# adrelino/mv-lm-icp

Hardware: AMD Instinct MI355X
Metric: ICP iterations/sec (NN+Jacobian+LM) (higher is better)
Workload: dtype f64; 1 GPU; cfg4: multiview 32 views x 200k pts, point-to-plane, SophusSE3 (E=62); views=32, pts_per_view=200000, edges=62, parallelism=single GPU, nn=auto

## Files before the change

mv-lm-icp_amd/csrc/api.cpp:

```cpp
#include <algorithm>
#include <cmath>
#include <cstring>
#include <ctime>
#include <chrono>
#include <condition_variable>
#include <exception>
#include <limits>
#include <mutex>
#include <new>
#include <thread>

#include "common.h"
#include "comm.h"
#include "nn_tie.h"
#include "../host/se3.h"

namespace mvicp {

static thread_local char g_err[1024] = "";

void set_error(const char* fmt, ...) {
  va_list ap;
  va_start(ap, fmt);
  vsnprintf(g_err, sizeof(g_err), fmt, ap);
// ... 35 lines not shown

int scratch_upload(mvicp_ctx* c, const void* src, size_t bytes, void** dptr) {
  const size_t aligned = (bytes + 255) & ~(size_t)255;
  if (c->scratch_used + aligned > c->scratch_bytes) {
    if (c->scratch_used != 0) { set_error("scratch overflow (%zu + %zu > %zu)", c->scratch_used, aligned, c->scratch_bytes); return MVICP_ERR_STATE; }
    MV_HIP(hipStreamSynchronize(c->stream));
    if (c->d_scratch) MV_HIP(hipFree(c->d_scratch));
    c->scratch_bytes = std::max<size_t>(aligned * 4, 1 << 20);
    MV_HIP(hipMalloc((void**)&c->d_scratch, c->scratch_bytes));
  }
  void* d = c->d_scratch + c->scratch_used;
  MV_HIP(hipMemcpyAsync(d, src, bytes, hipMemcpyHostToDevice, c->stream));
  MV_HIP(hipStreamSynchronize(c->stream));
  c->scratch_used += aligned;
  *dptr = d;
  return MVICP_OK;
}

ProfScope::ProfScope(mvicp_ctx* ctx, const char* nm, double bytes) : c(ctx), name(nm), on(ctx->profile) {
  if (on && ctx->profile_level >= 2 && ((std::strncmp(nm, "nn_", 3) != 0 && std::strncmp(nm, "linearize", 9) != 0 && std::strcmp(nm, "comm") != 0) ||
                                        std::strcmp(nm, "nn_tie") == 0)) on = false;
  if (!on) return;
  ProfEntry& pe = c->prof[name];
  auto get = [&]() {
    hipEvent_t ev = nullptr;
    if (!pe.pool.empty()) { ev = pe.pool.back(); pe.pool.pop_back(); }
    else if (hipEventCreate(&ev) != hipSuccess) ev = nullptr;
    return ev;
  };
  a = get(); b = get();
  pe.bytes += bytes;
  if (std::strncmp(nm, "nn_", 3) == 0) { pe.survey_bytes += bytes; pe.queries += bytes / 36.0; }
  pe.launches += 1;
  if (a) (void)hipEventRecord(a, c->stream);
}
ProfScope::~ProfScope() {
  if (!on) return;
  if (b) (void)hipEventRecord(b, c->stream);
  if (a && b) c->prof[name].pending.push_back(std::make_pair(a, b));
}
static double now_ms() {
  timespec ts;
  clock_gettime(CLOCK_MONOTONIC, &ts);
  return ts.tv_sec * 1e3 + ts.tv_nsec * 1e-6;
}
HostScope::HostScope(mvicp_ctx* ctx, const char* nm) : c(ctx), name(nm), t0(0.0), on(ctx->profile) { if (on) t0 = now_ms(); }
HostScope::~HostScope() {
  if (!on) return;
  ProfEntry& pe = c->prof[name];
  pe.ms += now_ms() - t0;
  pe.launches += 1;
}
void prof_collect_lazy(mvicp_ctx* c) {
  for (auto& kv : c->prof) if (kv.second.pending.size() > 256) { prof_collect(c); return; }
}
void prof_collect(mvicp_ctx* c) {
  for (auto& kv : c->prof) {
    ProfEntry& pe = kv.second;
    for (auto& pr : pe.pending) {
      float ms = 0.f;
      if (hipEventSynchronize(pr.second) == hipSuccess && hipEventElapsedTime(&ms, pr.first, pr.second) == hipSuccess) pe.ms += ms;
      pe.pool.push_back(pr.first);
      pe.pool.push_back(pr.second);
    }
    pe.pending.clear();
  }
}

namespace {

template <typename T> int dev_alloc(T** p, size_t n) {
  *p = nullptr;
  if (n == 0) n = 1;
  MV_HIP(hipMalloc((void**)p, sizeof(T) * n));
  return MVICP_OK;
}
template <typename T> void dev_free(T*& p) {
  if (p) (void)hipFree(p);
  p = nullptr;
}

void free_graph(mvicp_ctx* c) {
  dev_free(c->d_esrc); dev_free(c->d_edst); dev_free(c->d_cap_off); dev_free(c->d_count);
  dev_free(c->d_ctl); c->d_nsrc = nullptr; c->d_a = nullptr; c->d_xf = nullptr; c->d_rel = nullptr; c->d_rel2 = nullptr; c->d_dirty = nullptr;
  dev_free(c->d_nn_idx); dev_free(c->d_nn_d2); dev_free(c->d_nn_lb); dev_free(c->d_first); dev_free(c->d_second);
  dev_free(c->d_sblock_off); dev_free(c->d_sel_keys1); c->n_sblocks = 0;
  dev_free(c->d_cd2); dev_free(c->d_qpos); dev_free(c->d_dirty_slots); dev_free(c->d_dslot_off); dev_free(c->d_stream); dev_free(c->d_cblock_off); dev_free(c->d_cblock_cnt);
  dev_free(c->d_sel_hist); dev_free(c->d_median); dev_free(c->d_chunk_edge); dev_free(c->d_chunk_start);
  dev_free(c->d_chunk_first); dev_free(c->d_partials); dev_free(c->d_out);
  c->sym_lo_pin.release(); c->sym_lo_dev.release();
  if (c->h_pin) (void)hipHostFree(c->h_pin);
  c->h_pin = nullptr; c->h_pin_doubles = 0; c->d_res_host = nullptr; c->d_blocks_host = nullptr; c->lin_out = nullptr;
  c->census_pending = false; c->spec_ready = false; c->spec2_ready = false; c->spec_arm = false; c->d_spec_host = nullptr; c->d_adev_host = nullptr; c->d_res_target = nullptr; c->d_a_check = nullptr;
  dev_free(c->d_xblock_cnt); c->export_valid = false; c->export_in_flight = false; c->export_chunks = 0;
  for (hipEvent_t ev : c->export_events) (void)hipEventDestroy(ev);
  c->export_events.clear();
  if (c->d_export) (void)hipFree(c->d_export);
  if (c->h_export) (void)hipHostFree(c->h_export);
  c->d_export = nullptr; c->h_export = nullptr; c->export_cap = 0;
  c->E = 0; c->total_cap = 0; c->n_cblocks = 0; c->n_chunks = 0; c->have_corr = false;
}

int bind(mvicp_ctx* c) {
  if (!c) { set_error("null context"); return MVICP_ERR_ARG; }
  MV_HIP(hipSetDevice(c->device));
  return MVICP_OK;
}

double sqrt_bound(double t) {
  double x = t * t;
  while (std::sqrt(x) >= t && x > 0.0) x = std::nextafter(x, 0.0);
  while (std::sqrt(x) < t) x = std::nextafter(x, INFINITY);
  return x;
}

void inverse3(const double* m, double* r) {
#define M(i, j) m[(i) + 3 * (j)]
#define COF(i, j) (M(((i) + 1) % 3, ((j) + 1) % 3) * M(((i) + 2) % 3, ((j) + 2) % 3) - M(((i) + 1) % 3, ((j) + 2) % 3) * M(((i) + 2) % 3, ((j) + 1) % 3))
  const double c00 = COF(0, 0), c10 = COF(1, 0), c20 = COF(2, 0);
  const double det = (c00 * M(0, 0) + c10 * M(1, 0)) + c20 * M(2, 0);
  const double invdet = 1.0 / det;
  r[0] = c00 * invdet; r[3] = c10 * invdet; r[6] = c20 * invdet;
  r[1] = COF(0, 1) * invdet; r[4] = COF(1, 1) * invdet; r[7] = COF(2, 1) * invdet;
  r[2] = COF(0, 2) * invdet; r[5] = COF(1, 2) * invdet; r[8] = COF(2, 2) * invdet;
#undef COF
#undef M
}

void fill_query_xf(const double* Ps, const double* Pd, double* x) {
  double Rd[9];
  for (int j = 0; j < 3; ++j)
    for (int i = 0; i < 3; ++i) { x[i + 3 * j] = Ps[i + 4 * j]; Rd[i + 3 * j] = Pd[i + 4 * j]; }
  for (int i = 0; i < 3; ++i) { x[9 + i] = Ps[12 + i]; x[21 + i] = Pd[12 + i]; }
  inverse3(Rd, x + 12);
}

void query_affine(const double* x, double* Mq) {
  for (int j = 0; j < 3; ++j)
    for (int i = 0; i < 3; ++i) Mq[i + 3 * j] = x[12 + i] * x[0 + 3 * j] + x[12 + i + 3] * x[1 + 3 * j] + x[12 + i + 6] * x[2 + 3 * j];
  const double dt[3] = {x[9] - x[21], x[10] - x[22], x[11] - x[23]};
  for (int i = 0; i < 3; ++i) Mq[9 + i] = x[12 + i] * dt[0] + x[12 + i + 3] * dt[1] + x[12 + i + 6] * dt[2];
}

double cache_allowance_xf(const double* x_old, const double* x_new, double r) {
  if (std::memcmp(x_old, x_new, sizeof(double) * kXfRigid) == 0) return 0.0;
  double b = 0.0;
  for (const double* x : {x_old, x_new}) {
    double fr = 0.0, fi = 0.0;
    for (int k = 0; k < 9; ++k) { fr += x[k] * x[k]; fi += x[12 + k] * x[12 + k]; }
    const double dt[3] = {x[9] - x[21], x[10] - x[22], x[11] - x[23]};
    const double ts = std::sqrt(x[9] * x[9] + x[10] * x[10] + x[11] * x[11]), dtn = std::sqrt(dt[0] * dt[0] + dt[1] * dt[1] + dt[2] * dt[2]);
    b += std::sqrt(fi) * (ts + 16.0 * std::sqrt(fr) * r + 13.0 * dtn);
  }
  return std::max(0x1p-52 * b, std::numeric_limits<double>::min());
}

int ensure_pin(mvicp_ctx* c, size_t doubles) {
  if (doubles <= c->h_pin_doubles) return MVICP_OK;
  if (c->h_pin) MV_HIP(hipHostFree(c->h_pin));
  c->h_pin = nullptr;
  MV_HIP(hipHostMalloc((void**)&c->h_pin, sizeof(double) * doubles, hipHostMallocMapped));
  std::memset(c->h_pin, 0, sizeof(double) * doubles);
  c->h_pin_doubles = doubles;
  return MVICP_OK;
}

}
// ... 128 lines not shown
static int build_frame_structures(mvicp_ctx* c, FrameDev& f, const double* xyz, const double* nrm) {
  if (injected_build_failure(c)) return MVICP_ERR_INTERNAL;
  const auto t0 = std::chrono::steady_clock::now();
  MV_CHECK(build_grid(c, f, xyz));
  if (nrm) MV_CHECK(upload_sorted_normals(f, nrm));
  f.build_ms[0] = std::chrono::duration<double, std::milli>(std::chrono::steady_clock::now() - t0).count();
  f.build_ms[1] = -1.0;
  return MVICP_OK;
}

static int build_frame_structures_device(mvicp_ctx* c, FrameDev& f, const DevBounds& b, int grid_curve, double grid_target) {
  if (injected_build_failure(c)) return MVICP_ERR_INTERNAL;
  return build_grid_device(c, f, b, grid_curve, grid_target);
}

int finish_builds(mvicp_ctx* c) {
  for (FrameDev& f : c->frames) {
    if (!f.job) continue;
    int s1 = MVICP_ERR_INTERNAL;
    try { s1 = f.job->fut.get(); } catch (...) { f.job->err = "structure build threw"; }
    if (s1 != MVICP_OK) {
      f.build_error = f.job->err.empty() ? std::string("structure build failed") : f.job->err;
      (void)hipSetDevice(c->device);
      free_grid(f.grid); f.has_grid = false;
    }
    f.job.reset();
  }
  for (size_t i = 0; i < c->frames.size(); ++i)
    if (!c->frames[i].build_error.empty()) {
      set_error("frame %d: %s (upload the cloud again with mvicp_set_frame)", (int)i, c->frames[i].build_error.c_str());
      return MVICP_ERR_STATE;
    }
  return MVICP_OK;
}

static void throttle_builds(mvicp_ctx* c) {
  const int limit = std::max(2, (int)std::min(32u, std::thread::hardware_concurrency()));
  for (;;) {
    int pending = 0;
    BuildJob* oldest = nullptr;
    for (FrameDev& f : c->frames)
      if (f.job && f.job->fut.valid() && f.job->fut.wait_for(std::chrono::seconds(0)) != std::future_status::ready) { if (!oldest) oldest = f.job.get(); ++pending; }
    if (pending < limit || !oldest) return;
    oldest->fut.wait();
  }
}

static int check_evaluable(mvicp_ctx* c, int metric) {
  if (!c->have_corr) { set_error("no correspondences: call mvicp_correspond or mvicp_set_correspondences first"); return MVICP_ERR_STATE; }
  if (metric == MVICP_METRIC_SYMMETRIC) {
    for (int e = 0; e < c->E; ++e)
      if (c->owned[e] && c->h_count[e] > 0) {
        const int missing = c->frames[c->edst[e]].grid.snor == nullptr ? c->edst[e] : c->frames[c->esrc[e]].grid.snor == nullptr ? c->esrc[e] : -1;
        if (missing >= 0) { set_error("symmetric needs normals on frame %d", missing); return MVICP_ERR_STATE; }
      }
  } else if (metric) {
    for (int e = 0; e < c->E; ++e)
      if (c->owned[e] && c->h_count[e] > 0 && c->frames[c->edst[e]].grid.snor == nullptr) {
        set_error("point-to-plane needs normals on frame %d", c->edst[e]);
        return MVICP_ERR_STATE;
      }
  }
  return MVICP_OK;
}

int evaluate_pair(mvicp_ctx* c, const double* poses_a, const double* poses_b, int plane, int robust, double* out_a, double* out_b) {
  MV_CHECK(check_evaluable(c, plane));
  HostScope hs(c, "host.evaluate");
  const size_t n = (size_t)c->E * MVICP_EDGE_BLOCK;
  fill_rel_into(c, poses_b, c->h_pin + c->ctl_rel2_off);
  fill_rel(c, poses_a);
  MV_HIP(hipMemcpyAsync(c->d_rel2, c->h_pin + c->ctl_rel2_off, sizeof(double) * ((size_t)c->E * kEdgeRel + c->ctl_r2), hipMemcpyHostToDevice, c->stream));
  MV_CHECK(launch_linearize_pair(c, plane, robust, c->d_blocks_host, c->d_blocks2_host));
  MV_CHECK(stream_wait(c));
  std::memcpy(out_a, c->h_pin + c->pin_blocks_off, sizeof(double) * n);
  std::memcpy(out_b, c->h_pin + c->pin_blocks2_off, sizeof(double) * n);
  return MVICP_OK;
}

static int launch_metric(mvicp_ctx* c, int metric, int robust) {
  return metric == MVICP_METRIC_SYMMETRIC ? launch_linearize_sym(c, robust) : launch_linearize(c, metric, robust);
}

int evaluate_blocks(mvicp_ctx* c, const double* poses, int plane, int robust, double* out) {
  MV_CHECK(check_evaluable(c, plane));
  HostScope hs(c, "host.evaluate");
  const size_t n = (size_t)c->E * MVICP_EDGE_BLOCK;
  if (c->spec_ready) {
    c->spec_ready = false;
    if (plane == c->spec_q_plane && robust == c->spec_q_robust && c->spec_poses.size() == 16 * (size_t)c->n_frames &&
        std::memcmp(poses, c->spec_poses.data(), sizeof(double) * c->spec_poses.size()) == 0) {
      std::memcpy(out, c->h_pin + c->pin_spec_off, sizeof(double) * n);
      if (c->profile) c->prof["spec.hit"].launches += 1;
      return MVICP_OK;
    }
    c->spec2_ready = false;
  }
  if (c->spec2_ready) {
    c->spec2_ready = false;
    if (plane == c->spec2_plane && robust == c->spec2_robust && c->spec2_poses.size() == 16 * (size_t)c->n_frames &&
        std::memcmp(poses, c->spec2_poses.data(), sizeof(double) * c->spec2_poses.size()) == 0) {
      std::memcpy(out, c->h_pin + c->pin_spec2_off, sizeof(double) * n);
      if (c->profile) c->prof["spec2.hit"].launches += 1;
      c->last_cand_poses.assign(poses, poses + 16 * (size_t)c->n_frames); c->last_cand_plane = plane; c->last_cand_robust = robust;
      return MVICP_OK;
    }
  }
  c->last_cand_poses.assign(poses, poses + 16 * (size_t)c->n_frames); c->last_cand_plane = plane; c->last_cand_robust = robust;
  double* h = c->h_pin + c->pin_blocks_off;
  if (c->comm || c->ar_fn) {
    c->lin_out = c->d_out;
    int st_l = plane == MVICP_METRIC_SYMMETRIC ? upload_rel_sym(c, poses) : upload_rel(c, poses);
    if (st_l == MVICP_OK && c->fault_inject_eval > 0 && --c->fault_inject_eval == 0) { set_error("injected launch failure (option fault_inject_eval)"); st_l = MVICP_ERR_HIP; }
    if (st_l == MVICP_OK) st_l = launch_metric(c, plane, robust);
    char local_msg[sizeof(g_err)] = "";
    if (st_l != MVICP_OK) std::memcpy(local_msg, g_err, sizeof(local_msg));
    if (hipMemsetAsync(c->d_out + n, st_l == MVICP_OK ? 0 : 0xFF, sizeof(double), c->stream) != hipSuccess) {
      if (st_l != MVICP_OK) return st_l;
      set_error("hipMemsetAsync of the poison slot failed"); return MVICP_ERR_HIP;
    }
    { ProfScope pc(c, "comm", 8.0 * (double)(n + 1)); MV_CHECK(comm_allreduce_sum(c, c->d_out, n + 1)); }
    double* hx = c->h_pin + c->pin_spec_off;
    MV_HIP(hipMemcpyAsync(hx, c->d_out, sizeof(double) * (n + 1), hipMemcpyDeviceToHost, c->stream));
    MV_CHECK(stream_wait(c));
    if (std::isnan(hx[n])) {
      if (st_l != MVICP_OK) { set_error("%s", local_msg); return st_l; }
      set_error("a peer rank failed before the exchange of this evaluation (poisoned exchange buffer)");
      return MVICP_ERR_COMM;
    }
    std::memcpy(out, hx, sizeof(double) * n);
    return MVICP_OK;
  } else {
    MV_CHECK(plane == MVICP_METRIC_SYMMETRIC ? upload_rel_sym(c, poses) : upload_rel(c, poses));
    c->lin_out = c->d_blocks_host;
    MV_CHECK(launch_metric(c, plane, robust));
  }
  MV_CHECK(stream_wait(c));
  std::memcpy(out, h, sizeof(double) * n);
  return MVICP_OK;
}

}

using namespace mvicp;

extern "C" {

const char* mvicp_last_error(void) { return g_err; }
const char* mvicp_version(void) { return "mvicp_hip 0.5 (gfx950)"; }

int mvicp_create(int device, mvicp_ctx** out) try {
  if (!out) { set_error("out is null"); return MVICP_ERR_ARG; }
  *out = nullptr;
  int ndev = 0;
  hipError_t e = hipGetDeviceCount(&ndev);
  if (e != hipSuccess || ndev <= 0) {
    set_error("no HIP device available (%s): libmvicp_hip has no CPU fallback", e == hipSuccess ? "device count 0" : hipGetErrorString(e));
    return MVICP_ERR_HIP;
  }
  if (device < 0 || device >= ndev) { set_error("device %d out of range [0,%d)", device, ndev); return MVICP_ERR_ARG; }
  mvicp_ctx* c = new mvicp_ctx();
  c->device = device;
  MV_HIP(hipSetDevice(device));
  MV_HIP(hipStreamCreateWithFlags(&c->stream, hipStreamNonBlocking));
  *out = c;
  return MVICP_OK;
} MVICP_GUARD_ABI

static void release_stages(mvicp_ctx* c) {
  c->vox.release(); c->out.release(); c->knn.release(); c->fpfh.release();
  c->match.release(); c->cons.release(); c->coarse.release(); c->iss.release();
}

int mvicp_destroy(mvicp_ctx* c) try {
  if (!c) return MVICP_OK;
  (void)hipSetDevice(c->device);
  (void)finish_builds(c);
  (void)hipStreamSynchronize(c->stream);
  comm_destroy(c);
  free_graph(c);
  for (FrameDev& f : c->frames) { dev_free(f.pts); dev_free(f.nor); free_grid(f.grid); free_tie(f); }
  dev_free(c->d_split_idx); dev_free(c->d_split_d2); dev_free(c->d_scratch);
  free_overlap(c);
  release_stages(c);
  for (auto& kv : c->tables) if (kv.second.d) (void)hipFree(kv.second.d);
  if (c->d_census) (void)hipFree(c->d_census);
  if (c->h_census) (void)hipHostFree(c->h_census);
  if (c->d_tie_list) (void)hipFree(c->d_tie_list);
  if (c->d_tie_count) (void)hipFree(c->d_tie_count);
  if (c->d_tie_deep) (void)hipFree(c->d_tie_deep);
  if (c->h_tie_seen) (void)hipHostFree(c->h_tie_seen);
  if (c->h_far_seen) (void)hipHostFree(c->h_far_seen);
  if (c->d_far_list) (void)hipFree(c->d_far_list);
  if (c->d_far_count) (void)hipFree(c->d_far_count);
  for (auto& kv : c->prof) {
    for (auto& pr : kv.second.pending) { (void)hipEventDestroy(pr.first); (void)hipEventDestroy(pr.second); }
    for (hipEvent_t ev : kv.second.pool) (void)hipEventDestroy(ev);
  }
  (void)hipStreamDestroy(c->stream);
  delete c;
  return MVICP_OK;
} MVICP_GUARD_ABI

int mvicp_set_num_frames(mvicp_ctx* c, int n_frames) try {
  MV_CHECK(bind(c));
  if (n_frames < 0) { set_error("n_frames < 0"); return MVICP_ERR_ARG; }
  (void)finish_builds(c);
  if (c->E) free_graph(c);
  release_stages(c);
  for (FrameDev& f : c->frames) { dev_free(f.pts); dev_free(f.nor); free_grid(f.grid); free_tie(f); }
  c->frames.assign(n_frames, FrameDev());
  c->n_frames = n_frames;
  return MVICP_OK;
} MVICP_GUARD_ABI

int mvicp_set_frame(mvicp_ctx* c, int frame, const double* xyz, const double* nrm, int n) try {
  MV_CHECK(bind(c));
  if (frame < 0 || frame >= c->n_frames) { set_error("frame %d out of range [0,%d)", frame, c->n_frames); return MVICP_ERR_ARG; }
  if (n < 0 || (n > 0 && !xyz)) { set_error("bad cloud (n=%d)", n); return MVICP_ERR_ARG; }
  if (c->E) { set_error("set frames before mvicp_set_graph"); return MVICP_ERR_STATE; }
// ... 662 lines not shown
    });
    const int take = std::min<int>(knn, (int)cand.size());
    for (int k = 0; k < take; ++k) {
      parent[root(i)] = root(cand[k]);
      if (i == 0 && skip_frame0) continue;
      if (n_edges >= cap) { set_error("more than cap = %d edges (frame %d of %d, knn = %d)", cap, i, K, knn); return MVICP_ERR_ARG; }
      if (!src || !dst) { set_error("src / dst is null"); return MVICP_ERR_ARG; }
      src[n_edges] = i; dst[n_edges] = cand[k]; ++n_edges;
    }
  }
  if (n_components) {
    int comps = 0;
    for (int i = 0; i < K; ++i) comps += root(i) == i ? 1 : 0;
    *n_components = comps;
  }
  return n_edges;
} MVICP_GUARD_ABI

int mvicp_set_graph(mvicp_ctx* c, int n_edges, const int* src, const int* dst) try {
  MV_CHECK(bind(c));
  if (n_edges < 0 || (n_edges > 0 && (!src || !dst))) { set_error("bad edge list"); return MVICP_ERR_ARG; }
  for (int e = 0; e < n_edges; ++e)
    if (src[e] < 0 || src[e] >= c->n_frames || dst[e] < 0 || dst[e] >= c->n_frames || src[e] == dst[e]) {
      set_error("edge %d (%d->%d) invalid", e, src[e], dst[e]);
      return MVICP_ERR_ARG;
    }
  MV_CHECK(finish_builds(c));
  free_graph(c);
  const int E = n_edges;
  c->E = E;
  c->esrc.assign(src, src + E);
  c->edst.assign(dst, dst + E);
  c->owned.assign(E, 0);
  c->active.assign(E, 0);
  c->h_count.assign(E, 0);
  c->h_weight.assign(E, 0.f);
  {
    std::vector<int> ns(E), owner(E);
    for (int e = 0; e < E; ++e) ns[e] = c->frames[src[e]].n;
    MV_CHECK(mvicp_edge_owner(E, ns.data(), c->world, owner.data()));
    for (int e = 0; e < E; ++e) c->owned[e] = owner[e] == c->rank;
  }
  {
    double total = 0;
    for (int e = 0; e < E; ++e) total += c->frames[src[e]].n;
    c->lin_chunk = total >= 6e6 ? 8192 : total >= 2e6 ? 4096 : total >= 5e5 ? 1024 : 512;
    if (c->lin_chunk_override > 0) c->lin_chunk = c->lin_chunk_override;
  }
  const int kLinChunk = c->lin_chunk;
  c->cap_off.assign(E + 1, 0);
  c->cblock_off.assign(E + 1, 0);
  c->chunk_first.assign(E + 1, 0);
  std::vector<int> chunk_edge, chunk_start;
  for (int e = 0; e < E; ++e) {
    const long long n = c->owned[e] ? c->frames[src[e]].n : 0;
    c->cap_off[e + 1] = c->cap_off[e] + ((n + 63) / 64) * 64;
    c->cblock_off[e + 1] = c->cblock_off[e] + (int)((n + kCompactBlock - 1) / kCompactBlock);
    const int nch = (int)((n + kLinChunk - 1) / kLinChunk);
    c->chunk_first[e + 1] = c->chunk_first[e] + nch;
    for (int k = 0; k < nch; ++k) { chunk_edge.push_back(e); chunk_start.push_back(k * kLinChunk); }
  }
  c->total_cap = c->cap_off[E];
  c->n_cblocks = c->cblock_off[E];
  c->n_chunks = c->chunk_first[E];
  if (c->lin_interleave) {
    std::vector<int> ce, cs;
    for (int e0 = 0; e0 < E;) {
      int e1 = e0 + 1;
      while (e1 < E && src[e1] == src[e0]) ++e1;
      int maxc = 0;
      for (int e = e0; e < e1; ++e) maxc = std::max(maxc, c->chunk_first[e + 1] - c->chunk_first[e]);
      for (int g = 0; g < maxc; g += 8)
        for (int e = e0; e < e1; ++e) {
          const int nch = c->chunk_first[e + 1] - c->chunk_first[e];
          for (int k = g; k < std::min(g + 8, nch); ++k) { ce.push_back(e); cs.push_back(k * kLinChunk); }
        }
      e0 = e1;
    }
    chunk_edge.swap(ce); chunk_start.swap(cs);
  }
  const size_t cap = (size_t)c->total_cap;
  MV_CHECK(dev_alloc(&c->d_esrc, E)); MV_CHECK(dev_alloc(&c->d_edst, E)); MV_CHECK(dev_alloc(&c->d_cap_off, E + 1));
  MV_CHECK(dev_alloc(&c->d_count, E));
  c->ctl_r1 = (size_t)E * kEdgeXf + (size_t)E + 2 * (size_t)E;
  c->ctl_rel2_off = (c->ctl_r1 + 1) & ~(size_t)1;
  c->ctl_r2_off = c->ctl_rel2_off + (size_t)E * kEdgeRel;
  c->ctl_r2 = (size_t)E * (kEdgeRel + 1);
  MV_CHECK(dev_alloc(&c->d_ctl, c->ctl_r2_off + c->ctl_r2));
  MV_HIP(hipMemset(c->d_ctl, 0, sizeof(double) * std::max<size_t>(c->ctl_r2_off + c->ctl_r2, 1)));
  c->d_xf = c->d_ctl; c->d_nsrc = reinterpret_cast<int*>(c->d_ctl + (size_t)E * kEdgeXf); c->d_dirty = c->d_nsrc + E;
  c->d_sel_lohi = c->d_ctl + (size_t)E * (kEdgeXf + 1);
  c->sel_med1.assign(E, -1.0); c->sel_med2.assign(E, -1.0);
  c->d_rel = c->d_ctl + c->ctl_r2_off; c->d_a = c->d_rel + (size_t)E * kEdgeRel; c->d_rel2 = c->d_ctl + c->ctl_rel2_off;
  MV_CHECK(dev_alloc(&c->d_nn_idx, cap)); MV_CHECK(dev_alloc(&c->d_nn_d2, cap)); MV_CHECK(dev_alloc(&c->d_nn_lb, cap));
  c->nn_cache_valid = false; c->prev_q.assign((size_t)E * 12, 0.0); c->nn_cache_edge.assign(E, 0);
  c->auto_prev_dist = 0.0; c->auto_last_method = -1; c->corr_tie_seen = c->corr_far_seen = 1u;
  MV_CHECK(dev_alloc(&c->d_first, cap)); MV_CHECK(dev_alloc(&c->d_second, cap)); MV_CHECK(dev_alloc(&c->d_cd2, cap));
  MV_CHECK(dev_alloc(&c->d_stream, 10 * cap));
  MV_CHECK(dev_alloc(&c->d_qpos, cap));
  MV_HIP(hipMemset(c->d_qpos, 0xff, sizeof(int) * std::max<size_t>(cap, 1)));
  c->list_valid.assign(E, 0); c->explicit_list.assign(E, 0); c->export_valid = false; c->export_off.assign((size_t)E + 1, 0);
  c->qpos_valid.assign(E, 0); c->corr_epoch.assign(E, 0);
  for (int e = 0; e < E; ++e) c->corr_epoch[e] = ++c->epoch_counter;
  c->dslot_off.assign(E + 1, 0);
  for (int e = 0; e < E; ++e) c->dslot_off[e + 1] = c->dslot_off[e] + (int)(((c->owned[e] ? c->frames[src[e]].n : 0) + 255) / 256);
  c->n_dslots = c->dslot_off[E];
  MV_CHECK(dev_alloc(&c->d_dirty_slots, (size_t)c->n_dslots)); MV_CHECK(dev_alloc(&c->d_dslot_off, (size_t)E + 1));
  MV_HIP(hipMemset(c->d_dirty_slots, 0, sizeof(int) * std::max<size_t>((size_t)c->n_dslots, 1)));
  MV_HIP(hipMemcpy(c->d_dslot_off, c->dslot_off.data(), sizeof(int) * (E + 1), hipMemcpyHostToDevice));
  MV_CHECK(dev_alloc(&c->d_cblock_off, E + 1)); MV_CHECK(dev_alloc(&c->d_cblock_cnt, (size_t)c->n_cblocks));
  MV_CHECK(dev_alloc(&c->d_sel_hist, (size_t)E * (2048 + 2)));
  MV_HIP(hipMemset(c->d_sel_hist, 0, sizeof(unsigned int) * std::max<size_t>((size_t)E * (2048 + 2), 1)));
  c->sel_scratch_clean = true; c->sel_result_valid = false; c->sel_result_armed = false;
  c->sblock_off.assign(E + 1, 0);
  for (int e = 0; e < E; ++e) c->sblock_off[e + 1] = c->sblock_off[e] + (int)(((c->owned[e] ? c->frames[src[e]].n : 0) + kSelBlock - 1) / kSelBlock);
  c->n_sblocks = c->sblock_off[E];
  MV_CHECK(dev_alloc(&c->d_sblock_off, (size_t)E + 1));
  MV_HIP(hipMemcpy(c->d_sblock_off, c->sblock_off.data(), sizeof(int) * (E + 1), hipMemcpyHostToDevice));
  MV_CHECK(dev_alloc(&c->d_sel_keys1, cap));
  if (cap > c->far_cap) {
    if (c->d_far_list) MV_HIP(hipFree(c->d_far_list));
    c->d_far_list = nullptr; c->far_cap = 0;
    MV_HIP(hipMalloc(&c->d_far_list, sizeof(int) * 2 * cap));
    c->far_cap = cap;
  }
  MV_CHECK(warm_nn_grid(c)); MV_CHECK(warm_nn_tile(c)); MV_CHECK(warm_nn_mfma(c));
  if (c->tie_rule && !(c->tie_lazy && c->world == 1)) {
    std::vector<int> need;
    for (int e = 0; e < E; ++e) if (c->owned[e]) need.push_back(dst[e]);
    MV_CHECK(ensure_tie_trees(c, need));
  }
  MV_CHECK(dev_alloc(&c->d_median, E));
  MV_CHECK(dev_alloc(&c->d_chunk_edge, (size_t)c->n_chunks)); MV_CHECK(dev_alloc(&c->d_chunk_start, (size_t)c->n_chunks));
  MV_CHECK(dev_alloc(&c->d_chunk_first, E + 1));
  MV_CHECK(dev_alloc(&c->d_partials, 2 * (size_t)c->n_chunks * kLinPartial));
  MV_CHECK(dev_alloc(&c->d_out, (size_t)E * (MVICP_EDGE_BLOCK + 3) + 2));
  MV_HIP(hipMemset(c->d_out, 0, sizeof(double) * ((size_t)E * (MVICP_EDGE_BLOCK + 3) + 2)));
  if (E) {
    MV_HIP(hipMemcpy(c->d_esrc, src, sizeof(int) * E, hipMemcpyHostToDevice));
    MV_HIP(hipMemcpy(c->d_edst, dst, sizeof(int) * E, hipMemcpyHostToDevice));
    MV_HIP(hipMemset(c->d_count, 0, sizeof(int) * E));
  }
  MV_HIP(hipMemcpy(c->d_cap_off, c->cap_off.data(), sizeof(long long) * (E + 1), hipMemcpyHostToDevice));
  MV_HIP(hipMemcpy(c->d_cblock_off, c->cblock_off.data(), sizeof(int) * (E + 1), hipMemcpyHostToDevice));
  MV_HIP(hipMemcpy(c->d_chunk_first, c->chunk_first.data(), sizeof(int) * (E + 1), hipMemcpyHostToDevice));
  if (c->n_chunks) {
    MV_HIP(hipMemcpy(c->d_chunk_edge, chunk_edge.data(), sizeof(int) * c->n_chunks, hipMemcpyHostToDevice));
    MV_HIP(hipMemcpy(c->d_chunk_start, chunk_start.data(), sizeof(int) * c->n_chunks, hipMemcpyHostToDevice));
  }
  c->pin_blocks_off = c->ctl_r2_off + c->ctl_r2;
  c->pin_res_off = c->pin_blocks_off + (size_t)E * MVICP_EDGE_BLOCK;
  c->pin_misc_off = c->pin_res_off + 2 * (size_t)E + 2;
  c->pin_spec_off = c->pin_misc_off + 4 * (size_t)E + 64;
  c->pin_adev_off = c->pin_spec_off + (size_t)E * (MVICP_EDGE_BLOCK + 3) + 2;
  if (c->h_pin) { MV_HIP(hipHostFree(c->h_pin)); c->h_pin = nullptr; c->h_pin_doubles = 0; }
  c->pin_spec2_off = (c->pin_adev_off + (size_t)E + 8 + 1) & ~(size_t)1;
  c->pin_rel2_off = c->pin_spec2_off + (size_t)E * MVICP_EDGE_BLOCK + ((size_t)E * MVICP_EDGE_BLOCK & 1);
  c->pin_blocks2_off = (c->pin_rel2_off + (size_t)E * kEdgeRel + 1) & ~(size_t)1;
  MV_CHECK(ensure_pin(c, c->pin_blocks2_off + (size_t)E * MVICP_EDGE_BLOCK + 8));
  {
    void* dp = nullptr;
    MV_HIP(hipHostGetDevicePointer(&dp, c->h_pin, 0));
    c->d_blocks_host = (double*)dp + c->pin_blocks_off;
    c->d_res_host = (double*)dp + c->pin_res_off;
    c->d_spec_host = (double*)dp + c->pin_spec_off;
    c->d_adev_host = (double*)dp + c->pin_adev_off;
    c->d_spec2_host = (double*)dp + c->pin_spec2_off;
    c->d_blocks2_host = (double*)dp + c->pin_blocks2_off;
  }
  c->spec_ready = false; c->spec_arm = false;
  c->spec2_ready = false; c->spec2_armed = false; c->last_cand_poses.clear();
  c->prev_xf.assign((size_t)E * kXfRigid, 0.0);
  if (!c->h_census) MV_HIP(hipHostMalloc((void**)&c->h_census, 8 * sizeof(unsigned long long), hipHostMallocDefault));
  return MVICP_OK;
} MVICP_GUARD_ABI

static void forget_history(mvicp_ctx* c) {
  const int E = c->E;
  c->nn_cache_valid = false; c->nn_cache_thresh = -1.f;
  c->prev_q.assign((size_t)E * 12, 0.0); c->prev_xf.assign((size_t)E * kXfRigid, 0.0);
  c->nn_cache_edge.assign(E, 0);
  c->auto_prev_dist = 0.0; c->auto_last_method = -1; c->last_rms = -1.0; c->prev_grid_kernel = false;
  c->corr_tie_seen = c->corr_far_seen = 1u;
  c->list_valid.assign(E, 0);
  c->export_valid = false;
  c->qpos_valid.assign(E, 0);
  for (int e = 0; e < E; ++e) c->corr_epoch[e] = ++c->epoch_counter;
  c->sel_med1.assign(E, -1.0); c->sel_med2.assign(E, -1.0);
  c->sel_result_valid = false;
  c->spec_ready = false; c->spec_arm = false; c->spec_flags_valid = false;
  c->spec2_ready = false; c->spec2_armed = false; c->last_cand_poses.clear();
  c->have_corr = false;
  std::fill(c->h_count.begin(), c->h_count.end(), 0); std::fill(c->h_weight.begin(), c->h_weight.end(), 0.f);
}

int mvicp_reset_history(mvicp_ctx* c) try {
  MV_CHECK(bind(c));
  MV_HIP(hipStreamSynchronize(c->stream));
  forget_history(c);
  return MVICP_OK;
} MVICP_GUARD_ABI

static int correspond_once(mvicp_ctx* c, const double* poses, const unsigned char* fixed, float thresh, int nn_method, int* counts, float* weights, bool* tie_unresolved);

int mvicp_correspond(mvicp_ctx* c, const double* poses, const unsigned char* fixed, float thresh, int nn_method, int* counts, float* weights) try {
  MV_CHECK(bind(c));
  struct Forget { mvicp_ctx* c; bool ok = false; ~Forget() { if (!ok) { (void)hipStreamSynchronize(c->stream); forget_history(c); } } } forget{c};
  bool unresolved = false;
  MV_CHECK(correspond_once(c, poses, fixed, thresh, nn_method, counts, weights, &unresolved));
  if (!unresolved) { forget.ok = true; return MVICP_OK; }
  std::vector<int> need;
  for (int e = 0; e < c->E; ++e) if (c->active[e] && !c->frames[c->edst[e]].has_tie) need.push_back(c->edst[e]);
  MV_HIP(hipStreamSynchronize(c->stream));
  MV_CHECK(ensure_tie_trees(c, need));
  forget_history(c);
  unresolved = false;
  MV_CHECK(correspond_once(c, poses, fixed, thresh, nn_method, counts, weights, &unresolved));
  if (unresolved) { set_error("tie fix-up still without a tree after building them"); return MVICP_ERR_INTERNAL; }
  forget.ok = true;
  return MVICP_OK;
} MVICP_GUARD_ABI

static int correspond_body(mvicp_ctx* c, const double* poses, const unsigned char* fixed, float thresh, int nn_method, int* counts, float* weights, bool* tie_unresolved);

static int correspond_once(mvicp_ctx* c, const double* poses, const unsigned char* fixed, float thresh, int nn_method, int* counts, float* weights, bool* tie_unresolved) {
  struct Guard { mvicp_ctx* c; bool ok = false; ~Guard() { if (!ok) { c->sel_result_valid = false; c->sel_scratch_clean = false; } } } guard{c};
  const int st = correspond_body(c, poses, fixed, thresh, nn_method, counts, weights, tie_unresolved);
  guard.ok = st == MVICP_OK;
  return st;
}

static int correspond_body(mvicp_ctx* c, const double* poses, const unsigned char* fixed, float thresh, int nn_method, int* counts, float* weights, bool* tie_unresolved) {
  if (!poses) { set_error("poses is null"); return MVICP_ERR_ARG; }
  if (c->E == 0) { set_error("no graph: call mvicp_set_graph first"); return MVICP_ERR_STATE; }
  const int E = c->E;
  HostScope hs_all(c, "host.correspond");
  std::vector<int> nsrc(E, 0);
  std::vector<char> same_edge(E, 0);
  std::vector<char> unchanged(E, 0);
  const bool hist_ok = c->have_corr && (int)c->nn_cache_edge.size() == E && c->nn_cache_thresh == thresh && (int)c->qpos_valid.size() == E;
  std::vector<double> eps_ratio;
  bool same_active_set = (int)c->nn_cache_edge.size() == E;
  double* hx = c->h_pin;
  for (int e = 0; e < E; ++e) {
    c->active[e] = c->owned[e] && !(fixed && fixed[c->esrc[e]]);
    if (same_active_set && (c->active[e] != 0) != (c->nn_cache_edge[e] != 0)) same_active_set = false;
    nsrc[e] = c->active[e] ? c->frames[c->esrc[e]].n : 0;
    const double* Ps = poses + 16 * (size_t)c->esrc[e];
    const double* Pd = poses + 16 * (size_t)c->edst[e];
    double* x = hx + (size_t)e * kEdgeXf;
    fill_query_xf(Ps, Pd, x);
    double Mq[12];
    query_affine(x, Mq);
    double* pq = &c->prev_q[(size_t)e * 12];
    for (int k = 0; k < 12; ++k) x[kXfDM + k] = Mq[k] - pq[k];
    const double rmax = c->frames[c->esrc[e]].max_norm;
    if (c->active[e]) {
      double fro = 0.0;
      for (int k = 0; k < 9; ++k) fro += x[kXfDM + k] * x[kXfDM + k];
      const double eps_e = std::sqrt(fro) * rmax + std::sqrt(x[kXfDv] * x[kXfDv] + x[kXfDv + 1] * x[kXfDv + 1] + x[kXfDv + 2] * x[kXfDv + 2]);
      const double mu_e = c->tile_mu * c->frames[c->edst[e]].grid.cell;
      eps_ratio.push_back(mu_e > 0.0 ? eps_e / mu_e : 1e300);
    }
    const bool cache_on = c->nn_cache_valid && c->nn_cache_enable && c->active[e] && (int)c->nn_cache_edge.size() == E && c->nn_cache_edge[e] &&
                          c->nn_cache_thresh == thresh;
    double* pxf = &c->prev_xf[(size_t)e * kXfRigid];
    if (!c->owned[e]) unchanged[e] = 1;
    else if (c->active[e]) unchanged[e] = hist_ok && c->nn_cache_edge[e] && c->qpos_valid[e] && !c->explicit_list[e] && std::memcmp(pxf, x, sizeof(double) * kXfRigid) == 0;
    else unchanged[e] = hist_ok && !c->nn_cache_edge[e] && !c->explicit_list[e] && c->h_count[e] == 0;
    const bool same_xf = cache_on && std::memcmp(pxf, x, sizeof(double) * kXfRigid) == 0;
    x[kXfCache] = cache_on ? cache_allowance_xf(pxf, x, rmax) : -1.0;
    same_edge[e] = same_xf;
    std::memcpy(pxf, x, sizeof(double) * kXfRigid);
    for (int k = kXfPad; k < kEdgeXf; ++k) x[k] = 0.0;
    std::memcpy(pq, Mq, sizeof(Mq));
  }
  int* hn = reinterpret_cast<int*>(hx + (size_t)E * kEdgeXf);
  int* hd = hn + E;
  std::memcpy(hn, nsrc.data(), sizeof(int) * E);

  int st_local = MVICP_OK;
  if (c->tie_rule && !(c->tie_lazy && c->world == 1)) {
    std::vector<int> need;
    for (int e = 0; e < E; ++e) if (c->active[e] && !c->frames[c->edst[e]].has_tie) need.push_back(c->edst[e]);
    if (!need.empty()) st_local = ensure_tie_trees(c, need);
  }
  const double bound = sqrt_bound((double)thresh);
  double t_mark = now_ms();
  auto mark = [&](const char* nm) { if (c->profile) { const double t = now_ms(); ProfEntry& pe = c->prof[nm]; pe.ms += t - t_mark; pe.launches += 1; t_mark = t; } };
  mark("host.corr.setup");
  int method = nn_method;
  if (method == MVICP_NN_AUTO) {
    method = MVICP_NN_TILE;
    if (c->have_corr) {
      double dist = 0.0, cell = 0.0;
      int m = 0;
      for (int e = 0; e < E; ++e)
        if (c->h_count[e] > 0) { dist += c->h_weight[e] / 1.5; cell += c->frames[c->edst[e]].grid.cell; ++m; }
      if (m > 0) {
        dist /= m; cell /= m;
        const bool settled = c->auto_prev_dist > 0.0 ? dist > c->auto_settle * c->auto_prev_dist : dist < 0.5 * cell;
        if (c->nn_cell) {
          double pred = dist;
          if (c->last_rms >= 0.0) pred = std::min(pred, std::sqrt(c->last_rms * c->last_rms + 0.09 * cell * cell));
          if (pred < c->auto_switch * cell || c->auto_last_method == MVICP_NN_GRID) method = MVICP_NN_GRID;
        } else if (dist < 1.5 * cell && (settled || c->auto_last_method == MVICP_NN_GRID)) method = MVICP_NN_GRID;
        c->auto_prev_dist = dist;
      }
    }
  }
  if (method == MVICP_NN_GRID || method == MVICP_NN_TILE) {
    for (int e = 0; e < E; ++e)
      if (c->active[e] && (!c->frames[c->edst[e]].has_grid || !c->frames[c->esrc[e]].has_grid)) method = MVICP_NN_BRUTE;
  }
  bool tile_lb = false, handed_over = false;
  if (nn_method == MVICP_NN_AUTO && method == MVICP_NN_GRID && c->auto_last_method == MVICP_NN_TILE && c->tile_bounds >= 1 &&
      c->nn_cache_enable && !c->nn_cell) { method = MVICP_NN_TILE; tile_lb = true; handed_over = true; }
  if (method == MVICP_NN_TILE && c->tile_bounds >= 2 && c->nn_cache_enable) tile_lb = true;
  bool tile_cached = false;
  bool all_same = true;
  {
    for (int e = 0; e < E; ++e) if (c->active[e] && !same_edge[e]) all_same = false;
    if (nn_method == MVICP_NN_AUTO && method == MVICP_NN_GRID && !handed_over && c->tile_cache && c->tile_bounds >= 1 && c->nn_cache_valid &&
        c->nn_cache_enable && !c->nn_cell && !all_same) { method = MVICP_NN_TILE; tile_lb = true; tile_cached = true; handed_over = true; }
    if (method == MVICP_NN_TILE && !tile_cached && c->tile_cache >= 2 && tile_lb && c->nn_cache_valid && c->nn_cache_enable && !all_same) tile_cached = true;
  }
  {
    std::vector<int> dirty(E, 1);
    if ((method == MVICP_NN_TILE || (method == MVICP_NN_GRID && !c->nn_tree_only && !c->nn_skip_far)) && c->list_reuse)
      for (int e = 0; e < E; ++e) if (c->active[e] && c->list_valid[e]) dirty[e] = 0;
    std::memcpy(hd, dirty.data(), sizeof(int) * E);
  }
  bool use_bracket = c->sel_bracket && c->have_corr;
  {
    double* lohi = hx + (size_t)E * (kEdgeXf + 1);
    for (int e = 0; e < E; ++e) {
      lohi[2 * e] = lohi[2 * e + 1] = 0.0;
      if (!c->active[e]) continue;
      const double m1 = c->sel_med1[e], m2 = c->sel_med2[e];
      if (!(m1 > 0.0 && m2 > 0.0 && std::fabs(m1 - m2) <= 0.001 * m1)) { use_bracket = false; continue; }
      lohi[2 * e] = m1 * 0.994; lohi[2 * e + 1] = m1 * 1.006;
    }
  }
  bool nothing_can_change = method == MVICP_NN_GRID && c->list_reuse && !c->nn_tree_only && !c->nn_skip_far && same_active_set && !c->nn_cell;
  for (int e = 0; e < E && nothing_can_change; ++e)
    if (c->active[e] && !(same_edge[e] && hd[e] == 0)) nothing_can_change = false;
  c->skip_dirty_reduce = nothing_can_change;
  c->tie_skip = nothing_can_change && c->corr_tie_seen == 0u;
  c->far_skip = nothing_can_change && c->corr_far_seen == 0u && c->prev_grid_kernel && method == MVICP_NN_GRID;
  const bool tie_launched = c->tie_rule && !c->tie_skip, far_launched = method == MVICP_NN_GRID && !c->far_skip;
  const bool exchange = c->comm != nullptr || c->ar_fn != nullptr;
  c->spec_ready = false; c->spec2_ready = false;
  c->spec_arm = c->spec_enable && c->spec_flags_valid;
  if (c->spec_arm && c->spec_plane)
    for (int e = 0; e < E; ++e) if (!(fixed && fixed[c->esrc[e]]) && c->frames[c->edst[e]].n > 0 && c->frames[c->edst[e]].grid.snor == nullptr) c->spec_arm = false;
  const size_t nb = (size_t)E * MVICP_EDGE_BLOCK, ntail = 3 * (size_t)E + 1;
  c->d_res_target = exchange ? c->d_out + nb : nullptr;
  c->d_a_check = exchange ? c->d_out + nb + 2 * (size_t)E + 1 : c->d_adev_host;
  size_t upload_doubles = c->ctl_r1;
  bool spec2_plan = false;
  if (c->spec_arm) {
    c->spec_poses.resize(16 * (size_t)c->n_frames);
    double xp[7];
    for (int k = 0; k < c->n_frames; ++k) { se3::pose_to_x(c->spec_param, poses + 16 * (size_t)k, xp); se3::x_to_pose(c->spec_param, xp, &c->spec_poses[16 * (size_t)k]); }
    fill_rel(c, c->spec_poses.data());
    c->spec_q_plane = c->spec_plane; c->spec_q_robust = c->spec_robust;
    upload_doubles = c->ctl_r2_off + (size_t)E * kEdgeRel;
    spec2_plan = !exchange && c->spec2_enable && all_same && same_active_set && c->have_corr && c->last_cand_poses.size() == 16 * (size_t)c->n_frames &&
                 c->last_cand_plane == c->spec_q_plane && c->last_cand_robust == c->spec_q_robust;
    if (spec2_plan && c->lin_pair) fill_rel_into(c, c->last_cand_poses.data(), hx + c->ctl_rel2_off);
  }
  const bool sel_skip = !exchange && c->sel_reuse && nothing_can_change && c->sel_result_valid && (!c->spec_arm || c->sel_result_armed);
  if (method != MVICP_NN_BRUTE && method != MVICP_NN_GRID && method != MVICP_NN_TILE) { set_error("unknown nn_method %d", nn_method); return MVICP_ERR_ARG; }
  bool all_unchanged = true;
  for (int e = 0; e < E; ++e) { if (!unchanged[e]) all_unchanged = false; if (c->active[e]) c->qpos_valid[e] = 0; }
  auto local_search = [&]() -> int {
  MV_HIP(hipMemcpyAsync(c->d_ctl, hx, sizeof(double) * upload_doubles, hipMemcpyHostToDevice, c->stream));
  c->far_narrow = nn_method == MVICP_NN_AUTO && method == MVICP_NN_GRID && c->nn_cache_valid && c->nn_cache_enable && all_same;
  if (c->fault_inject > 0 && --c->fault_inject == 0) { set_error("injected launch failure (option fault_inject)"); return MVICP_ERR_HIP; }
  if (method == MVICP_NN_BRUTE) MV_CHECK(launch_nn_brute_edges(c));
  else if (method == MVICP_NN_GRID) MV_CHECK(launch_nn_grid_edges(c, bound));
  else {
    c->cached_on_mfma = false;
    if (tile_cached && c->tile_mfma == 1 && c->cache_mfma_ratio > 0.0 && !eps_ratio.empty()) {
      std::nth_element(eps_ratio.begin(), eps_ratio.begin() + eps_ratio.size() / 2, eps_ratio.end());
      const double med = eps_ratio[eps_ratio.size() / 2];
      if (c->profile) { ProfEntry& pe = c->prof["auto.eps_over_mu"]; pe.ms = med; pe.launches += 1; }
      c->cached_on_mfma = med > c->cache_mfma_ratio;
    }
    MV_CHECK(launch_nn_tile_edges(c, bound, tile_lb, tile_cached, c->list_reuse));
  }
  c->tie_skip = false; c->far_skip = false;
  c->prev_grid_kernel = method == MVICP_NN_GRID;
  c->last_rms = -1.0;
  c->nn_cache_valid = ((method == MVICP_NN_GRID) && !c->nn_tree_only && !c->nn_skip_far) || tile_lb;
  c->nn_cache_thresh = thresh;
  c->auto_last_method = handed_over ? MVICP_NN_GRID : method;
  c->nn_cache_edge.assign(c->active.begin(), c->active.end());
  for (int e = 0; e < E; ++e) { c->list_valid[e] = c->active[e]; if (c->owned[e]) c->qpos_valid[e] = c->active[e]; if (c->active[e]) c->explicit_list[e] = 0; }
  if (!all_unchanged) c->export_valid = false;

  mark("host.corr.nn_launch");
  if (!nothing_can_change) {
    MV_CHECK(launch_compact(c, bound));
    MV_CHECK(launch_gather_stream(c));
  }
  if (sel_skip) { c->h_pin[c->pin_res_off + 2 * (size_t)E] = c->spec_arm ? 1.0 : 0.0; return MVICP_OK; }
  return use_bracket ? launch_select_bracket(c) : launch_select_median(c, bound);
  };
  if (st_local == MVICP_OK) st_local = local_search();
  if (st_local != MVICP_OK && !exchange) { c->spec_flags_valid = false; return st_local; }
  int st_q = MVICP_OK;
  char local_msg[sizeof(g_err)] = "";
  if (exchange) {
    c->lin_out = c->d_out;
    if (st_local == MVICP_OK) {
      if (c->spec_arm) st_local = launch_linearize(c, c->spec_q_plane, c->spec_q_robust);
      else {
        if (hipMemsetAsync(c->d_out, 0, sizeof(double) * nb, c->stream) != hipSuccess ||
            hipMemsetAsync(c->d_out + nb + 2 * (size_t)E + 1, 0, sizeof(double) * (size_t)E, c->stream) != hipSuccess) { set_error("hipMemsetAsync of the exchange buffer failed"); st_local = MVICP_ERR_HIP; }
      }
    }
    if (st_local != MVICP_OK) {
      std::memcpy(local_msg, g_err, sizeof(local_msg));
      if (hipMemsetAsync(c->d_out + nb + 2 * (size_t)E, 0xFF, sizeof(double), c->stream) != hipSuccess) {
        set_error("%s — and the exchange buffer could not be poisoned: the peers of this rank will block in the collective", local_msg);
        c->spec_flags_valid = false; c->spec_arm = false;
        return st_local;
      }
    }
    { ProfScope pc(c, "comm", 8.0 * (double)(nb + ntail)); st_q = comm_allreduce_sum(c, c->d_out, nb + ntail); }
    if (st_q == MVICP_OK && hipMemcpyAsync(c->h_pin + c->pin_spec_off, c->d_out, sizeof(double) * (nb + ntail), hipMemcpyDeviceToHost, c->stream) != hipSuccess) {
      set_error("hipMemcpyAsync of the exchanged buffer failed"); st_q = MVICP_ERR_HIP;
    }
  } else if (c->spec_arm && spec2_plan && c->lin_pair) {
    c->spec2_armed = false;
    st_q = launch_linearize_pair(c, c->spec_q_plane, c->spec_q_robust, c->d_spec_host, c->d_spec2_host);
    if (st_q == MVICP_OK) { c->spec2_armed = true; c->spec2_poses = c->last_cand_poses; c->spec2_plane = c->spec_q_plane; c->spec2_robust = c->spec_q_robust; }
  } else if (c->spec_arm) {
    c->lin_out = c->d_spec_host;
    st_q = launch_linearize(c, c->spec_q_plane, c->spec_q_robust);
    c->spec2_armed = false;
    if (st_q == MVICP_OK && spec2_plan) {
      fill_rel_into(c, c->last_cand_poses.data(), c->h_pin + c->pin_rel2_off);
      if (hipMemcpyAsync(c->d_rel, c->h_pin + c->pin_rel2_off, sizeof(double) * (size_t)E * kEdgeRel, hipMemcpyHostToDevice, c->stream) == hipSuccess) {
        c->lin_out = c->d_spec2_host;
        st_q = launch_linearize(c, c->spec_q_plane, c->spec_q_robust);
        if (st_q == MVICP_OK) { c->spec2_armed = true; c->spec2_poses = c->last_cand_poses; c->spec2_plane = c->spec_q_plane; c->spec2_robust = c->spec_q_robust; }
      }
    }
  }
  mark("host.corr.post_launch");
  if (st_q == MVICP_OK) st_q = stream_wait(c);
  if (st_q != MVICP_OK) { c->spec_flags_valid = false; c->spec_arm = false; return st_q; }
  if (exchange && std::isnan(c->h_pin[c->pin_spec_off + nb + 2 * (size_t)E])) {
    forget_history(c);
    c->census_pending = false;
    if (st_local != MVICP_OK) { set_error("%s", local_msg); return st_local; }
    set_error("a peer rank failed before the exchange of this search (poisoned exchange buffer); nothing was updated, cross-round state dropped on every rank");
    return MVICP_ERR_COMM;
  }
  census_resolve(c);
  if (tie_launched) c->corr_tie_seen = c->h_tie_seen ? *c->h_tie_seen : 1u;
  if (tie_launched && c->h_tie_seen && c->h_tie_seen[1] != 0u) *tie_unresolved = true;
  if (tie_launched && c->h_tie_seen && c->h_tie_seen[2] != 0u) { set_error("tie fix-up: a walk ran out of stack (a tree deeper than its recorded levels)"); return MVICP_ERR_INTERNAL; }
  if (far_launched) c->corr_far_seen = c->h_far_seen ? *c->h_far_seen : 1u;
  else if (method != MVICP_NN_GRID) c->corr_far_seen = 1u;
  mark("host.corr.wait");
  const double* hr = exchange ? c->h_pin + c->pin_spec_off + nb : c->h_pin + c->pin_res_off;
  bool spec_bad = false;
  {
    bool redo = false;
    for (int e = 0; e < E; ++e) if (hr[2 * e + 1] < 0.0) redo = true;
    if (redo) {
      spec_bad = true;
      int st_r = launch_select_median(c, bound);
      if (exchange) {
        int st_x = MVICP_OK;
        if (st_r != MVICP_OK) {
          std::memcpy(local_msg, g_err, sizeof(local_msg));
          if (hipMemsetAsync(c->d_out + nb + 2 * (size_t)E, 0xFF, sizeof(double), c->stream) != hipSuccess) { c->spec_flags_valid = false; c->spec_arm = false; return st_r; }
        }
        { ProfScope pc(c, "comm", 8.0 * (double)ntail); st_x = comm_allreduce_sum(c, c->d_out + nb, ntail); }
        if (st_x == MVICP_OK && hipMemcpyAsync(c->h_pin + c->pin_spec_off + nb, c->d_out + nb, sizeof(double) * ntail, hipMemcpyDeviceToHost, c->stream) != hipSuccess) {
          set_error("hipMemcpyAsync of the exchanged tail failed"); st_x = MVICP_ERR_HIP;
        }
        if (st_x == MVICP_OK) st_x = stream_wait(c);
        if (st_x != MVICP_OK) { c->spec_flags_valid = false; c->spec_arm = false; return st_x; }
// ... 182 lines not shown
  c->have_corr = true;
  const int one = 1;
  MV_HIP(hipMemcpy(c->d_dirty + edge, &one, sizeof(int), hipMemcpyHostToDevice));
  MV_CHECK(launch_gather_stream(c));
  MV_HIP(hipStreamSynchronize(c->stream));
  return MVICP_OK;
} MVICP_GUARD_ABI

int mvicp_nn_query(mvicp_ctx* c, int frame, const double* queries, int n, int nn_method, int* idx, double* d2) try {
  MV_CHECK(bind(c));
  if (frame < 0 || frame >= c->n_frames) { set_error("frame %d out of range", frame); return MVICP_ERR_ARG; }
  if (n < 0 || (n && (!queries || !idx || !d2))) { set_error("bad query buffers"); return MVICP_ERR_ARG; }
  if (nn_method < MVICP_NN_AUTO || nn_method > MVICP_NN_TILE) { set_error("unknown nn_method %d", nn_method); return MVICP_ERR_ARG; }
  MV_CHECK(finish_builds(c));
  const FrameDev& f = c->frames[frame];
  if (f.n == 0) { set_error("frame %d is empty (nanoflann throws here: nanoflann.hpp:904)", frame); return MVICP_ERR_STATE; }
  if (n == 0) return MVICP_OK;
  double* dq = nullptr; int* di = nullptr; double* dd = nullptr;
  MV_CHECK(dev_alloc(&dq, 3 * (size_t)n)); MV_CHECK(dev_alloc(&di, (size_t)n)); MV_CHECK(dev_alloc(&dd, (size_t)n));
  MV_HIP(hipMemcpy(dq, queries, sizeof(double) * 3 * (size_t)n, hipMemcpyHostToDevice));
  int method = (nn_method == MVICP_NN_AUTO || nn_method == MVICP_NN_TILE) ? MVICP_NN_GRID : nn_method;
  if (c->tie_rule) MV_CHECK(ensure_tie_trees(c, std::vector<int>(1, frame)));
  c->tie_skip = false;
  if (method == MVICP_NN_GRID && !f.has_grid) method = MVICP_NN_BRUTE;
  int st;
  if (method == MVICP_NN_BRUTE) st = launch_nn_brute_queries(c, f, dq, n, di, dd);
  else if (method == MVICP_NN_GRID) st = launch_nn_grid_queries(c, f, dq, n, di, dd);
  else { set_error("unknown nn_method %d", nn_method); st = MVICP_ERR_ARG; }
  if (st == MVICP_OK) {
    hipError_t e1 = hipStreamSynchronize(c->stream);
    if (e1 == hipSuccess) census_resolve(c);
    if (e1 == hipSuccess && c->tie_rule && c->h_tie_seen && c->h_tie_seen[2] != 0u) { set_error("tie fix-up: a walk ran out of stack (a tree deeper than its recorded levels)"); st = MVICP_ERR_INTERNAL; }
    hipError_t e2 = hipMemcpy(idx, di, sizeof(int) * n, hipMemcpyDeviceToHost);
    hipError_t e3 = hipMemcpy(d2, dd, sizeof(double) * n, hipMemcpyDeviceToHost);
    if (e1 != hipSuccess || e2 != hipSuccess || e3 != hipSuccess) { set_error("nn_query copy-back failed"); st = MVICP_ERR_HIP; }
  }
  dev_free(dq); dev_free(di); dev_free(dd);
  if (c->profile) prof_collect_lazy(c);
  return st;
} MVICP_GUARD_ABI

int mvicp_linearize(mvicp_ctx* c, const double* poses, int point_to_plane, int robust, double* out) try {
  MV_CHECK(bind(c));
  if (!poses || !out) { set_error("null argument"); return MVICP_ERR_ARG; }
  if (c->E == 0) { set_error("no graph"); return MVICP_ERR_STATE; }
  MV_CHECK(evaluate_blocks(c, poses, point_to_plane ? MVICP_METRIC_PLANE : MVICP_METRIC_POINT, robust, out));
  if (c->profile) prof_collect_lazy(c);
  return MVICP_OK;
} MVICP_GUARD_ABI

int mvicp_linearize_metric(mvicp_ctx* c, const double* poses, int metric, int robust, double* out) try {
  if (metric != MVICP_METRIC_POINT && metric != MVICP_METRIC_PLANE && metric != MVICP_METRIC_SYMMETRIC) { set_error("metric %d is not an mvicp_metric", metric); return MVICP_ERR_ARG; }
  MV_CHECK(bind(c));
  if (!poses || !out) { set_error("null argument"); return MVICP_ERR_ARG; }
  if (c->E == 0) { set_error("no graph"); return MVICP_ERR_STATE; }
  MV_CHECK(evaluate_blocks(c, poses, metric, robust, out));
  if (c->profile) prof_collect_lazy(c);
  return MVICP_OK;
} MVICP_GUARD_ABI

int mvicp_linearize_pair(mvicp_ctx* c, const double* poses_a, const double* poses_b, int point_to_plane, int robust, double* out_a, double* out_b) try {
  MV_CHECK(bind(c));
  if (!poses_a || !poses_b || !out_a || !out_b) { set_error("null argument"); return MVICP_ERR_ARG; }
  if (c->E == 0) { set_error("no graph"); return MVICP_ERR_STATE; }
  if (c->comm || c->ar_fn) {
    MV_CHECK(evaluate_blocks(c, poses_a, point_to_plane ? MVICP_METRIC_PLANE : MVICP_METRIC_POINT, robust, out_a));
    MV_CHECK(evaluate_blocks(c, poses_b, point_to_plane ? MVICP_METRIC_PLANE : MVICP_METRIC_POINT, robust, out_b));
  } else {
    MV_CHECK(evaluate_pair(c, poses_a, poses_b, point_to_plane ? MVICP_METRIC_PLANE : MVICP_METRIC_POINT, robust, out_a, out_b));
  }
  if (c->profile) prof_collect_lazy(c);
  return MVICP_OK;
} MVICP_GUARD_ABI

int mvicp_set_option(mvicp_ctx* c, const char* name, double value) try {
  MV_CHECK(bind(c));
  if (!name) { set_error("null option name"); return MVICP_ERR_ARG; }
  if (std::strcmp(name, "async_build") == 0) { c->async_build = value != 0.0; return MVICP_OK; }
  if (std::strcmp(name, "grid_target") == 0 || std::strcmp(name, "grid_curve") == 0) MV_CHECK(finish_builds(c));
  if (std::strcmp(name, "nn_tree_only") == 0) { c->nn_tree_only = value != 0.0; return MVICP_OK; }
  if (std::strcmp(name, "nn_cache") == 0) { c->nn_cache_enable = value != 0.0; c->nn_cache_valid = false; return MVICP_OK; }
  if (std::strcmp(name, "lin_chunk") == 0) { c->lin_chunk_override = (int)value; return MVICP_OK; }
  if (std::strcmp(name, "list_reuse") == 0) { c->list_reuse = value != 0.0; return MVICP_OK; }
  if (std::strcmp(name, "lin_interleave") == 0) { c->lin_interleave = value != 0.0; return MVICP_OK; }
  if (std::strcmp(name, "lin_share_p") == 0) { c->lin_share_p = value != 0.0; return MVICP_OK; }
  if (std::strcmp(name, "lin_pair") == 0) { c->lin_pair = value != 0.0; return MVICP_OK; }
  if (std::strcmp(name, "nn_census") == 0) { c->nn_census = value != 0.0; return MVICP_OK; }
  if (std::strcmp(name, "nn_skip_far") == 0) { c->nn_skip_far = value != 0.0; return MVICP_OK; }
  if (std::strcmp(name, "sel_bracket") == 0) { c->sel_bracket = value != 0.0; return MVICP_OK; }
  if (std::strcmp(name, "sel_reuse") == 0) { c->sel_reuse = value != 0.0; return MVICP_OK; }
  if (std::strcmp(name, "prune_rho") == 0) { c->prune_rho = value; return MVICP_OK; }
  if (std::strcmp(name, "grid_curve") == 0) { c->grid_curve = (int)value; return MVICP_OK; }
  if (std::strcmp(name, "auto_settle") == 0) { c->auto_settle = value; return MVICP_OK; }
  if (std::strcmp(name, "auto_switch") == 0) { c->auto_switch = value; return MVICP_OK; }
  if (std::strcmp(name, "nn_cell") == 0) { c->nn_cell = value != 0.0; return MVICP_OK; }
  if (std::strcmp(name, "nn_search_factor") == 0) { if (!(value >= 0.0)) { set_error("nn_search_factor < 0"); return MVICP_ERR_ARG; } c->nn_search_factor = value; c->nn_cache_valid = false; return MVICP_OK; }
  if (std::strcmp(name, "tie_rule") == 0) {
    const bool on = value != 0.0;
    if (on != c->tie_rule) { MV_HIP(hipStreamSynchronize(c->stream)); c->tie_rule = on; forget_history(c); }
    return MVICP_OK;
  }
  if (std::strcmp(name, "tie_lazy") == 0) { c->tie_lazy = value != 0.0; return MVICP_OK; }
  if (std::strcmp(name, "tile_seed") == 0) { c->tile_seed = value != 0.0; return MVICP_OK; }
  if (std::strcmp(name, "tile_bounds") == 0) { c->tile_bounds = (int)value; return MVICP_OK; }
  if (std::strcmp(name, "tile_mu") == 0) { if (!(value > 0.0 && value <= 1.0)) { set_error("tile_mu outside (0, 1]"); return MVICP_ERR_ARG; } c->tile_mu = value; return MVICP_OK; }
  if (std::strcmp(name, "mfma_kacc") == 0) { if (!(value >= 1.0 && value <= 1024.0)) { set_error("mfma_kacc outside [1, 1024]"); return MVICP_ERR_ARG; } c->mfma_kacc = value; return MVICP_OK; }
  if (std::strcmp(name, "mfma_lbt") == 0) { c->mfma_lbt = (int)value; return MVICP_OK; }
  if (std::strcmp(name, "mfma_entry") == 0) { c->mfma_entry = (int)value; return MVICP_OK; }
  if (std::strcmp(name, "mfma_trig") == 0) { c->mfma_trig = (int)value; return MVICP_OK; }
  if (std::strcmp(name, "tile_mfma") == 0) { c->tile_mfma = (int)value; return MVICP_OK; }
  if (std::strcmp(name, "tile_waves") == 0) { c->tile_waves = (int)value; return MVICP_OK; }
  if (std::strcmp(name, "cache_mfma_ratio") == 0) { c->cache_mfma_ratio = value; return MVICP_OK; }
  if (std::strcmp(name, "reject_cache") == 0) { c->reject_cache = value != 0.0; return MVICP_OK; }
  if (std::strcmp(name, "tile_miss") == 0) { if (!(value >= 0.0 && value <= 64.0)) { set_error("tile_miss outside [0, 64]"); return MVICP_ERR_ARG; } c->tile_miss = (int)value; return MVICP_OK; }
  if (std::strcmp(name, "tile_cache") == 0) { c->tile_cache = (int)value; return MVICP_OK; }
  if (std::strcmp(name, "voxel_permute") == 0) { c->voxel_permute = value != 0.0; return MVICP_OK; }
  if (std::strcmp(name, "knn_order") == 0) { c->knn_order = value != 0.0; return MVICP_OK; }
  if (std::strcmp(name, "match_chunk") == 0) {
    if (!(value >= 1.0 && value < 2147483648.0)) { set_error("match_chunk must be in [1, 2^31)"); return MVICP_ERR_ARG; }
    c->match_chunk = (int)value; return MVICP_OK;
  }
  if (std::strcmp(name, "spin_wait") == 0) { c->spin_wait = value != 0.0; return MVICP_OK; }
  if (std::strcmp(name, "fault_inject") == 0) { c->fault_inject = (int)value; return MVICP_OK; }
  if (std::strcmp(name, "fault_inject_build") == 0) { c->fault_inject_build.store((int)value); return MVICP_OK; }
  if (std::strcmp(name, "fault_inject_eval") == 0) { c->fault_inject_eval = (int)value; return MVICP_OK; }
  if (std::strcmp(name, "spec_eval") == 0) { c->spec_enable = value != 0.0; c->spec_ready = false; c->spec2_ready = false; return MVICP_OK; }
  if (std::strcmp(name, "spec2_eval") == 0) { c->spec2_enable = value != 0.0; c->spec2_ready = false; return MVICP_OK; }
  if (std::strcmp(name, "grid_target") == 0) {
    if (!(value >= 0.5 && value <= 64.0)) { set_error("grid_target out of range"); return MVICP_ERR_ARG; }
    c->grid_target = value;
    return MVICP_OK;
  }
  set_error("unknown option '%s'", name);
  return MVICP_ERR_ARG;
} MVICP_GUARD_ABI
int mvicp_nn_census_ex(mvicp_ctx* c, double* out, int cap) try {
  MV_CHECK(bind(c));
  if (!out || cap < 0) { set_error("bad output buffer"); return MVICP_ERR_ARG; }
  const double v[10] = {c->nn_queries, c->nn_candidates, c->nn_nodes, c->nn_far, c->nn_hits, c->nn_fetched, c->nn_dbg[0], c->nn_dbg[1], c->nn_dbg[2], c->nn_dbg[3]};
  const int n = std::min(cap, 10);
  for (int i = 0; i < n; ++i) out[i] = v[i];
  return n;
} MVICP_GUARD_ABI
int mvicp_nn_census(mvicp_ctx* c, double* out5) try {
  const int n = mvicp_nn_census_ex(c, out5, 5);
  return n < 0 ? n : MVICP_OK;
} MVICP_GUARD_ABI

int mvicp_profile_enable(mvicp_ctx* c, int on) try {
  MV_CHECK(bind(c));
  c->profile = on != 0;
  c->profile_level = on;
  return MVICP_OK;
} MVICP_GUARD_ABI
int mvicp_profile_reset(mvicp_ctx* c) try {
  MV_CHECK(bind(c));
  MV_HIP(hipStreamSynchronize(c->stream));
  prof_collect(c);
  for (auto& kv : c->prof) { kv.second.ms = 0; kv.second.launches = 0; kv.second.bytes = 0; kv.second.survey_bytes = 0; kv.second.queries = 0; }
  c->nn_candidates = c->nn_nodes = c->nn_far = c->nn_queries = c->nn_hits = c->nn_fetched = 0;
  for (int k = 0; k < 4; ++k) c->nn_dbg[k] = 0;
  return MVICP_OK;
} MVICP_GUARD_ABI
static void prof_sum(mvicp_ctx* c, const char* kernel, double out[5]) {
  for (int k = 0; k < 5; ++k) out[k] = 0.0;
  const std::string key = kernel ? kernel : "";
// ... 38 lines not shown
```

mv-lm-icp_amd/csrc/common.h:

```cpp
#pragma once
#include <hip/hip_runtime.h>

#include <atomic>
#include <cstdarg>
#include <cstdio>
#include <future>
#include <map>
#include <memory>
#include <string>
#include <vector>

#include "../../include/mvicp.h"
#include "abi_guard.h"

namespace mvicp {

void set_error(const char* fmt, ...);

#define MV_HIP(expr)                                                                          \
  do {                                                                                        \
    hipError_t _e = (expr);                                                                   \
    if (_e != hipSuccess) {                                                                   \
      mvicp::set_error("%s:%d: %s -> %s", __FILE__, __LINE__, #expr, hipGetErrorString(_e));  \
      return MVICP_ERR_HIP;                                                                   \
// ... 117 lines not shown
};
struct OutlierStage {
  DevBuf dev, tmp; PinBuf pin;
  double* xyz = nullptr; double* nrm = nullptr; double* mdist = nullptr; double* kd2 = nullptr; int* idx = nullptr;
  long long n = -1, kept = -1; int has_normals = 0;
  void release() { dev.release(); tmp.release(); pin.release(); *this = OutlierStage(); }
};
struct KnnStage {
  DevBuf dev, ent, tmp; PinBuf pin;
  int* cnt = nullptr; long long* off = nullptr; int* idx = nullptr; double* d2 = nullptr;
  long long m = -1, total = 0; int k = 0;
  void release() { dev.release(); ent.release(); tmp.release(); pin.release(); *this = KnnStage(); }
};
struct FpfhStage {
  DevBuf dev;
  double* desc = nullptr; int* used = nullptr;
  long long rows = -1;
  void release() { dev.release(); *this = FpfhStage(); }
};
struct MatchStage {
  DevBuf dev, tmp;
  int* fwd_idx = nullptr; int* bwd_idx = nullptr; double* fwd_d2 = nullptr; double* bwd_d2 = nullptr;
  long long m = -1, n = -1;
  void release() { dev.release(); tmp.release(); *this = MatchStage(); }
};
struct ConsensusStage {
  DevBuf dev;
  int* count = nullptr; unsigned char* flags = nullptr;
  long long H = -1, c = -1;
  void release() { dev.release(); *this = ConsensusStage(); }
};
struct CoarseStage {
  DevBuf dev, tmp, work;
  int* pairs = nullptr; unsigned char* flags = nullptr;
  std::vector<long long> seg; std::vector<int> cnt;
  int edges = -1;
  void release() { dev.release(); tmp.release(); work.release(); *this = CoarseStage(); }
};
struct IssStage {
  DevBuf dev, tmp; PinBuf pin;
  double* sal = nullptr; int* cnt_s = nullptr; int* cnt_n = nullptr; int* idx = nullptr; double* xyz = nullptr; double* nrm = nullptr;
  long long n = -1, k = 0; int has_normals = 0;
  void release() { dev.release(); tmp.release(); pin.release(); *this = IssStage(); }
};

struct RcclApi;

}

struct mvicp_ctx {
  int device = 0;
  hipStream_t stream = nullptr;
  int n_frames = 0;
  std::vector<mvicp::FrameDev> frames;

  int rank = 0, world = 1;
  int E = 0;
  std::vector<int> esrc, edst;
  std::vector<char> owned;
  std::vector<long long> cap_off;
  long long total_cap = 0;
  std::vector<int> h_count;
  std::vector<float> h_weight;
  bool have_corr = false;

  double* d_ctl = nullptr; size_t ctl_r1 = 0, ctl_rel2_off = 0, ctl_r2_off = 0, ctl_r2 = 0;
  int* d_esrc = nullptr; int* d_edst = nullptr;
  long long* d_cap_off = nullptr;
  int* d_nsrc = nullptr;
  int* d_count = nullptr;
  double* d_a = nullptr;
  double* d_xf = nullptr;
  double* d_rel = nullptr;
  double* d_rel2 = nullptr;
  int* d_nn_idx = nullptr; double* d_nn_d2 = nullptr;
  float* d_nn_lb = nullptr;
  bool nn_cache_valid = false; bool nn_cache_enable = true; float nn_cache_thresh = -1.f;
  std::vector<char> nn_cache_edge;
  std::vector<double> prev_q;
  std::vector<double> prev_xf;
  int* d_first = nullptr; int* d_second = nullptr; double* d_cd2 = nullptr;
  int* d_qpos = nullptr;
  int* d_dirty = nullptr;
  int* d_dirty_slots = nullptr; int* d_dslot_off = nullptr; std::vector<int> dslot_off; int n_dslots = 0;
  std::vector<char> list_valid;
  std::vector<char> explicit_list;
  void* d_export = nullptr; void* h_export = nullptr; size_t export_cap = 0;
  int* d_xblock_cnt = nullptr;
  std::vector<long long> export_off;
  bool export_valid = false;
  std::vector<hipEvent_t> export_events; std::vector<int> export_edge_chunk; int export_chunks = 0; bool export_in_flight = false;
  std::vector<char> qpos_valid;
  std::vector<unsigned long long> corr_epoch;
  unsigned long long epoch_counter = 0;
  double* d_stream = nullptr;
  int n_cblocks = 0;
  std::vector<int> cblock_off;
  int* d_cblock_off = nullptr; int* d_cblock_cnt = nullptr;
  unsigned int* d_sel_hist = nullptr;
  double* d_median = nullptr;
  int n_sblocks = 0; std::vector<int> sblock_off; int* d_sblock_off = nullptr;
  double* d_sel_lohi = nullptr;
  std::vector<double> sel_med1, sel_med2;
  bool sel_bracket = true;
  bool sel_scratch_clean = false;
  bool sel_reuse = true;
  bool sel_result_valid = false;
  bool sel_result_armed = false;
  double* d_sel_keys1 = nullptr;
  bool lin_interleave = true;
  bool lin_share_p = true;
  int lin_chunk_override = 0;
  int lin_chunk = 4096;
  int n_chunks = 0;
  std::vector<int> chunk_first;
  int* d_chunk_edge = nullptr; int* d_chunk_start = nullptr; int* d_chunk_first = nullptr;
  double* d_partials = nullptr;
  bool lin_pair = true;
  mvicp::PinBuf sym_lo_pin; mvicp::DevBuf sym_lo_dev;
  double* d_out = nullptr;
  double* d_res_target = nullptr;
  double* h_pin = nullptr; size_t h_pin_doubles = 0;
  size_t pin_blocks_off = 0, pin_res_off = 0, pin_misc_off = 0;
  double* d_res_host = nullptr;
  double* d_blocks_host = nullptr;
  double* lin_out = nullptr;
  bool spec_enable = true; bool spec_flags_valid = false; int spec_param = 0, spec_plane = 0, spec_robust = 0;
  int spec_q_plane = 0, spec_q_robust = 0;
  bool spec_arm = false;
  bool spec_ready = false;
  std::vector<double> spec_poses;
  size_t pin_spec_off = 0, pin_adev_off = 0; double* d_spec_host = nullptr; double* d_adev_host = nullptr;
  bool spec2_enable = true, spec2_armed = false, spec2_ready = false; int spec2_plane = 0, spec2_robust = 0;
  std::vector<double> spec2_poses;
  std::vector<double> last_cand_poses;
  int last_cand_plane = -1, last_cand_robust = -1;
  size_t pin_spec2_off = 0, pin_rel2_off = 0; double* d_spec2_host = nullptr;
  size_t pin_blocks2_off = 0; double* d_blocks2_host = nullptr;
  double* d_a_check = nullptr;
  bool spin_wait = false;
  unsigned long long* h_census = nullptr;
  bool census_pending = false; double census_nq = 0; int census_kind = 0; const char* census_scope = "nn_grid";
  int* d_split_idx = nullptr; double* d_split_d2 = nullptr; size_t split_cap = 0;

  char* ov_dev = nullptr; char* ov_pin = nullptr; size_t ov_bytes = 0;

  mvicp::VoxelStage vox;
  int voxel_permute = 1;
  mvicp::OutlierStage out;
  mvicp::KnnStage knn;
  int knn_order = 1;
  mvicp::FpfhStage fpfh;
  mvicp::MatchStage match;
  int match_chunk = 2048;
  mvicp::ConsensusStage cons;
  mvicp::CoarseStage coarse;
  mvicp::IssStage iss;

  struct CachedTable { std::vector<char> bytes; void* d = nullptr; size_t cap = 0; };
  std::map<std::string, CachedTable> tables;
  char* d_scratch = nullptr; size_t scratch_bytes = 0, scratch_used = 0;
  std::vector<char> active;

  mvicp::RcclApi* rccl = nullptr;
  void* comm = nullptr;
  mvicp_allreduce_fn ar_fn = nullptr; void* ar_user = nullptr;
  std::vector<double> ar_host;

  bool async_build = true;
  std::atomic<int> fault_inject_build{0};
  int fault_inject = 0, fault_inject_eval = 0;
  bool list_reuse = true;
  bool nn_tree_only = false;
  bool nn_census = false;
  void* d_census = nullptr; size_t census_bytes = 0;
  void* d_far_list = nullptr; size_t far_cap = 0; unsigned int* d_far_count = nullptr;
  int far_parity = 0;
  unsigned int* h_far_seen = nullptr; unsigned int* d_far_seen = nullptr;
  bool prev_grid_kernel = false;
  bool far_skip = false;
  bool far_narrow = false;
  bool skip_dirty_reduce = false;
  bool nn_skip_far = false;
  double nn_search_factor = 4.0;
  bool tie_lazy = true;
  bool tie_rule = true;
  unsigned long long* d_tie_list = nullptr; size_t tie_cap = 0; unsigned int* d_tie_count = nullptr; int tie_parity = 0;
  void* d_tie_deep = nullptr; size_t tie_deep_bytes = 0;
  unsigned int* h_tie_seen = nullptr; unsigned int* d_tie_seen = nullptr;
  unsigned int corr_tie_seen = 1u, corr_far_seen = 1u;
  bool tie_skip = false;
  bool tile_seed = true;
  int tile_bounds = 1;
  int tile_cache = 1;
  double cache_mfma_ratio = 3.0;
  bool cached_on_mfma = false;
  bool reject_cache = true;
  int tile_miss = 8;
  double tile_mu = 0.02;
  int tile_mfma = 1;
  double mfma_kacc = 34.0;
  int mfma_lbt = 1;
  int mfma_entry = 0;
  int mfma_trig = 2;
  int tile_waves = 0;
  double auto_prev_dist = 0.0; int auto_last_method = -1; double auto_settle = 0.5;
  double last_rms = -1.0;
  bool nn_cell = false;
  double auto_switch = 1.0;
  double prune_rho = 0.05;
  int grid_curve = 2;
  double grid_target = 5.0;
  double nn_candidates = 0, nn_nodes = 0, nn_far = 0, nn_queries = 0, nn_hits = 0, nn_fetched = 0;
  double nn_dbg[4] = {0, 0, 0, 0};

  bool profile = false; int profile_level = 0;
  std::map<std::string, mvicp::ProfEntry> prof;
};

namespace mvicp {

int launch_nn_brute_edges(mvicp_ctx* c);
int launch_nn_brute_queries(mvicp_ctx* c, const FrameDev& f, const double* d_q, int n, int* d_idx, double* d_d2);
int launch_nn_grid_edges(mvicp_ctx* c, double d2_bound);
double search_bound(const mvicp_ctx* c, double d2_bound);
int launch_nn_tile_edges(mvicp_ctx* c, double d2_bound, bool with_bounds, bool with_cache, bool with_list);
int launch_nn_mfma_edges(mvicp_ctx* c, double d2_bound, bool with_bounds, bool with_cache, bool with_list);
int build_mfma(FrameDev& f, const double* sorted_pts);
int warm_nn_mfma(mvicp_ctx* c);
int warm_nn_tile(mvicp_ctx* c); int warm_nn_grid(mvicp_ctx* c);
int build_wide(FrameDev& f, const double* sorted_pts);
int launch_nn_grid_queries(mvicp_ctx* c, const FrameDev& f, const double* d_q, int n, int* d_idx, double* d_d2);
int build_grid(mvicp_ctx* c, FrameDev& f, const double* h_xyz);
int device_bounds(hipStream_t stream, const double* d_xyz, int n, DevBounds* out);
int build_grid_device(mvicp_ctx* c, FrameDev& f, const DevBounds& b, int grid_curve, double grid_target);
int finish_builds(mvicp_ctx* c);
void free_grid(GridDev& g);
void free_tie(FrameDev& f);
int overlap_census(mvicp_ctx* c, const double* xf, double B2, double scale, int max_samples, int* samples, int* hits, long long* sumq);
void free_overlap(mvicp_ctx* c);
long long voxel_reduce(mvicp_ctx* c, int n_sel, const int* sel, const double* poses, double voxel, int* has_normals);
long long outlier_filter(mvicp_ctx* c, const FrameDev& f, int k, double std_ratio, double radius, mvicp_outlier_stats* stats);
long long knn_search(mvicp_ctx* c, const FrameDev& f, const double* queries, int queries_on_device, long long m, int k, double radius, double B2);
long long fpfh_compute(mvicp_ctx* c, const FrameDev& f, int max_nn, double radius, double B2);
long long feature_match(mvicp_ctx* c, const double* A, int a_on_device, long long m, const double* B, int b_on_device, long long n, int dim);
int consensus(mvicp_ctx* c, const double* P, int p_on_device, const double* Q, int q_on_device, long long n_pairs, long long H, unsigned long long seed,
              double tau, double edge_sim, mvicp_consensus_result* out);
long long coarse_pairs(mvicp_ctx* c, const double* desc, int desc_on_device, const double* xyz, int xyz_on_device, const long long* offsets, int n_sets, int dim,
                       int n_edges, const int* src, const int* dst, const unsigned long long* seeds, int mutual, double ratio, long long H, double tau,
                       double edge_sim, mvicp_coarse_edge* results);
long long iss_keypoints(mvicp_ctx* c, const FrameDev& f, double B2_salient, double B2_nms, int q, double gamma21, double gamma32, int min_neighbors);
int launch_compact(mvicp_ctx* c, double d2_bound);
int launch_gather_stream(mvicp_ctx* c);
int launch_select_median(mvicp_ctx* c, double d2_bound);
int launch_export(mvicp_ctx* c);
int launch_select_bracket(mvicp_ctx* c);
int launch_linearize(mvicp_ctx* c, int plane, int robust);
int launch_linearize_pair(mvicp_ctx* c, int plane, int robust, double* out_a, double* out_b);
int launch_linearize_sym(mvicp_ctx* c, int robust);
int launch_normals(mvicp_ctx* c, FrameDev& f, int k, int* d_knn);
int stream_wait(mvicp_ctx* c);
void census_resolve(mvicp_ctx* c);

int cached_upload(mvicp_ctx* c, const char* key, const void* src, size_t bytes, void** dptr);
void scratch_reset(mvicp_ctx* c);
int scratch_upload(mvicp_ctx* c, const void* src, size_t bytes, void** dptr);

struct ProfScope {
  mvicp_ctx* c; const char* name; hipEvent_t a = nullptr, b = nullptr; bool on;
  ProfScope(mvicp_ctx* c, const char* name, double bytes);
  ~ProfScope();
};
void prof_collect(mvicp_ctx* c);
void prof_collect_lazy(mvicp_ctx* c);
struct HostScope {
  mvicp_ctx* c; const char* name; double t0; bool on;
  HostScope(mvicp_ctx* c, const char* name);
  ~HostScope();
};

}
```

mv-lm-icp_amd/csrc/corr.hip:

```cpp
#include "common.h"

#include <cstring>

namespace mvicp {

namespace {

constexpr int NT = 256;
constexpr int IPT = kCompactBlock / NT;

__device__ __forceinline__ int find_edge(const int* __restrict__ off, int E, int b) {
  int lo = 0, hi = E;
  while (hi - lo > 1) {
    const int mid = (lo + hi) >> 1;
    if (off[mid] <= b) lo = mid; else hi = mid;
  }
  return lo;
}

__device__ __forceinline__ int block_exclusive_scan(int v, int* __restrict__ wave_tot, int* total) {
  const int lane = threadIdx.x & 63, wave = threadIdx.x >> 6;
  int inc = v;
#pragma unroll
  for (int d = 1; d < 64; d <<= 1) {
// ... 59 lines not shown
}

__global__ __launch_bounds__(NT) void scatter_kernel(const int* __restrict__ cblock_off, int E, const int* __restrict__ nsrc,
                                                     const long long* __restrict__ cap_off, const int* __restrict__ nn_idx,
                                                     const double* __restrict__ nn_d2, double bound, const int* __restrict__ cblock_cnt,
                                                     int* __restrict__ first, int* __restrict__ second, double* __restrict__ cd2,
                                                     int* __restrict__ qpos, const int* __restrict__ dirty) {
  __shared__ int wave_tot[NT / 64];
  const int b = blockIdx.x;
  const int e = find_edge(cblock_off, E, b);
  if (dirty[e] == 0) return;
  const int lb = b - cblock_off[e];
  const int n = nsrc[e];
  const long long base = cap_off[e];
  int idx[IPT];
  double d2[IPT];
  bool ok[IPT];
  int cnt = 0;
#pragma unroll
  for (int i = 0; i < IPT; ++i) {
    const int k = lb * kCompactBlock + threadIdx.x * IPT + i;
    ok[i] = false;
    if (k < n) {
      idx[i] = nn_idx[base + k];
      d2[i] = nn_d2[base + k];
      ok[i] = idx[i] >= 0 && d2[i] < bound;
    }
    cnt += ok[i] ? 1 : 0;
  }
  int total;
  int pos = cblock_cnt[b] + block_exclusive_scan(cnt, wave_tot, &total);
#pragma unroll
  for (int i = 0; i < IPT; ++i) {
    const int k = lb * kCompactBlock + threadIdx.x * IPT + i;
    if (k < n) qpos[base + k] = ok[i] ? pos : -1;
    if (!ok[i]) continue;
    first[base + pos] = k;
    second[base + pos] = idx[i];
    cd2[base + pos] = d2[i];
    ++pos;
  }
}

__global__ __launch_bounds__(NT) void gather_kernel(const int* __restrict__ cblock_off, int E, const int* __restrict__ count,
                                                    const long long* __restrict__ cap_off, long long total_cap, const int* __restrict__ first,
                                                    const int* __restrict__ second, const PointRec* const* __restrict__ src_rec,
                                                    const PointRec* const* __restrict__ dst_rec, const double* const* __restrict__ dst_nor,
                                                    double* __restrict__ stream, const int* __restrict__ dirty) {
  const int b = blockIdx.x;
  const int e = find_edge(cblock_off, E, b);
  if (dirty[e] == 0) return;
  const int lb = b - cblock_off[e];
  const int cnt = count[e];
  if (lb * kCompactBlock >= cnt) return;
  const long long base = cap_off[e];
  const PointRec* __restrict__ sp = src_rec[e];
  const PointRec* __restrict__ dp = dst_rec[e];
  const double* __restrict__ dn = dst_nor[e];
  for (int i = 0; i < IPT; ++i) {
    const int pos = lb * kCompactBlock + i * NT + threadIdx.x;
    if (pos >= cnt) break;
    const size_t f = (size_t)first[base + pos], s = (size_t)second[base + pos];
    const size_t o = (size_t)(base + pos);
    const double2* pa = reinterpret_cast<const double2*>(sp + f);
    const double2 a0 = pa[0], a1 = pa[1];
    const double2* pb = reinterpret_cast<const double2*>(dp + s);
    const double2 b0 = pb[0], b1 = pb[1];
    __builtin_nontemporal_store(a0.x, &stream[0 * total_cap + o]);
    __builtin_nontemporal_store(a0.y, &stream[1 * total_cap + o]);
    __builtin_nontemporal_store(a1.x, &stream[2 * total_cap + o]);
    __builtin_nontemporal_store(b0.x, &stream[7 * total_cap + o]);
    __builtin_nontemporal_store(b0.y, &stream[8 * total_cap + o]);
    __builtin_nontemporal_store(b1.x, &stream[9 * total_cap + o]);
    if (dn != nullptr) {
      const double n0 = dn[3 * s], n1 = dn[3 * s + 1], n2 = dn[3 * s + 2];
      __builtin_nontemporal_store(n0, &stream[3 * total_cap + o]);
      __builtin_nontemporal_store(n1, &stream[4 * total_cap + o]);
      __builtin_nontemporal_store(n2, &stream[5 * total_cap + o]);
      __builtin_nontemporal_store(n0 * b0.x + n1 * b0.y + n2 * b1.x, &stream[6 * total_cap + o]);
    }
  }
}

constexpr int kSelBins = 2048;
constexpr int kSelShift = 46;

__device__ __forceinline__ unsigned int sel_bin(unsigned long long key, long long kbq) {
  const long long d = kbq - (long long)(key >> kSelShift);
  return d <= 0 ? (unsigned int)(kSelBins - 1) : d >= kSelBins - 1 ? 0u : (unsigned int)(kSelBins - 1 - d);
}

template <int PER, typename F>
__device__ __forceinline__ void pick_bin(F get, unsigned int k, int* __restrict__ wave_tot, int* __restrict__ sh_pick, int& bin, unsigned int& below) {
  unsigned int h[PER];
  int mine = 0;
#pragma unroll
  for (int i = 0; i < PER; ++i) { h[i] = get(threadIdx.x * PER + i); mine += (int)h[i]; }
  int total;
  const int ex = block_exclusive_scan(mine, wave_tot, &total);
  if (threadIdx.x == 0) { sh_pick[0] = NT * PER - 1; sh_pick[1] = total; }
  __syncthreads();
  if ((unsigned int)ex <= k && k < (unsigned int)(ex + mine)) {
    unsigned int cum = (unsigned int)ex;
#pragma unroll
    for (int i = 0; i < PER; ++i) {
      if (cum + h[i] > k) { sh_pick[0] = threadIdx.x * PER + i; sh_pick[1] = (int)cum; break; }
      cum += h[i];
    }
  }
  __syncthreads();
  bin = sh_pick[0]; below = (unsigned int)sh_pick[1];
  __syncthreads();
}

__global__ __launch_bounds__(NT) void select_hist_kernel(const int* __restrict__ sblock_off, int E, const int* __restrict__ count,
                                                         const long long* __restrict__ cap_off, const double* __restrict__ keys,
                                                         long long kbq, unsigned int* __restrict__ hist) {
  constexpr int SPT = kSelBlock / NT;
  __shared__ unsigned int lh[kSelBins];
  const int b = blockIdx.x;
  const int e = find_edge(sblock_off, E, b);
  const int lb = b - sblock_off[e];
  const int cnt = count[e];
  if ((long long)lb * kSelBlock >= cnt) return;
  for (int i = threadIdx.x; i < kSelBins; i += NT) lh[i] = 0u;
  __syncthreads();
  const long long base = cap_off[e];
#pragma unroll
  for (int i = 0; i < SPT / 2; ++i) {
    const int pos = lb * kSelBlock + 2 * (i * NT + threadIdx.x);
    if (pos + 1 < cnt) {
      typedef double d2v __attribute__((ext_vector_type(2)));
      const d2v v = __builtin_nontemporal_load(reinterpret_cast<const d2v*>(keys + base + pos));
      atomicAdd(&lh[sel_bin((unsigned long long)__double_as_longlong(v.x), kbq)], 1u);
      atomicAdd(&lh[sel_bin((unsigned long long)__double_as_longlong(v.y), kbq)], 1u);
    } else if (pos < cnt) {
      atomicAdd(&lh[sel_bin((unsigned long long)__double_as_longlong(keys[base + pos]), kbq)], 1u);
    }
  }
  __syncthreads();
  for (int i = threadIdx.x; i < kSelBins; i += NT) {
    const unsigned int v = lh[i];
    if (v) atomicAdd(&hist[(size_t)e * kSelBins + i], v);
  }
}

__global__ __launch_bounds__(NT) void select_pick_kernel(int E, const int* __restrict__ count, unsigned int* __restrict__ hist, long long kbq,
                                                         double* __restrict__ lohi) {
  __shared__ int wave_tot[NT / 64];
  __shared__ int sh_pick[2];
  const int e = blockIdx.x;
  const int cnt = count[e];
  if (cnt <= 0) {
    if (threadIdx.x == 0) { lohi[2 * e] = 0.0; lohi[2 * e + 1] = 0.0; }
    return;
  }
  unsigned int* hp = hist + (size_t)e * kSelBins;
  int bin; unsigned int below;
  pick_bin<kSelBins / NT>([&](int i) { return hp[i]; }, (unsigned int)(cnt / 2), wave_tot, sh_pick, bin, below);
#pragma unroll
  for (int i = 0; i < kSelBins / NT; ++i) hp[threadIdx.x * (kSelBins / NT) + i] = 0u;
  if (threadIdx.x == 0) {
    const long long q = kbq - (long long)(kSelBins - 1 - bin);
    const unsigned long long low_mask = (1ull << kSelShift) - 1ull;
    unsigned long long lo = 0ull, hi = 0ull;
    if (bin == kSelBins - 1) { lo = (unsigned long long)(kbq > 0 ? kbq : 0) << kSelShift; hi = 0x7FFFFFFFFFFFFFFFull; }
// ... 67 lines not shown

__global__ __launch_bounds__(NT) void bracket_final_kernel(int E, const int* __restrict__ count, const long long* __restrict__ cap_off,
                                                           const double* __restrict__ keys1, unsigned int* __restrict__ cnt_lt,
                                                           unsigned int* __restrict__ cnt_mid, double* __restrict__ median,
                                                           double* __restrict__ host_res, double* __restrict__ a_dev, double* __restrict__ a_host, double armed) {
  __shared__ unsigned int lh[kSelBins];
  __shared__ int wave_tot[NT / 64];
  __shared__ int sh_pick[2];
  const int e = blockIdx.x;
  const int cnt = count[e];
  double med = 0.0;
  bool ok = true;
  if (cnt > 0) {
    const unsigned int k = (unsigned int)(cnt / 2), nlt = cnt_lt[e], nmid = cnt_mid[e];
    ok = nlt <= k && k < nlt + nmid;
    if (ok) {
      unsigned long long prefix = 0ull;
      unsigned int rank = k - nlt;
      const long long base = cap_off[e];
      constexpr int KR = 8;
      const bool in_regs = nmid <= (unsigned int)(KR * NT);
      unsigned long long kreg[KR];
#pragma unroll
      for (int i = 0; i < KR; ++i) {
        const unsigned int pos = threadIdx.x + i * NT;
        kreg[i] = (in_regs && pos < nmid) ? (unsigned long long)__double_as_longlong(keys1[base + pos]) : ~0ull;
      }
      int hi_bit = 63;
#pragma unroll 1
      for (int pass = 0; pass < 6; ++pass) {
        const int bits = pass < 3 ? 11 : 10;
        const int shift = hi_bit - bits;
        for (int i = threadIdx.x; i < kSelBins; i += NT) lh[i] = 0u;
        __syncthreads();
        if (in_regs) {
#pragma unroll
          for (int i = 0; i < KR; ++i) {
            const unsigned long long key = kreg[i];
            if ((key >> hi_bit) == (prefix >> hi_bit)) atomicAdd(&lh[(key >> shift) & ((1ull << bits) - 1ull)], 1u);
          }
        } else {
          for (unsigned int pos = threadIdx.x; pos < nmid; pos += NT) {
            const unsigned long long key = (unsigned long long)__double_as_longlong(keys1[base + pos]);
            if ((key >> hi_bit) == (prefix >> hi_bit)) atomicAdd(&lh[(key >> shift) & ((1ull << bits) - 1ull)], 1u);
          }
        }
        __syncthreads();
        int bin; unsigned int below;
        pick_bin<kSelBins / NT>([&](int i) { return lh[i]; }, rank, wave_tot, sh_pick, bin, below);
        prefix |= (unsigned long long)bin << shift;
        rank -= below;
        hi_bit = shift;
      }
      med = __longlong_as_double((long long)prefix);
    }
  }
  if (threadIdx.x == 0) {
    if (ok) median[e] = med;
    host_res[2 * e] = (double)(cnt > 0 ? cnt : 0);
    host_res[2 * e + 1] = ok ? med : -1.0;
    if (e == 0) host_res[2 * E] = armed;
    write_a_scale(ok ? cnt : 0, med, e, a_dev, a_host);
  }
  __syncthreads();
  if (threadIdx.x == 0) { cnt_lt[e] = 0u; cnt_mid[e] = 0u; }
}

}

int launch_compact(mvicp_ctx* c, double d2_bound) {
  if (c->n_cblocks == 0) return MVICP_OK;
  double bytes = 0;
  for (int e = 0; e < c->E; ++e) if (c->owned[e]) bytes += 2.0 * 12.0 * c->frames[c->esrc[e]].n;
  ProfScope ps(c, "compact", bytes);
  hipLaunchKernelGGL(count_kernel, dim3(c->n_cblocks), dim3(NT), 0, c->stream, c->d_cblock_off, c->E, c->d_nsrc, c->d_cap_off, c->d_nn_idx,
                     c->d_nn_d2, d2_bound, c->d_cblock_cnt, c->d_dirty);
  hipLaunchKernelGGL(scan_kernel, dim3(c->E), dim3(NT), 0, c->stream, c->d_cblock_off, c->d_cblock_cnt, c->d_count, c->d_dirty);
  hipLaunchKernelGGL(scatter_kernel, dim3(c->n_cblocks), dim3(NT), 0, c->stream, c->d_cblock_off, c->E, c->d_nsrc, c->d_cap_off, c->d_nn_idx,
                     c->d_nn_d2, d2_bound, c->d_cblock_cnt, c->d_first, c->d_second, c->d_cd2, c->d_qpos, c->d_dirty);
  MV_HIP(hipGetLastError());
  return MVICP_OK;
}

int launch_gather_stream(mvicp_ctx* c) {
  if (c->n_cblocks == 0) return MVICP_OK;
  std::vector<const void*> tab(3 * (size_t)c->E, nullptr);
  for (int e = 0; e < c->E; ++e) {
    tab[e] = c->frames[c->esrc[e]].grid.srec;
    tab[c->E + e] = c->frames[c->edst[e]].grid.srec;
    tab[2 * c->E + e] = c->frames[c->edst[e]].grid.snor;
  }
  const void** d_tab = nullptr;
  MV_CHECK(cached_upload(c, "gather_tab", tab.data(), sizeof(void*) * tab.size(), (void**)&d_tab));
  {
    ProfScope ps(c, "gather", 0.0);
    hipLaunchKernelGGL(gather_kernel, dim3(c->n_cblocks), dim3(NT), 0, c->stream, c->d_cblock_off, c->E, c->d_count, c->d_cap_off, c->total_cap,
                       c->d_first, c->d_second, (const PointRec* const*)d_tab, (const PointRec* const*)(d_tab + c->E), (const double* const*)(d_tab + 2 * c->E), c->d_stream, c->d_dirty);
  }
  MV_HIP(hipGetLastError());
  return MVICP_OK;
}

static int select_scratch(mvicp_ctx* c, unsigned int** cnt_lt, unsigned int** cnt_mid, unsigned int** hist) {
  const size_t E = (size_t)c->E;
  *cnt_lt = c->d_sel_hist; *cnt_mid = *cnt_lt + E; *hist = *cnt_mid + E;
  if (!c->sel_scratch_clean) {
    MV_HIP(hipMemsetAsync(c->d_sel_hist, 0, sizeof(unsigned int) * E * (kSelBins + 2), c->stream));
    c->sel_scratch_clean = true;
  }
  return MVICP_OK;
}

static void launch_bracket_final(mvicp_ctx* c, unsigned int* cnt_lt, unsigned int* cnt_mid) {
  hipLaunchKernelGGL(bracket_final_kernel, dim3(c->E), dim3(NT), 0, c->stream, c->E, c->d_count, c->d_cap_off, c->d_sel_keys1, cnt_lt,
                     cnt_mid, c->d_median, c->d_res_target ? c->d_res_target : c->d_res_host, c->spec_arm ? c->d_a : (double*)nullptr,
                     c->spec_arm ? c->d_a_check : (double*)nullptr, c->spec_arm ? 1.0 : 0.0);
}

int launch_select_bracket(mvicp_ctx* c) {
  if (c->E == 0) return MVICP_OK;
  double bytes = 0;
  for (int e = 0; e < c->E; ++e) if (c->owned[e]) bytes += 8.0 * c->h_count[e];
  ProfScope ps(c, "select", bytes);
  unsigned int *cnt_lt, *cnt_mid, *hist;
  MV_CHECK(select_scratch(c, &cnt_lt, &cnt_mid, &hist));
  if (c->n_sblocks)
    hipLaunchKernelGGL(bracket_pass_kernel, dim3(c->n_sblocks), dim3(NT), 0, c->stream, c->d_sblock_off, c->E, c->d_count, c->d_cap_off, c->d_cd2,
                       (const double*)c->d_sel_lohi, cnt_lt, c->d_sel_keys1, cnt_mid);
  launch_bracket_final(c, cnt_lt, cnt_mid);
  MV_HIP(hipGetLastError());
  return MVICP_OK;
}

int launch_select_median(mvicp_ctx* c, double d2_bound) {
  if (c->E == 0) return MVICP_OK;
  double bytes = 0;
  for (int e = 0; e < c->E; ++e) if (c->owned[e]) bytes += 16.0 * c->h_count[e];
  ProfScope ps(c, "select", bytes);
  unsigned int *cnt_lt, *cnt_mid, *hist;
  MV_CHECK(select_scratch(c, &cnt_lt, &cnt_mid, &hist));
  if (c->n_sblocks) {
    long long kb;
    std::memcpy(&kb, &d2_bound, sizeof(kb));
    const long long kbq = kb > 0 ? kb >> kSelShift : 0;
    const dim3 grid(c->n_sblocks), blk(NT);
    hipLaunchKernelGGL(select_hist_kernel, grid, blk, 0, c->stream, c->d_sblock_off, c->E, c->d_count, c->d_cap_off, c->d_cd2, kbq, hist);
    hipLaunchKernelGGL(select_pick_kernel, dim3(c->E), blk, 0, c->stream, c->E, c->d_count, hist, kbq, c->d_sel_lohi);
    hipLaunchKernelGGL(bracket_pass_kernel, grid, blk, 0, c->stream, c->d_sblock_off, c->E, c->d_count, c->d_cap_off, c->d_cd2,
                       (const double*)c->d_sel_lohi, cnt_lt, c->d_sel_keys1, cnt_mid);
  }
  launch_bracket_final(c, cnt_lt, cnt_mid);
  MV_HIP(hipGetLastError());
  return MVICP_OK;
}

}
```

mv-lm-icp_amd/csrc/lin_common.h:

```cpp
#pragma once
#include "common.h"

namespace mvicp {

namespace {

constexpr int NT = kLinThreads;
constexpr int NB = MVICP_EDGE_BLOCK;
constexpr int NACC = kLinPartial;

__device__ __forceinline__ double half_rho(double s, double w) {
  const double d = 1.0 + w;
  double r = __builtin_amdgcn_rcp(d);
  r = __builtin_fma(__builtin_fma(-d, r, 1.0), r, r);
  r = __builtin_fma(__builtin_fma(-d, r, 1.0), r, r);
  return (s * w) * r;
}

__device__ __forceinline__ double fast_rsqrt(double y) {
  double r = __builtin_amdgcn_rsq(y);
  r = r * (1.5 - 0.5 * y * r * r);
  r = r * (1.5 - 0.5 * y * r * r);
  return r;
}

template <int NP> struct PairArgs {};
template <> struct PairArgs<2> { const double* rel2; size_t partials2_off; double* out2; };

__device__ __forceinline__ void cross_mat(const double* a, double* M) {
  M[0] = 0; M[1] = -a[2]; M[2] = a[1];
  M[3] = a[2]; M[4] = 0; M[5] = -a[0];
  M[6] = -a[1]; M[7] = a[0]; M[8] = 0;
}

template <bool PLANE, int NP>
__global__ __launch_bounds__(256) void reduce_expand_kernel(const int* __restrict__ chunk_first, int chunk, const int* __restrict__ count,
                                                           const double* __restrict__ rel, const double* __restrict__ partials,
                                                           double* __restrict__ out, PairArgs<NP> x) {
  if constexpr (NP > 1) {
    if (blockIdx.y) { rel = x.rel2; partials += x.partials2_off; out = x.out2; }
  }
  const int e = blockIdx.x;
  const int tid = threadIdx.x;
  __shared__ double m[8][NACC];
  __shared__ double S[36], X[36], Y[36], R6[36], Lm[36], T1[36], T2[36], T3[36], H[144], v[6];
  const int c0 = chunk_first[e];
  const int nchunks = min(chunk_first[e + 1] - c0, (count[e] + chunk - 1) / chunk);
  {
    const int val = tid & (NACC - 1), part = tid >> 5;
    double s = 0.0;
    for (int c = part; c < nchunks; c += 8) s += partials[(size_t)(c0 + c) * NACC + val];
    m[part][val] = s;
  }
  if (tid < 36) { S[tid] = 0.0; X[tid] = 0.0; Y[tid] = 0.0; R6[tid] = 0.0; Lm[tid] = (tid / 6 == tid % 6) ? 1.0 : 0.0; }
  __syncthreads();
  if (tid < NACC) {
    double s = m[0][tid];
#pragma unroll
    for (int k = 1; k < 8; ++k) s += m[k][tid];
    m[0][tid] = s;
  }
  __syncthreads();
  const double* mm = m[0];
  const double* A = rel + (size_t)e * kEdgeRel;
  const double* t = A + 9;
  if (tid < 9) {
    const int i = tid / 3, j = tid % 3;
    double tx[9];
    cross_mat(t, tx);
    const double a = A[i + 3 * j];
    R6[i * 6 + j] = a;
    R6[(3 + i) * 6 + 3 + j] = a;
    Lm[(3 + i) * 6 + j] = tx[i * 3 + j];
    if (PLANE) {
      if (tid < 6) v[tid] = mm[21 + tid];
    } else {
      const double w = mm[0];
      const double px[3] = {mm[1], mm[2], mm[3]};
      const double P[9] = {mm[4], mm[5], mm[6], mm[5], mm[7], mm[8], mm[6], mm[8], mm[9]};
      const double rr[3] = {mm[10], mm[11], mm[12]};
      const double PR[9] = {mm[13], mm[14], mm[15], mm[16], mm[17], mm[18], mm[19], mm[20], mm[21]};
      const double RR[9] = {mm[22], mm[23], mm[24], mm[23], mm[25], mm[26], mm[24], mm[26], mm[27]};
      double pxm[9], rxm[9];
      cross_mat(px, pxm);
      cross_mat(rr, rxm);
      const double trP = P[0] + P[4] + P[8], trRR = RR[0] + RR[4] + RR[8], trPR = PR[0] + PR[4] + PR[8];
      const double I = i == j ? 1.0 : 0.0;
      S[i * 6 + j] = w * I;
      S[i * 6 + 3 + j] = -pxm[i * 3 + j];
      S[(3 + i) * 6 + j] = pxm[i * 3 + j];
      S[(3 + i) * 6 + 3 + j] = trP * I - P[i * 3 + j];
      X[i * 6 + 3 + j] = -rxm[i * 3 + j];
      X[(3 + i) * 6 + 3 + j] = -(PR[j * 3 + i] - trPR * I);
      Y[(3 + i) * 6 + 3 + j] = trRR * I - RR[i * 3 + j];
      if (tid == 0) {
        v[0] = rr[0]; v[1] = rr[1]; v[2] = rr[2];
        v[3] = PR[1 * 3 + 2] - PR[2 * 3 + 1];
        v[4] = PR[2 * 3 + 0] - PR[0 * 3 + 2];
        v[5] = PR[0 * 3 + 1] - PR[1 * 3 + 0];
      }
    }
  }
  if (PLANE && tid >= 16 && tid < 16 + 21) {
    const int k = tid - 16;
    int i = 0, o = k;
    while (o >= 6 - i) { o -= 6 - i; ++i; }
    const int j = i + o;
    S[i * 6 + j] = mm[k];
    S[j * 6 + i] = mm[k];
  }
  __syncthreads();
  if (tid < 36) {
    const int i = tid / 6, j = tid % 6;
    double s = 0.0;
#pragma unroll
    for (int k = 0; k < 6; ++k) s += S[i * 6 + k] * R6[k * 6 + j];
    T1[tid] = s;
    T2[tid] = S[tid] - X[tid];
    T3[tid] = S[tid] - X[tid] - X[j * 6 + i] + Y[tid];
  }
  __syncthreads();
  double zl = 0.0, dl = 0.0;
  if (tid < 36) {
    const int i = tid / 6, j = tid % 6;
#pragma unroll
    for (int k = 0; k < 6; ++k) { zl += T2[i * 6 + k] * Lm[j * 6 + k]; dl += T3[i * 6 + k] * Lm[j * 6 + k]; }
  }
  __syncthreads();
  if (tid < 36) { T2[tid] = zl; T3[tid] = dl; }
  __syncthreads();
  double* o = out + (size_t)e * NB;
  if (tid < 36) {
    const int i = tid / 6, j = tid % 6;
    double hss = 0.0, hsd = 0.0, hdd = 0.0;
#pragma unroll
    for (int k = 0; k < 6; ++k) { hss += R6[k * 6 + i] * T1[k * 6 + j]; hsd += R6[k * 6 + i] * T2[k * 6 + j]; hdd += Lm[i * 6 + k] * T3[k * 6 + j]; }
    H[i * 12 + j] = hss;
    H[i * 12 + 6 + j] = -hsd;
    H[(6 + i) * 12 + 6 + j] = hdd;
  } else if (tid < 42) {
    const int i = tid - 36;
    double s = 0.0, l = 0.0;
#pragma unroll
    for (int k = 0; k < 6; ++k) { s += R6[k * 6 + i] * v[k]; l += Lm[i * 6 + k] * v[k]; }
    o[78 + i] = s;
    o[84 + i] = -l;
  } else if (tid == 42) {
    o[90] = count[e] > 0 ? mm[PLANE ? 27 : 28] : 0.0;
  }
  __syncthreads();
  for (int k = tid; k < 78; k += 256) {
    int i = 0, r = k;
    while (r >= 12 - i) { r -= 12 - i; ++i; }
// ... 19 lines not shown
```

mv-lm-icp_amd/csrc/linearize.hip:

```cpp
#include "lin_common.h"

namespace mvicp {

namespace {

template <bool PLANE, bool ROBUST>
__device__ __forceinline__ void accumulate(double (&acc)[NACC], const double* __restrict__ A, const double* __restrict__ t, double inv_a2,
                                           double p0, double p1, double p2, double q0, double q1, double q2, double n0, double n1, double n2) {
  const double x0 = __builtin_fma(A[6], p2, __builtin_fma(A[3], p1, A[0] * p0));
  const double x1 = __builtin_fma(A[7], p2, __builtin_fma(A[4], p1, A[1] * p0));
  const double x2 = __builtin_fma(A[8], p2, __builtin_fma(A[5], p1, A[2] * p0));
  if (PLANE) {
    const double nt_c = __builtin_fma(n2, t[2], __builtin_fma(n1, t[1], __builtin_fma(n0, t[0], -q0)));
    const double r = __builtin_fma(n2, x2, __builtin_fma(n1, x1, n0 * x0)) + nt_c;
    double u[6];
    u[0] = n0; u[1] = n1; u[2] = n2;
    u[3] = x1 * n2 - x2 * n1; u[4] = x2 * n0 - x0 * n2; u[5] = x0 * n1 - x1 * n0;
    const double s = r * r;
    double w = 1.0;
    if (ROBUST) {
      const double y = 1.0 + s * inv_a2;
      w = fast_rsqrt(y);
      acc[27] += half_rho(s, w);
    } else {
      acc[27] += 0.5 * s;
    }
    int o = 0;
#pragma unroll
    for (int i = 0; i < 6; ++i) {
      const double wu = w * u[i];
#pragma unroll
      for (int j = i; j < 6; ++j) { acc[o] = __builtin_fma(wu, u[j], acc[o]); ++o; }
      acc[21 + i] = __builtin_fma(wu, r, acc[21 + i]);
    }
  } else {
    const double f0 = (x0 + t[0]) - q0, f1 = (x1 + t[1]) - q1, f2 = (x2 + t[2]) - q2;
    const double s = f0 * f0 + f1 * f1 + f2 * f2;
    double w = 1.0;
    if (ROBUST) {
      const double y = 1.0 + s * inv_a2;
      w = fast_rsqrt(y);
      acc[28] += half_rho(s, w);
    } else {
      acc[28] += 0.5 * s;
    }
    const double wx0 = w * x0, wx1 = w * x1, wx2 = w * x2;
    const double wf0 = w * f0, wf1 = w * f1, wf2 = w * f2;
    acc[0] += w;
    acc[1] += wx0; acc[2] += wx1; acc[3] += wx2;
    acc[4] += wx0 * x0; acc[5] += wx0 * x1; acc[6] += wx0 * x2; acc[7] += wx1 * x1; acc[8] += wx1 * x2; acc[9] += wx2 * x2;
    acc[10] += wf0; acc[11] += wf1; acc[12] += wf2;
    acc[13] += wx0 * f0; acc[14] += wx0 * f1; acc[15] += wx0 * f2;
    acc[16] += wx1 * f0; acc[17] += wx1 * f1; acc[18] += wx1 * f2;
    acc[19] += wx2 * f0; acc[20] += wx2 * f1; acc[21] += wx2 * f2;
    acc[22] += wf0 * f0; acc[23] += wf0 * f1; acc[24] += wf0 * f2; acc[25] += wf1 * f1; acc[26] += wf1 * f2; acc[27] += wf2 * f2;
  }
}

template <bool PLANE, bool ROBUST, int NP>
__global__ __launch_bounds__(NT) void linearize_kernel(const int* __restrict__ chunk_edge, const int* __restrict__ chunk_start, int chunk,
                                                       const int* __restrict__ count, const long long* __restrict__ cap_off, long long total_cap,
                                                       const double* __restrict__ rel, const double* __restrict__ a_scale,
                                                       const double* __restrict__ stream, double* __restrict__ partials,
                                                       const double* const* __restrict__ src_pts, const int* __restrict__ nsrc,
                                                       const int* __restrict__ chunk_first, PairArgs<NP> x) {
  const int e = chunk_edge[blockIdx.x];
  const int start = chunk_start[blockIdx.x];
  const int c = chunk_first[e] + start / chunk;
  const int cnt = count[e];
  if (start >= cnt) return;
  const int end = min(cnt, start + chunk);
  __shared__ double srel[NP][kEdgeRel];
  __shared__ double red[NACC / 2][NT + 1];
  if (threadIdx.x < kEdgeRel) srel[0][threadIdx.x] = rel[(size_t)e * kEdgeRel + threadIdx.x];
  if constexpr (NP > 1) { if (threadIdx.x >= 32 && threadIdx.x < 32 + kEdgeRel) srel[1][threadIdx.x - 32] = x.rel2[(size_t)e * kEdgeRel + threadIdx.x - 32]; }
  __syncthreads();
  double A[NP][9], t[NP][3];
#pragma unroll
  for (int k = 0; k < NP; ++k) {
#pragma unroll
    for (int i = 0; i < 9; ++i) A[k][i] = srel[k][i];
#pragma unroll
    for (int i = 0; i < 3; ++i) t[k][i] = srel[k][9 + i];
  }
  double inv_a2 = 1.0;
  if (ROBUST) { const double a = a_scale[e]; inv_a2 = 1.0 / (a * a); }

  double acc[NP][NACC];
#pragma unroll
  for (int k = 0; k < NP; ++k)
#pragma unroll
    for (int i = 0; i < NACC; ++i) acc[k][i] = 0.0;

  const size_t base = (size_t)cap_off[e];
  const double* __restrict__ s0 = stream + base;
  constexpr int NS = PLANE ? 7 : 6;
  auto arr = [](int j) { return PLANE ? j : (j < 3 ? j : j + 4); };
  int pos = start + 2 * threadIdx.x;
  double2 cur[9], nxt[9];
#pragma unroll
  for (int j = 0; j < 9; ++j) { cur[j] = make_double2(0.0, 0.0); nxt[j] = make_double2(0.0, 0.0); }
  const double* __restrict__ sp = (src_pts != nullptr && cnt == nsrc[e]) ? src_pts[e] : nullptr;
  auto load = [&](double2 (&v)[9], int at) {
    if (at + 1 < end) {
      if (sp != nullptr) {
        const double2 a = *reinterpret_cast<const double2*>(sp + 3 * (size_t)at);
        const double2 b = *reinterpret_cast<const double2*>(sp + 3 * (size_t)at + 2);
        const double2 c2 = *reinterpret_cast<const double2*>(sp + 3 * (size_t)at + 4);
        v[0] = make_double2(a.x, b.y); v[1] = make_double2(a.y, c2.x); v[2] = make_double2(b.x, c2.y);
      }
#pragma unroll
      for (int j = 0; j < NS; ++j) {
        if (j < 3 && sp != nullptr) continue;
        typedef double d2v __attribute__((ext_vector_type(2)));
        const d2v t = __builtin_nontemporal_load(reinterpret_cast<const d2v*>(s0 + (size_t)arr(j) * total_cap + at));
        v[j] = make_double2(t.x, t.y);
      }
    } else if (at < end) {
#pragma unroll
      for (int j = 0; j < NS; ++j) { v[j].x = (j < 3 && sp != nullptr) ? sp[3 * (size_t)at + j] : s0[(size_t)arr(j) * total_cap + at]; v[j].y = 0.0; }
    }
  };
  load(cur, pos);
  while (pos < end) {
    const int npos = pos + 2 * NT;
    load(nxt, npos);
#define MVICP_LIN_STEP(k)                                                                                                                                   \
    if (PLANE) {                                                                                                                                            \
      accumulate<PLANE, ROBUST>(acc[k], A[k], t[k], inv_a2, cur[0].x, cur[1].x, cur[2].x, cur[6].x, 0.0, 0.0, cur[3].x, cur[4].x, cur[5].x);             \
      if (pos + 1 < end)                                                                                                                                    \
        accumulate<PLANE, ROBUST>(acc[k], A[k], t[k], inv_a2, cur[0].y, cur[1].y, cur[2].y, cur[6].y, 0.0, 0.0, cur[3].y, cur[4].y, cur[5].y);           \
    } else {                                                                                                                                                \
      accumulate<PLANE, ROBUST>(acc[k], A[k], t[k], inv_a2, cur[0].x, cur[1].x, cur[2].x, cur[3].x, cur[4].x, cur[5].x, 0.0, 0.0, 0.0);                  \
      if (pos + 1 < end)                                                                                                                                    \
        accumulate<PLANE, ROBUST>(acc[k], A[k], t[k], inv_a2, cur[0].y, cur[1].y, cur[2].y, cur[3].y, cur[4].y, cur[5].y, 0.0, 0.0, 0.0);                \
    }
    MVICP_LIN_STEP(0)
    if constexpr (NP > 1) { MVICP_LIN_STEP(NP - 1) }
#undef MVICP_LIN_STEP
#pragma unroll
    for (int j = 0; j < 9; ++j) cur[j] = nxt[j];
    pos = npos;
  }

#pragma unroll
  for (int k = 0; k < NP; ++k) {
    double* __restrict__ pk = partials;
    if constexpr (NP > 1) { if (k) pk = partials + x.partials2_off; }
#pragma unroll
    for (int pass = 0; pass < 2; ++pass) {
      if (pass || k) __syncthreads();
#pragma unroll
      for (int j = 0; j < NACC / 2; ++j) red[j][threadIdx.x] = acc[k][pass * (NACC / 2) + j];
      __syncthreads();
      const int row = threadIdx.x >> 4, part = threadIdx.x & 15;
      double sum = 0.0;
#pragma unroll 8
      for (int i = 0; i < NT / 16; ++i) sum += red[row][part + 16 * i];
      sum += __shfl_xor(sum, 1, 64);
      sum += __shfl_xor(sum, 2, 64);
      sum += __shfl_xor(sum, 4, 64);
      sum += __shfl_xor(sum, 8, 64);
      if (part == 0) pk[(size_t)c * NACC + pass * (NACC / 2) + row] = sum;
    }
  }
}

}

static double stream_pass_bytes(mvicp_ctx* c, int plane) {
  double bytes = 0;
  std::vector<char> src_counted((size_t)c->n_frames, 0);
  for (int e = 0; e < c->E; ++e) {
    if (!c->owned[e]) continue;
    const double cnt = c->h_count[e];
    const int s = c->esrc[e];
    bytes += (plane ? 32.0 : 24.0) * cnt;
    if (c->lin_share_p && c->lin_interleave && c->h_count[e] == c->frames[s].n) { if (!src_counted[s]) { bytes += 24.0 * cnt; src_counted[s] = 1; } }
    else bytes += 24.0 * cnt;
  }
  return bytes;
}

int launch_linearize(mvicp_ctx* c, int plane, int robust) {
  if (c->E == 0) return MVICP_OK;
  const int chunk = c->lin_chunk;
  if (c->n_chunks > 0) {
    const double bytes = stream_pass_bytes(c, plane);
    const double* const* d_src = nullptr;
    MV_CHECK(source_table(c, &d_src));
    ProfScope ps(c, "linearize", bytes);
#define LAUNCH(P, R)                                                                                                                           \
  hipLaunchKernelGGL((linearize_kernel<P, R, 1>), dim3(c->n_chunks), dim3(NT), 0, c->stream, c->d_chunk_edge, c->d_chunk_start, chunk, c->d_count, \
                     c->d_cap_off, c->total_cap, c->d_rel, c->d_a, c->d_stream, c->d_partials, d_src, (const int*)c->d_nsrc, (const int*)c->d_chunk_first, PairArgs<1>{})
    if (plane && robust) LAUNCH(true, true);
    else if (plane) LAUNCH(true, false);
    else if (robust) LAUNCH(false, true);
    else LAUNCH(false, false);
#undef LAUNCH
  }
  {
    ProfScope ps(c, "reduce", 0.0);
    if (plane)
      hipLaunchKernelGGL((reduce_expand_kernel<true, 1>), dim3(c->E), dim3(256), 0, c->stream, c->d_chunk_first, chunk, c->d_count, c->d_rel, c->d_partials, c->lin_out ? c->lin_out : c->d_out, PairArgs<1>{});
    else
      hipLaunchKernelGGL((reduce_expand_kernel<false, 1>), dim3(c->E), dim3(256), 0, c->stream, c->d_chunk_first, chunk, c->d_count, c->d_rel, c->d_partials, c->lin_out ? c->lin_out : c->d_out, PairArgs<1>{});
  }
  MV_HIP(hipGetLastError());
  return MVICP_OK;
}

int launch_linearize_pair(mvicp_ctx* c, int plane, int robust, double* out_a, double* out_b) {
  if (c->E == 0) return MVICP_OK;
  const int chunk = c->lin_chunk;
  PairArgs<2> x;
  x.rel2 = c->d_rel2; x.partials2_off = (size_t)c->n_chunks * kLinPartial; x.out2 = out_b;
  if (c->n_chunks > 0) {
    const double bytes = stream_pass_bytes(c, plane);
    const double* const* d_src = nullptr;
    MV_CHECK(source_table(c, &d_src));
    ProfScope ps(c, "linearize_pair", bytes);
#define LAUNCH(P, R)                                                                                                                              \
  hipLaunchKernelGGL((linearize_kernel<P, R, 2>), dim3(c->n_chunks), dim3(NT), 0, c->stream, c->d_chunk_edge, c->d_chunk_start, chunk, c->d_count, \
                     c->d_cap_off, c->total_cap, c->d_rel, c->d_a, c->d_stream, c->d_partials, d_src, (const int*)c->d_nsrc, (const int*)c->d_chunk_first, x)
    if (plane && robust) LAUNCH(true, true);
    else if (plane) LAUNCH(true, false);
    else if (robust) LAUNCH(false, true);
    else LAUNCH(false, false);
#undef LAUNCH
  }
  {
    ProfScope ps(c, "reduce", 0.0);
    if (plane)
      hipLaunchKernelGGL((reduce_expand_kernel<true, 2>), dim3(c->E, 2), dim3(256), 0, c->stream, c->d_chunk_first, chunk, c->d_count, c->d_rel, c->d_partials, out_a, x);
    else
      hipLaunchKernelGGL((reduce_expand_kernel<false, 2>), dim3(c->E, 2), dim3(256), 0, c->stream, c->d_chunk_first, chunk, c->d_count, c->d_rel, c->d_partials, out_a, x);
  }
  MV_HIP(hipGetLastError());
  return MVICP_OK;
}

}
```

mv-lm-icp_amd/csrc/nn_grid.hip:

```cpp
#include <algorithm>
#include <atomic>
#include <cmath>
#include <cstring>
#include <limits>
#include <numeric>
#include <system_error>
#include <thread>
#include <unordered_set>

#include "build_common.h"
#include "common.h"
#include "nn_cache.h"
#include "nn_census.h"
#include "nn_list.h"
#include "nn_metric.h"
#include "nn_tie.h"

namespace mvicp {

namespace {

#ifndef MVICP_GRID_THREADS
#define MVICP_GRID_THREADS 256
#endif
constexpr int NT = MVICP_GRID_THREADS;
constexpr unsigned long long EMPTY = ~0ull;

struct GridView {
  const double* spts; const int* sidx; const PointRec* srec; int n;
  const PointRec* crec;
  const HashEntry* table; unsigned int mask; int shift;
  double ox, oy, oz, h, inv_h;
  int dx, dy, dz;
  const float* oct; int oct_leaf; long long oct_first_leaf;
  const BrickEntry* bricks; const uint2* celltab; int bx, by, bz;
};

struct GridJob {
  GridView dst;
  const double* q; const int* qidx;
  const double* xf;
  int n;
  int* out_idx; double* out_d2;
  const int* inv;
  ListRef list;
  float* out_lb;
  int seed;
  TieRef tie;
};

__device__ __forceinline__ unsigned long long __reduce_add_u64(unsigned long long v) {
  unsigned long long total = 0;
  unsigned long long mask = __ballot(1);
  while (mask) {
    const int l = __ffsll((long long)mask) - 1;
    total += __shfl(v, l, 64);
    mask &= mask - 1;
  }
  return total;
}
__device__ __forceinline__ bool __lane0() {
  const unsigned long long mask = __ballot(1);
  return (int)(threadIdx.x & 63) == __ffsll((long long)mask) - 1;
}

__global__ void dirty_reduce_kernel(int E, const int* __restrict__ slot_off, int* __restrict__ slots, int* __restrict__ dirty) {
  const int e = blockIdx.x;
  int any = 0;
  for (int k = slot_off[e] + threadIdx.x; k < slot_off[e + 1]; k += blockDim.x) {
    const int v = slots[k];
    if (v) { any = 1; slots[k] = 0; }
  }
  if (__syncthreads_or(any) && threadIdx.x == 0) dirty[e] = 1;
}

template <bool TREE_ONLY>
__global__ __launch_bounds__(NT) void nn_grid_kernel(const GridJob* __restrict__ jobs, double bound, double search, unsigned long long* __restrict__ stats, int skip_far,
                                                     int2* __restrict__ far_list, unsigned int* __restrict__ far_count, double prune_rho) {
  __shared__ double sxf[kEdgeXf];
  __shared__ uint2 s_rng[8][NT];
  const GridJob& job = jobs[blockIdx.y];
  const int i = blockIdx.x * NT + threadIdx.x;
  if (blockIdx.x * NT >= job.n) return;
  const bool has_xf = job.xf != nullptr;
  if (has_xf && threadIdx.x < kEdgeXf) sxf[threadIdx.x] = job.xf[threadIdx.x];
  __syncthreads();
  if (i >= job.n) return;
  const GridView& g = job.dst;

  double qx, qy, qz;
  {
    const double p0 = job.q[3 * (size_t)i], p1 = job.q[3 * (size_t)i + 1], p2 = job.q[3 * (size_t)i + 2];
    if (has_xf) xf_point(sxf, p0, p1, p2, qx, qy, qz);
    else { qx = p0; qy = p1; qz = p2; }
  }
  const int out = i;

  double best = search;
  int bi = 0x7fffffff;
  bool resolved = false;
  unsigned int n_cand = 0;
  double second = 1.7976931348623157e308;

  const double slack = has_xf ? sxf[kXfCache] : -1.0;
  double rp2 = -1.0;
  if (!TREE_ONLY && job.seed) {
    const int pi = job.out_idx[out];
    if (pi < 0 && job.out_lb != nullptr && cache_still_none(slack, job.out_lb, out)) {
      if (stats) {
        unsigned long long c1 = __reduce_add_u64(1ull);
        const size_t slot = ((size_t)blockIdx.y * gridDim.x + blockIdx.x) * (NT / 64) + (threadIdx.x >> 6);
        if (__lane0()) atomicAdd(&stats[8 * slot + 3], c1);
      }
      return;
    }
    if (pi >= 0 && pi < g.n) {
      const double* tp = g.spts + 3 * (size_t)pi;
      const double d = dist2(qx, qy, qz, tp[0], tp[1], tp[2]);
      if (slack >= 0.0 && job.out_lb != nullptr) {
        const double p0 = job.q[3 * (size_t)i], p1 = job.q[3 * (size_t)i + 1], p2 = job.q[3 * (size_t)i + 2];
        const double eps = cache_eps(sxf, p0, p1, p2);
        const float lb_old = job.out_lb[out];
        if (cache_hit(eps, lb_old, d, bound, true, false)) {
          cache_refresh(job, out, pi, d, eps, lb_old, bound);
          if (stats) {
            unsigned long long c1 = __reduce_add_u64(1ull);
            const size_t slot = ((size_t)blockIdx.y * gridDim.x + blockIdx.x) * (NT / 64) + (threadIdx.x >> 6);
            if (__lane0()) atomicAdd(&stats[8 * slot + 3], c1);
          }
          return;
        }
      }
      if (prune_rho > 0.0) { const double rp = sqrt(d) + prune_rho * g.h; rp2 = rp * rp * 1.002; }
    }
  }

  double m2 = 0.0;
  double skipped = 1.7976931348623157e308;
  if (!TREE_ONLY) {
    const double cx = (qx - g.ox) * g.inv_h - 0.5, cy = (qy - g.oy) * g.inv_h - 0.5, cz = (qz - g.oz) * g.inv_h - 0.5;
    const double lim = 2.0e6;
    const int bx = (int)floor(fmin(fmax(cx, -lim), lim)), by = (int)floor(fmin(fmax(cy, -lim), lim)), bz = (int)floor(fmin(fmax(cz, -lim), lim));
    unsigned long long key[8];
    unsigned int slot[8];
    HashEntry ent[8];
    const double ax = qx - (g.ox + (bx + 1) * g.h), ay = qy - (g.oy + (by + 1) * g.h), az = qz - (g.oz + (bz + 1) * g.h);
    const double ax2 = ax * ax * 0.998, ay2 = ay * ay * 0.998, az2 = az * az * 0.998;
    const int home = (ax >= 0.0 ? 1 : 0) | (ay >= 0.0 ? 2 : 0) | (az >= 0.0 ? 4 : 0);
#pragma unroll
    for (int c = 0; c < 8; ++c) {
      const int ix = bx + (c & 1), iy = by + ((c >> 1) & 1), iz = bz + (c >> 2);
      bool in = !(ix < 0 || iy < 0 || iz < 0 || ix >= g.dx || iy >= g.dy || iz >= g.dz);
      if (rp2 >= 0.0) {
        const int df = c ^ home;
        const double lbc = ((df & 1) ? ax2 : 0.0) + ((df & 2) ? ay2 : 0.0) + ((df & 4) ? az2 : 0.0);
        if (lbc > rp2) { in = false; skipped = fmin(skipped, lbc); }
// ... 656 lines not shown
namespace {
GridView view_of(const FrameDev& f) {
  GridView v;
  const GridDev& g = f.grid;
  v.spts = g.spts; v.sidx = g.sidx; v.srec = (const PointRec*)g.srec; v.crec = (const PointRec*)g.crec; v.n = f.n;
  v.table = (const HashEntry*)g.table; v.mask = g.table_mask; v.shift = g.table_shift;
  v.ox = g.origin[0]; v.oy = g.origin[1]; v.oz = g.origin[2]; v.h = g.cell; v.inv_h = g.inv_cell;
  v.dx = g.dims[0]; v.dy = g.dims[1]; v.dz = g.dims[2];
  v.oct = g.oct; v.oct_leaf = g.oct_leaf; v.oct_first_leaf = g.oct_first_leaf;
  v.bricks = (const BrickEntry*)g.bricks; v.celltab = (const uint2*)g.celltab; v.bx = g.bdims[0]; v.by = g.bdims[1]; v.bz = g.bdims[2];
  return v;
}

int run(mvicp_ctx* c, std::vector<GridJob>& jobs, double bound, const FrameDev* const* dst_of) {
  if (jobs.empty()) return MVICP_OK;
  const double search = search_bound(c, bound);
  std::vector<TieJob> ties;
  if (!(c->tie_skip && jobs[0].list.dirty_slots != nullptr)) {
    double launch_q = 0;
    for (const GridJob& j : jobs) launch_q += j.n;
    const TieRef tref = tie_ref(c, (size_t)launch_q, 0u);
    for (size_t k = 0; k < jobs.size(); ++k) {
      GridJob& j = jobs[k];
      j.tie = tref; j.tie.job = (unsigned int)k;
      TieJob t;
      std::memset(&t, 0, sizeof(t));
      tie_job_fill(*dst_of[k], t);
      t.q = j.q; t.xf = j.xf; t.n = j.n; t.out_idx = j.out_idx; t.out_d2 = j.out_d2; t.inv = j.inv; t.list = j.list;
      ties.push_back(t);
    }
  }
  int max_n = 0;
  double nq = 0;
  for (const GridJob& j : jobs) { max_n = std::max(max_n, j.n); nq += j.n; }
  if (max_n == 0) return MVICP_OK;
  GridJob* d_jobs = nullptr;
  MV_CHECK(cached_upload(c, jobs[0].xf ? "grid_jobs" : "grid_jobs_raw", jobs.data(), sizeof(GridJob) * jobs.size(), (void**)&d_jobs));
  unsigned long long* d_stats = nullptr;
  const size_t slots = (size_t)((max_n + NT - 1) / NT) * jobs.size() * (NT / 64);
  MV_CHECK(census_scratch(c, slots, &d_stats));
  const size_t total_q = (size_t)nq;
  if (total_q > c->far_cap) {
    if (c->d_far_list) MV_HIP(hipFree(c->d_far_list));
    MV_HIP(hipMalloc((void**)&c->d_far_list, sizeof(int2) * total_q));
    c->far_cap = total_q;
  }
  const bool edge_path = jobs[0].list.dirty_slots != nullptr;
  if (!c->d_far_count) {
    MV_HIP(hipMalloc((void**)&c->d_far_count, 2 * sizeof(unsigned int)));
    MV_HIP(hipMemsetAsync(c->d_far_count, 0, 2 * sizeof(unsigned int), c->stream));
    c->far_parity = 0;
  }
  unsigned int* far_cnt = c->d_far_count + c->far_parity;
  unsigned int* far_next = c->d_far_count + (c->far_parity ^ 1);
  c->far_parity ^= 1;
  bool use_cell = false;
  const dim3 grid((max_n + NT - 1) / NT, (unsigned)jobs.size());
  {
    ProfScope ps(c, "nn_grid", 36.0 * nq);
    use_cell = c->nn_cell && !c->nn_tree_only && !c->nn_skip_far && edge_path;
    for (const GridJob& j : jobs) if (j.dst.bricks == nullptr || j.xf == nullptr) use_cell = false;
    if (c->nn_tree_only)
      hipLaunchKernelGGL((nn_grid_kernel<true>), grid, dim3(NT), 0, c->stream, d_jobs, bound, search, d_stats, 0, (int2*)c->d_far_list, far_cnt, 0.0);
    else if (use_cell)
      hipLaunchKernelGGL(nn_cell_kernel, grid, dim3(NT), 0, c->stream, d_jobs, bound, search, d_stats, (int2*)c->d_far_list, far_cnt, c->prune_rho);
    else
      hipLaunchKernelGGL((nn_grid_kernel<false>), grid, dim3(NT), 0, c->stream, d_jobs, bound, search, d_stats, c->nn_skip_far ? 1 : 0, (int2*)c->d_far_list, far_cnt,
                         c->prune_rho);
  }
  const bool launch_far = !(edge_path && c->far_skip), launch_dirty = edge_path && !c->skip_dirty_reduce;
  if (launch_far || launch_dirty) {
    ProfScope ps(c, "nn_far", 0.0);
    const size_t far_wide = (edge_path && c->far_narrow) ? 128 : 256 * 8;
    const unsigned int far_blocks = (unsigned int)std::min<size_t>(far_wide, (total_q * 8 + NT - 1) / NT);
    if (!c->h_far_seen) {
      MV_HIP(hipHostMalloc((void**)&c->h_far_seen, sizeof(unsigned int), hipHostMallocMapped));
      *c->h_far_seen = 1u;
      MV_HIP(hipHostGetDevicePointer((void**)&c->d_far_seen, c->h_far_seen, 0));
    }
    if (launch_far)
      hipLaunchKernelGGL(nn_far_kernel, dim3(far_blocks), dim3(NT), 0, c->stream, d_jobs, (const int2*)c->d_far_list, bound, (const unsigned int*)far_cnt, far_next, d_stats, slots,
                         edge_path ? c->d_far_seen : nullptr);
    if (launch_dirty)
      hipLaunchKernelGGL(dirty_reduce_kernel, dim3(c->E), dim3(256), 0, c->stream, c->E, c->d_dslot_off, c->d_dirty_slots, c->d_dirty);
  }
  MV_HIP(hipGetLastError());
  if (d_stats) MV_CHECK(census_collect(c, d_stats, slots, nq, c->nn_tree_only ? 1 : (use_cell ? 3 : 0), "nn_grid"));
  MV_CHECK(launch_tie_fixup(c, ties, bound));
  return MVICP_OK;
}
}

int launch_dirty_reduce(mvicp_ctx* c) {
  hipLaunchKernelGGL(dirty_reduce_kernel, dim3(c->E), dim3(256), 0, c->stream, c->E, c->d_dslot_off, c->d_dirty_slots, c->d_dirty);
  MV_HIP(hipGetLastError());
  return MVICP_OK;
}

namespace { __global__ void grid_warm_kernel() {} }

int warm_nn_grid(mvicp_ctx* c) {
  if (!c->d_far_count) {
    MV_HIP(hipMalloc((void**)&c->d_far_count, 2 * sizeof(unsigned int)));
    MV_HIP(hipMemsetAsync(c->d_far_count, 0, 2 * sizeof(unsigned int), c->stream));
    c->far_parity = 0;
  }
  hipLaunchKernelGGL(grid_warm_kernel, dim3(1), dim3(64), 0, c->stream);
  MV_HIP(hipGetLastError());
  return MVICP_OK;
}

int launch_nn_grid_edges(mvicp_ctx* c, double d2_bound) {
  std::vector<GridJob> jobs;
  std::vector<const FrameDev*> dsts;
  for (int e = 0; e < c->E; ++e) {
    if (!c->active[e]) continue;
    const FrameDev& s = c->frames[c->esrc[e]];
    const FrameDev& d = c->frames[c->edst[e]];
    if (!s.has_grid || !d.has_grid) { set_error("grid NN needs the per-cloud structure on frames %d and %d", c->esrc[e], c->edst[e]); return MVICP_ERR_STATE; }
    GridJob j;
    std::memset(&j, 0, sizeof(j));
    j.dst = view_of(d);
    j.q = s.grid.spts; j.qidx = nullptr; j.xf = c->d_xf + (size_t)e * kEdgeXf; j.n = s.n;
    j.out_idx = c->d_nn_idx + c->cap_off[e]; j.out_d2 = c->d_nn_d2 + c->cap_off[e];
    j.inv = d.grid.inv; j.out_lb = c->d_nn_lb + c->cap_off[e];
    j.list = ListRef{c->d_qpos + c->cap_off[e], c->d_second + c->cap_off[e], c->d_cd2 + c->cap_off[e], c->d_dirty + e, c->d_dirty_slots + c->dslot_off[e],
                     c->d_stream + c->cap_off[e], c->total_cap, d.grid.snor, (const PointRec*)d.grid.srec};
    j.seed = ((int)c->nn_cache_edge.size() == c->E && c->nn_cache_edge[e]) ? 1 : 0;
    jobs.push_back(j); dsts.push_back(&d);
  }
  return run(c, jobs, d2_bound, dsts.data());
}

int launch_nn_grid_queries(mvicp_ctx* c, const FrameDev& f, const double* d_q, int n, int* d_idx, double* d_d2) {
  if (!f.has_grid) { set_error("grid NN structure missing"); return MVICP_ERR_STATE; }
  std::vector<GridJob> jobs(1);
  std::memset(&jobs[0], 0, sizeof(GridJob));
  jobs[0].dst = view_of(f);
  jobs[0].q = d_q; jobs[0].qidx = nullptr; jobs[0].xf = nullptr; jobs[0].n = n;
  jobs[0].out_idx = d_idx; jobs[0].out_d2 = d_d2;
  jobs[0].inv = nullptr; jobs[0].out_lb = nullptr;
  const FrameDev* dst = &f;
  return run(c, jobs, 1.7976931348623157e308, &dst);
}

}
```

mv-lm-icp_amd/csrc/nn_list.h:

```cpp
#pragma once
#include "common.h"

namespace mvicp {

struct ListRef {
  const int* qpos; int* second; double* cd2; const int* dirty; int* dirty_slots;
  double* stream; long long total_cap; const double* dst_nor;
  const PointRec* dst_srec;
};

__device__ __forceinline__ void update_list_entry(const ListRef& R, int i, int idx_new, double d2_new, double bound, bool same_neighbour) {
  if (*R.dirty != 0) return;
  const int pos = R.qpos[i];
  const bool acc = idx_new >= 0 && d2_new < bound;
  bool clean;
  if (pos < 0) clean = !acc;
  else {
    clean = acc;
    if (clean) {
      if (!same_neighbour && R.second[pos] != idx_new) {
        R.second[pos] = idx_new;
        const double2* pb = reinterpret_cast<const double2*>(R.dst_srec + idx_new);
        const double2 b0 = pb[0], b1 = pb[1];
        double* st = R.stream + pos;
        st[7 * R.total_cap] = b0.x; st[8 * R.total_cap] = b0.y; st[9 * R.total_cap] = b1.x;
        if (R.dst_nor != nullptr) {
          const double n0 = R.dst_nor[3 * (size_t)idx_new], n1 = R.dst_nor[3 * (size_t)idx_new + 1], n2 = R.dst_nor[3 * (size_t)idx_new + 2];
          st[3 * R.total_cap] = n0; st[4 * R.total_cap] = n1; st[5 * R.total_cap] = n2;
          st[6 * R.total_cap] = n0 * b0.x + n1 * b0.y + n2 * b1.x;
        }
      }
      R.cd2[pos] = d2_new;
    }
  }
  if (!clean) R.dirty_slots[i / 256] = 1;
}

int launch_dirty_reduce(mvicp_ctx* c);

}
```

mv-lm-icp_amd/csrc/nn_tie.hip:

```cpp
#include <algorithm>
#include <thread>

#include "kdvisit.h"
#include "nn_metric.h"
#include "nn_tie.h"
#include "tie_walk.h"

namespace mvicp {

namespace {

constexpr int TIE_STACK = 128;
constexpr int TIE_DEEP_LANES = 1024;
constexpr int TIE_MAX_LEVELS = 16384;

template <bool DEEP>
__device__ __forceinline__ void tie_pass(const TieJob* __restrict__ jobs, int n_jobs, const unsigned long long* __restrict__ list, unsigned int reported,
                                         unsigned int cap, double bound, unsigned int* __restrict__ seen, TiePending* __restrict__ st, int st_cap) {
  const bool everything = reported > cap;
  const long long total = everything ? jobs[n_jobs - 1].q_begin + jobs[n_jobs - 1].n : (long long)reported;
  for (long long t = (long long)blockIdx.x * blockDim.x + threadIdx.x; t < total; t += (long long)gridDim.x * blockDim.x) {
    int jb, i;
    if (everything) {
      int lo = 0, hi = n_jobs - 1;
      while (lo < hi) { const int mid = (lo + hi + 1) >> 1; if (jobs[mid].q_begin <= t) lo = mid; else hi = mid - 1; }
      jb = lo; i = (int)(t - jobs[lo].q_begin);
    } else {
      const unsigned long long e = list[t];
      jb = (int)(e >> 32); i = (int)(e & 0xffffffffull);
    }
    const TieJob& J = jobs[jb];
    if (i >= J.n) continue;
    if (J.nodes == nullptr) { if (!DEEP) seen[1] = 1u; continue; }
    if ((J.levels > TIE_STACK) != DEEP) continue;
    const int cur = J.out_idx[i];
    if (cur < 0) continue;
    double qx, qy, qz;
    {
      const double p0 = J.q[3 * (size_t)i], p1 = J.q[3 * (size_t)i + 1], p2 = J.q[3 * (size_t)i + 2];
      if (J.xf != nullptr) xf_point(J.xf, p0, p1, p2, qx, qy, qz);
      else { qx = p0; qy = p1; qz = p2; }
    }
    double d2 = 0.0;
    const TieTree T{static_cast<const VisitNode*>(J.nodes), J.ord, J.tpts, J.box};
    const int bi = tie_walk(T, qx, qy, qz, st, st_cap, &d2);
    if (bi == TIE_WALK_TRUNCATED) { seen[2] = 1u; continue; }
    if (bi < 0 || d2 != J.out_d2[i]) continue;
    const int pos = J.inv ? J.inv[bi] : bi;
    if (pos != cur) {
      J.out_idx[i] = pos;
      if (J.list.dirty) update_list_entry(J.list, i, pos, d2, bound, false);
    }
  }
}

__global__ __launch_bounds__(64) void nn_tie_kernel(const TieJob* __restrict__ jobs, int n_jobs, const unsigned long long* __restrict__ list,
                                                    const unsigned int* __restrict__ count, unsigned int* __restrict__ next_count, unsigned int cap,
                                                    double bound, unsigned int* __restrict__ seen) {
  const unsigned int reported = *count;
  if (blockIdx.x == 0 && threadIdx.x == 0) { *next_count = 0u; *seen = reported; }
  if (reported == 0u) return;
  TiePending st[TIE_STACK];
  tie_pass<false>(jobs, n_jobs, list, reported, cap, bound, seen, st, TIE_STACK);
}

__global__ __launch_bounds__(64) void nn_tie_deep_kernel(const TieJob* __restrict__ jobs, int n_jobs, const unsigned long long* __restrict__ list,
                                                         const unsigned int* __restrict__ count, unsigned int cap, double bound,
                                                         unsigned int* __restrict__ seen, TiePending* __restrict__ deep_st, int deep_cap) {
  const unsigned int reported = *count;
  if (reported == 0u) return;
  TiePending* st = deep_st + (size_t)(blockIdx.x * blockDim.x + threadIdx.x) * (size_t)deep_cap;
  tie_pass<true>(jobs, n_jobs, list, reported, cap, bound, seen, st, deep_cap);
}

}

void free_tie(FrameDev& f) {
  if (f.tie_nodes) (void)hipFree(f.tie_nodes);
  if (f.tie_ord) (void)hipFree(f.tie_ord);
  if (f.tie_slot) (void)hipFree(f.tie_slot);
  f.tie_nodes = nullptr; f.tie_ord = nullptr; f.tie_slot = nullptr; f.has_tie = false; f.tie_levels = 0;
}

int ensure_tie_trees(mvicp_ctx* c, const std::vector<int>& frames) {
  std::vector<int> todo;
  for (int f : frames)
    if (f >= 0 && f < c->n_frames && !c->frames[f].has_tie && c->frames[f].n > 0 && std::find(todo.begin(), todo.end(), f) == todo.end()) todo.push_back(f);
  if (todo.empty()) return MVICP_OK;
  struct Built { std::vector<double> xyz; std::vector<VisitNode> nodes; std::vector<int> slot, ord; double box[6]; int levels; };
  std::vector<Built> B(todo.size());
  for (size_t k = 0; k < todo.size(); ++k) {
    const FrameDev& F = c->frames[todo[k]];
    B[k].xyz.resize(3 * (size_t)F.n);
    MV_HIP(hipMemcpy(B[k].xyz.data(), F.pts, sizeof(double) * 3 * (size_t)F.n, hipMemcpyDeviceToHost));
  }
  auto work = [&](size_t k) {
    Built& b = B[k];
    const int n = (int)(b.xyz.size() / 3);
    b.levels = build_visit_tree(b.xyz.data(), n, b.nodes, b.slot);
    b.ord.assign(n, 0);
    for (int i = 0; i < n; ++i) b.ord[b.slot[i]] = i;
    for (int a = 0; a < 3; ++a) b.box[a] = b.box[3 + a] = b.xyz[a];
    for (int i = 1; i < n; ++i)
      for (int a = 0; a < 3; ++a) { const double v = b.xyz[3 * (size_t)i + a]; if (v < b.box[a]) b.box[a] = v; if (v > b.box[3 + a]) b.box[3 + a] = v; }
  };
  const unsigned int nthreads = std::max(1u, std::min<unsigned int>({(unsigned int)todo.size(), std::thread::hardware_concurrency(), 16u}));
  if (nthreads <= 1) { for (size_t k = 0; k < todo.size(); ++k) work(k); }
  else {
    std::vector<std::thread> pool;
    for (unsigned int t = 0; t < nthreads; ++t) pool.emplace_back([&, t]() { for (size_t k = t; k < todo.size(); k += nthreads) work(k); });
    for (auto& th : pool) th.join();
  }
  for (size_t k = 0; k < todo.size(); ++k)
    if (B[k].levels > TIE_MAX_LEVELS) {
      set_error("frame %d: its nanoflann-equivalent tree has %d levels, the tie fix-up walks at most %d (tie_rule = 0 searches such a cloud with the lowest-index rule)",
                todo[k], B[k].levels, TIE_MAX_LEVELS);
      return MVICP_ERR_ARG;
    }
  for (size_t k = 0; k < todo.size(); ++k) {
    FrameDev& F = c->frames[todo[k]];
    auto upload = [&]() -> int {
      MV_HIP(hipMalloc(&F.tie_nodes, sizeof(VisitNode) * B[k].nodes.size()));
      MV_HIP(hipMemcpy(F.tie_nodes, B[k].nodes.data(), sizeof(VisitNode) * B[k].nodes.size(), hipMemcpyHostToDevice));
      MV_HIP(hipMalloc((void**)&F.tie_ord, sizeof(int) * B[k].ord.size()));
      MV_HIP(hipMemcpy(F.tie_ord, B[k].ord.data(), sizeof(int) * B[k].ord.size(), hipMemcpyHostToDevice));
      MV_HIP(hipMalloc((void**)&F.tie_slot, sizeof(int) * B[k].slot.size()));
      MV_HIP(hipMemcpy(F.tie_slot, B[k].slot.data(), sizeof(int) * B[k].slot.size(), hipMemcpyHostToDevice));
      return MVICP_OK;
    };
    const int st = upload();
    if (st != MVICP_OK) { free_tie(F); return st; }
    for (int a = 0; a < 6; ++a) F.tie_box[a] = B[k].box[a];
    F.tie_levels = B[k].levels;
    F.has_tie = true;
// ... 70 lines not shown
```

mv-lm-icp_amd/csrc/nn_tile_common.h:

```cpp
#pragma once
#include <algorithm>
#include <cmath>
#include <cstring>
#include <limits>
#include <vector>

#include "common.h"
#include "nn_cache.h"
#include "nn_census.h"
#include "nn_list.h"
#include "nn_metric.h"
#include "nn_tie.h"

namespace mvicp {

namespace {

constexpr int NT = 256;
#ifndef MVICP_TILE_LEAF
#define MVICP_TILE_LEAF 32
#endif
constexpr int LEAF = MVICP_TILE_LEAF;
constexpr int FAN = 64;

// ... 142 lines not shown
  const int lane = threadIdx.x & 63;
  const float inf = __int_as_float(0x7f800000);
  float b0 = inf, b1 = inf, b2 = inf, b3 = -inf, b4 = -inf, b5 = -inf;
  if (lane < nchild) {
    const float* base = g.wide + g.off[LEVEL] + first + lane;
    const long long st = g.cnt[LEVEL];
    b0 = base[0]; b1 = base[st]; b2 = base[2 * st]; b3 = base[3 * st]; b4 = base[4 * st]; b5 = base[5 * st];
  }
  return NodeBoxes{b0, b1, b2, b3, b4, b5};
}

__device__ __forceinline__ void node_cull(const PatchBox& G, const NodeBoxes& B, float& ddf, float& key) {
  const float e0 = fmaxf(fmaxf(B.b0 - G.hi[0], G.lo[0] - B.b3), 0.f);
  const float e1 = fmaxf(fmaxf(B.b1 - G.hi[1], G.lo[1] - B.b4), 0.f);
  const float e2 = fmaxf(fmaxf(B.b2 - G.hi[2], G.lo[2] - B.b5), 0.f);
  ddf = (e0 * e0 + e1 * e1 + e2 * e2) * 0.999999f;
  const float k0 = fmaxf(fmaxf(B.b0 - G.c[0], G.c[0] - B.b3), 0.f);
  const float k1 = fmaxf(fmaxf(B.b1 - G.c[1], G.c[1] - B.b4), 0.f);
  const float k2 = fmaxf(fmaxf(B.b2 - G.c[2], G.c[2] - B.b5), 0.f);
  key = k0 * k0 + k1 * k1 + k2 * k2;
}

__device__ __forceinline__ void node_park(float2* __restrict__ mybox, const NodeBoxes& B) {
  const int lane = threadIdx.x & 63;
  __builtin_amdgcn_wave_barrier();
  mybox[lane] = make_float2(B.b0, B.b3);
  mybox[FAN + lane] = make_float2(B.b1, B.b4);
  mybox[2 * FAN + lane] = make_float2(B.b2, B.b5);
  __builtin_amdgcn_fence(__ATOMIC_RELEASE, "wavefront");
  __builtin_amdgcn_wave_barrier();
  __builtin_amdgcn_fence(__ATOMIC_ACQUIRE, "wavefront");
}

template <bool IN_LDS>
__device__ __forceinline__ NodeBoxes node_child(const float2* __restrict__ mybox, const NodeBoxes& B, int c) {
  if (IN_LDS) {
    const float2 u = mybox[c], v = mybox[FAN + c], w = mybox[2 * FAN + c];
    return NodeBoxes{u.x, v.x, w.x, u.y, v.y, w.y};
  }
  return NodeBoxes{bcast(B.b0, c), bcast(B.b1, c), bcast(B.b2, c), bcast(B.b3, c), bcast(B.b4, c), bcast(B.b5, c)};
}

template <bool BND, bool BY_INDEX>
__device__ __forceinline__ void store_result(const TileJob& job, int i, int key, double best, double second, bool tie, float mu, double bound) {
  constexpr int NONE = BY_INDEX ? 0x7fffffff : -1;
  job.out_idx[i] = key == NONE ? -1 : (BY_INDEX && job.inv ? job.inv[key] : key);
  job.out_d2[i] = best;
  if (BND) job.out_lb[i] = key == NONE ? -1.f : __double2float_rd(fmin(sqrt(second), sqrt(best) + (double)mu) * (1.0 - 1e-9));
  if (job.list.dirty) update_list_entry(job.list, i, key == NONE ? -1 : (BY_INDEX ? job.inv[key] : key), best, bound, false);
  if ((BND ? second == best : tie) && key != NONE) tie_report(job.tie, (unsigned int)i);
}
TileView view_of(const FrameDev& f) {
  TileView v;
  v.spts = f.grid.spts; v.sidx = f.grid.sidx; v.n = f.n;
  v.wide = f.grid.wide; v.levels = f.grid.wide_levels;
  for (int l = 0; l < 6; ++l) { v.cnt[l] = f.grid.wide_cnt[l]; v.off[l] = f.grid.wide_off[l]; }
  v.maxabs = f.grid.maxabs;
  v.srec = (const PointRec*)f.grid.srec;
  v.mf_ops = (const uint4*)f.grid.mf_ops; v.mf_blk = (const MfBlock*)f.grid.mf_blk;
  return v;
}

inline int build_tile_jobs(mvicp_ctx* c, bool with_bounds, bool with_cache, bool with_list, std::vector<TileJob>& jobs, int& max_n, double& nq, std::vector<TieJob>& ties) {
  max_n = 0; nq = 0;
  double launch_q = 0;
  for (int e = 0; e < c->E; ++e) if (c->active[e]) launch_q += c->frames[c->esrc[e]].n;
  const TieRef tref = tie_ref(c, (size_t)launch_q, 0u);
  for (int e = 0; e < c->E; ++e) {
    if (!c->active[e]) continue;
    const FrameDev& s = c->frames[c->esrc[e]];
    const FrameDev& d = c->frames[c->edst[e]];
    if (!s.has_grid || !d.has_grid) { set_error("tile NN needs the per-cloud structure on frames %d and %d", c->esrc[e], c->edst[e]); return MVICP_ERR_STATE; }
    TileJob j;
    std::memset(&j, 0, sizeof(j));
    j.dst = view_of(d);
    j.q = s.grid.spts; j.qidx = nullptr; j.xf = c->d_xf + (size_t)e * kEdgeXf; j.n = s.n;
    j.out_idx = c->d_nn_idx + c->cap_off[e]; j.out_d2 = c->d_nn_d2 + c->cap_off[e];
    j.inv = d.grid.inv;
    j.seed = (c->tile_seed && (int)c->nn_cache_edge.size() == c->E && c->nn_cache_edge[e]) ? 1 : 0;
    if (with_bounds) { j.out_lb = c->d_nn_lb + c->cap_off[e]; j.mu = (float)(c->tile_mu * d.grid.cell); }
    if (with_bounds && with_cache) { j.cache = 1; j.miss_max = c->tile_miss; j.reject_cache = c->reject_cache ? 1 : 0; }
    if (with_list) {
      j.list = ListRef{c->d_qpos + c->cap_off[e], c->d_second + c->cap_off[e], c->d_cd2 + c->cap_off[e], c->d_dirty + e, c->d_dirty_slots + c->dslot_off[e],
                       c->d_stream + c->cap_off[e], c->total_cap, d.grid.snor, (const PointRec*)d.grid.srec};
    }
    j.kacc = (float)c->mfma_kacc; j.trig = c->mfma_trig;
    j.tie = tref; j.tie.job = (unsigned int)jobs.size();
    {
      TieJob t;
      std::memset(&t, 0, sizeof(t));
      tie_job_fill(d, t);
      t.q = j.q; t.xf = j.xf; t.n = j.n; t.out_idx = j.out_idx; t.out_d2 = j.out_d2; t.inv = j.inv; t.list = j.list;
      ties.push_back(t);
    }
    jobs.push_back(j);
    max_n = std::max(max_n, s.n);
    nq += s.n;
  }
  return MVICP_OK;
}

template <typename Launch>
inline int launch_tile_search(mvicp_ctx* c, double d2_bound, bool with_bounds, bool with_cache, bool with_list, int wg, const char* scope, Launch launch) {
  std::vector<TileJob> jobs;
  int max_n = 0;
  double nq = 0;
  std::vector<TieJob> ties;
  MV_CHECK(build_tile_jobs(c, with_bounds, with_cache, with_list, jobs, max_n, nq, ties));
  if (jobs.empty() || max_n == 0) return MVICP_OK;
  TileJob* d_jobs = nullptr;
  MV_CHECK(cached_upload(c, jobs[0].xf ? "tile_jobs" : "tile_jobs_raw", jobs.data(), sizeof(TileJob) * jobs.size(), (void**)&d_jobs));
  unsigned long long* d_stats = nullptr;
  const size_t slots = (size_t)((max_n + wg - 1) / wg) * jobs.size() * (wg / 64);
  MV_CHECK(census_scratch(c, slots, &d_stats));
  {
    ProfScope ps(c, scope, 36.0 * nq);
    const dim3 grid((max_n + wg - 1) / wg, (unsigned)jobs.size());
    int top = jobs[0].dst.levels - 1;
    for (const TileJob& j : jobs) if (j.dst.levels - 1 != top) top = -1;
    launch(jobs, d_jobs, grid, top, d_stats);
  }
  MV_HIP(hipGetLastError());
  MV_CHECK(launch_tie_fixup(c, ties, d2_bound));
  if (with_list) MV_CHECK(launch_dirty_reduce(c));
  if (d_stats) MV_CHECK(census_collect(c, d_stats, slots, nq, 2, scope));
  return MVICP_OK;
}

}

}
```

Baseline: 1178 iterations/s.

## Presume identity list for invalid edges, add fused compact and mapped rel staging

Edges whose correspondence list is invalid but whose cache flag is negative are now presumed clean: NN kernels write list entries in place at identity positions and the dirty-reduce kernel sets count to the full source size, skipping the compact+gather pass when nothing is rejected. It also adds an optional fused compact+gather kernel, optional zero-copy mapped relative-pose input for linearization, and hoists per-edge rotation loads in the linearize kernel. The presumption is on by default and introduces a new code path whose correctness depends on the dirty-slot fallback. The fused compaction and mapped-rel paths are off by default.

```diff
diff --git a/mv-lm-icp_amd/csrc/api.cpp b/mv-lm-icp_amd/csrc/api.cpp
--- a/mv-lm-icp_amd/csrc/api.cpp
+++ b/mv-lm-icp_amd/csrc/api.cpp
@@ -141,7 +141,7 @@
 
 void free_graph(mvicp_ctx* c) {
   dev_free(c->d_esrc); dev_free(c->d_edst); dev_free(c->d_cap_off); dev_free(c->d_count);
-  dev_free(c->d_ctl); c->d_nsrc = nullptr; c->d_a = nullptr; c->d_xf = nullptr; c->d_rel = nullptr; c->d_rel2 = nullptr; c->d_dirty = nullptr;
+  dev_free(c->d_ctl); c->d_nsrc = nullptr; c->d_a = nullptr; c->d_xf = nullptr; c->d_rel = nullptr; c->d_rel2 = nullptr; c->d_dirty = nullptr; c->d_presume = nullptr;
   dev_free(c->d_nn_idx); dev_free(c->d_nn_d2); dev_free(c->d_nn_lb); dev_free(c->d_first); dev_free(c->d_second);
   dev_free(c->d_sblock_off); dev_free(c->d_sel_keys1); c->n_sblocks = 0;
   dev_free(c->d_cd2); dev_free(c->d_qpos); dev_free(c->d_dirty_slots); dev_free(c->d_dslot_off); dev_free(c->d_stream); dev_free(c->d_cblock_off); dev_free(c->d_cblock_cnt);
@@ -436,6 +436,19 @@
   return metric == MVICP_METRIC_SYMMETRIC ? launch_linearize_sym(c, robust) : launch_linearize(c, metric, robust);
 }
 
+struct MappedRel {
+  mvicp_ctx* c; bool in_flight = false;
+  ~MappedRel() { c->lin_rel = nullptr; if (in_flight) (void)hipStreamSynchronize(c->stream); }
+};
+static int stage_rel(mvicp_ctx* c, const double* poses, int metric, MappedRel& m) {
+  if (metric == MVICP_METRIC_SYMMETRIC) return upload_rel_sym(c, poses);
+  if (!c->rel_mapped || c->d_rel_host == nullptr) return upload_rel(c, poses);
+  fill_rel(c, poses);
+  c->lin_rel = c->d_rel_host;
+  m.in_flight = true;
+  return MVICP_OK;
+}
+
 int evaluate_blocks(mvicp_ctx* c, const double* poses, int plane, int robust, double* out) {
   MV_CHECK(check_evaluable(c, plane));
   HostScope hs(c, "host.evaluate");
@@ -462,11 +475,13 @@
   }
   c->last_cand_poses.assign(poses, poses + 16 * (size_t)c->n_frames); c->last_cand_plane = plane; c->last_cand_robust = robust;
   double* h = c->h_pin + c->pin_blocks_off;
+  MappedRel mapped{c};
   if (c->comm || c->ar_fn) {
     c->lin_out = c->d_out;
-    int st_l = plane == MVICP_METRIC_SYMMETRIC ? upload_rel_sym(c, poses) : upload_rel(c, poses);
+    int st_l = stage_rel(c, poses, plane, mapped);
     if (st_l == MVICP_OK && c->fault_inject_eval > 0 && --c->fault_inject_eval == 0) { set_error("injected launch failure (option fault_inject_eval)"); st_l = MVICP_ERR_HIP; }
     if (st_l == MVICP_OK) st_l = launch_metric(c, plane, robust);
+    c->lin_rel = nullptr;
     char local_msg[sizeof(g_err)] = "";
     if (st_l != MVICP_OK) std::memcpy(local_msg, g_err, sizeof(local_msg));
     if (hipMemsetAsync(c->d_out + n, st_l == MVICP_OK ? 0 : 0xFF, sizeof(double), c->stream) != hipSuccess) {
@@ -477,6 +492,7 @@
     double* hx = c->h_pin + c->pin_spec_off;
     MV_HIP(hipMemcpyAsync(hx, c->d_out, sizeof(double) * (n + 1), hipMemcpyDeviceToHost, c->stream));
     MV_CHECK(stream_wait(c));
+    mapped.in_flight = false;
     if (std::isnan(hx[n])) {
       if (st_l != MVICP_OK) { set_error("%s", local_msg); return st_l; }
       set_error("a peer rank failed before the exchange of this evaluation (poisoned exchange buffer)");
@@ -485,11 +501,13 @@
     std::memcpy(out, hx, sizeof(double) * n);
     return MVICP_OK;
   } else {
-    MV_CHECK(plane == MVICP_METRIC_SYMMETRIC ? upload_rel_sym(c, poses) : upload_rel(c, poses));
+    MV_CHECK(stage_rel(c, poses, plane, mapped));
     c->lin_out = c->d_blocks_host;
     MV_CHECK(launch_metric(c, plane, robust));
+    c->lin_rel = nullptr;
   }
   MV_CHECK(stream_wait(c));
+  mapped.in_flight = false;
   std::memcpy(out, h, sizeof(double) * n);
   return MVICP_OK;
 }
@@ -1318,7 +1336,7 @@
   const size_t cap = (size_t)c->total_cap;
   MV_CHECK(dev_alloc(&c->d_esrc, E)); MV_CHECK(dev_alloc(&c->d_edst, E)); MV_CHECK(dev_alloc(&c->d_cap_off, E + 1));
   MV_CHECK(dev_alloc(&c->d_count, E));
-  c->ctl_r1 = (size_t)E * kEdgeXf + (size_t)E + 2 * (size_t)E;
+  c->ctl_r1 = (size_t)E * kEdgeXf + (size_t)E + 2 * (size_t)E + ((size_t)E + 1) / 2;
   c->ctl_rel2_off = (c->ctl_r1 + 1) & ~(size_t)1;
   c->ctl_r2_off = c->ctl_rel2_off + (size_t)E * kEdgeRel;
   c->ctl_r2 = (size_t)E * (kEdgeRel + 1);
@@ -1326,6 +1344,7 @@
   MV_HIP(hipMemset(c->d_ctl, 0, sizeof(double) * std::max<size_t>(c->ctl_r2_off + c->ctl_r2, 1)));
   c->d_xf = c->d_ctl; c->d_nsrc = reinterpret_cast<int*>(c->d_ctl + (size_t)E * kEdgeXf); c->d_dirty = c->d_nsrc + E;
   c->d_sel_lohi = c->d_ctl + (size_t)E * (kEdgeXf + 1);
+  c->d_presume = reinterpret_cast<int*>(c->d_ctl + (size_t)E * (kEdgeXf + 3));
   c->sel_med1.assign(E, -1.0); c->sel_med2.assign(E, -1.0);
   c->d_rel = c->d_ctl + c->ctl_r2_off; c->d_a = c->d_rel + (size_t)E * kEdgeRel; c->d_rel2 = c->d_ctl + c->ctl_rel2_off;
   MV_CHECK(dev_alloc(&c->d_nn_idx, cap)); MV_CHECK(dev_alloc(&c->d_nn_d2, cap)); MV_CHECK(dev_alloc(&c->d_nn_lb, cap));
@@ -1398,6 +1417,7 @@
     void* dp = nullptr;
     MV_HIP(hipHostGetDevicePointer(&dp, c->h_pin, 0));
     c->d_blocks_host = (double*)dp + c->pin_blocks_off;
+    c->d_rel_host = (double*)dp + c->ctl_r2_off;
     c->d_res_host = (double*)dp + c->pin_res_off;
     c->d_spec_host = (double*)dp + c->pin_spec_off;
     c->d_adev_host = (double*)dp + c->pin_adev_off;
@@ -1553,7 +1573,7 @@
   if (nn_method == MVICP_NN_AUTO && method == MVICP_NN_GRID && c->auto_last_method == MVICP_NN_TILE && c->tile_bounds >= 1 &&
       c->nn_cache_enable && !c->nn_cell) { method = MVICP_NN_TILE; tile_lb = true; handed_over = true; }
   if (method == MVICP_NN_TILE && c->tile_bounds >= 2 && c->nn_cache_enable) tile_lb = true;
-  bool tile_cached = false;
+  bool tile_cached = false, any_presumed = false;
   bool all_same = true;
   {
     for (int e = 0; e < E; ++e) if (c->active[e] && !same_edge[e]) all_same = false;
@@ -1562,10 +1582,18 @@
     if (method == MVICP_NN_TILE && !tile_cached && c->tile_cache >= 2 && tile_lb && c->nn_cache_valid && c->nn_cache_enable && !all_same) tile_cached = true;
   }
   {
-    std::vector<int> dirty(E, 1);
+    std::vector<int> dirty(E, 1), presume(E, 0);
     if ((method == MVICP_NN_TILE || (method == MVICP_NN_GRID && !c->nn_tree_only && !c->nn_skip_far)) && c->list_reuse)
-      for (int e = 0; e < E; ++e) if (c->active[e] && c->list_valid[e]) dirty[e] = 0;
+      for (int e = 0; e < E; ++e) {
+        if (!c->active[e]) continue;
+        if (c->list_valid[e]) dirty[e] = 0;
+        else if (c->list_presume && hx[(size_t)e * kEdgeXf + kXfCache] < 0.0) { dirty[e] = 0; presume[e] = 1; }
+      }
     std::memcpy(hd, dirty.data(), sizeof(int) * E);
+    std::memcpy(reinterpret_cast<int*>(hx + (size_t)E * (kEdgeXf + 3)), presume.data(), sizeof(int) * E);
+    int n_presumed = 0;
+    for (int e = 0; e < E; ++e) if (presume[e]) { any_presumed = true; ++n_presumed; }
+    if (c->profile && n_presumed) c->prof["list.presumed"].launches += n_presumed;
   }
   bool use_bracket = c->sel_bracket && c->have_corr;
   {
@@ -1581,6 +1609,7 @@
   bool nothing_can_change = method == MVICP_NN_GRID && c->list_reuse && !c->nn_tree_only && !c->nn_skip_far && same_active_set && !c->nn_cell;
   for (int e = 0; e < E && nothing_can_change; ++e)
     if (c->active[e] && !(same_edge[e] && hd[e] == 0)) nothing_can_change = false;
+  if (any_presumed) nothing_can_change = false;
   c->skip_dirty_reduce = nothing_can_change;
   c->tie_skip = nothing_can_change && c->corr_tie_seen == 0u;
   c->far_skip = nothing_can_change && c->corr_far_seen == 0u && c->prev_grid_kernel && method == MVICP_NN_GRID;
@@ -1638,8 +1667,11 @@
 
   mark("host.corr.nn_launch");
   if (!nothing_can_change) {
-    MV_CHECK(launch_compact(c, bound));
-    MV_CHECK(launch_gather_stream(c));
+    if (c->compact_fused) MV_CHECK(launch_compact_fused(c, bound));
+    else {
+      MV_CHECK(launch_compact(c, bound));
+      MV_CHECK(launch_gather_stream(c));
+    }
   }
   if (sel_skip) { c->h_pin[c->pin_res_off + 2 * (size_t)E] = c->spec_arm ? 1.0 : 0.0; return MVICP_OK; }
   return use_bracket ? launch_select_bracket(c) : launch_select_median(c, bound);
@@ -1988,6 +2020,9 @@
   if (std::strcmp(name, "nn_cache") == 0) { c->nn_cache_enable = value != 0.0; c->nn_cache_valid = false; return MVICP_OK; }
   if (std::strcmp(name, "lin_chunk") == 0) { c->lin_chunk_override = (int)value; return MVICP_OK; }
   if (std::strcmp(name, "list_reuse") == 0) { c->list_reuse = value != 0.0; return MVICP_OK; }
+  if (std::strcmp(name, "compact_fused") == 0) { c->compact_fused = value != 0.0; return MVICP_OK; }
+  if (std::strcmp(name, "rel_mapped") == 0) { c->rel_mapped = value != 0.0; return MVICP_OK; }
+  if (std::strcmp(name, "list_presume") == 0) { c->list_presume = value != 0.0; return MVICP_OK; }
   if (std::strcmp(name, "lin_interleave") == 0) { c->lin_interleave = value != 0.0; return MVICP_OK; }
   if (std::strcmp(name, "lin_share_p") == 0) { c->lin_share_p = value != 0.0; return MVICP_OK; }
   if (std::strcmp(name, "lin_pair") == 0) { c->lin_pair = value != 0.0; return MVICP_OK; }
diff --git a/mv-lm-icp_amd/csrc/common.h b/mv-lm-icp_amd/csrc/common.h
--- a/mv-lm-icp_amd/csrc/common.h
+++ b/mv-lm-icp_amd/csrc/common.h
@@ -223,6 +223,7 @@
   int* d_first = nullptr; int* d_second = nullptr; double* d_cd2 = nullptr;
   int* d_qpos = nullptr;
   int* d_dirty = nullptr;
+  int* d_presume = nullptr;
   int* d_dirty_slots = nullptr; int* d_dslot_off = nullptr; std::vector<int> dslot_off; int n_dslots = 0;
   std::vector<char> list_valid;
   std::vector<char> explicit_list;
@@ -265,6 +266,9 @@
   size_t pin_blocks_off = 0, pin_res_off = 0, pin_misc_off = 0;
   double* d_res_host = nullptr;
   double* d_blocks_host = nullptr;
+  double* d_rel_host = nullptr;
+  const double* lin_rel = nullptr;
+  bool rel_mapped = false;
   double* lin_out = nullptr;
   bool spec_enable = true; bool spec_flags_valid = false; int spec_param = 0, spec_plane = 0, spec_robust = 0;
   int spec_q_plane = 0, spec_q_robust = 0;
@@ -312,6 +316,8 @@
   std::atomic<int> fault_inject_build{0};
   int fault_inject = 0, fault_inject_eval = 0;
   bool list_reuse = true;
+  bool compact_fused = false;
+  bool list_presume = true;
   bool nn_tree_only = false;
   bool nn_census = false;
   void* d_census = nullptr; size_t census_bytes = 0;
@@ -393,6 +399,7 @@
 long long iss_keypoints(mvicp_ctx* c, const FrameDev& f, double B2_salient, double B2_nms, int q, double gamma21, double gamma32, int min_neighbors);
 int launch_compact(mvicp_ctx* c, double d2_bound);
 int launch_gather_stream(mvicp_ctx* c);
+int launch_compact_fused(mvicp_ctx* c, double d2_bound);
 int launch_select_median(mvicp_ctx* c, double d2_bound);
 int launch_export(mvicp_ctx* c);
 int launch_select_bracket(mvicp_ctx* c);
diff --git a/mv-lm-icp_amd/csrc/corr.hip b/mv-lm-icp_amd/csrc/corr.hip
--- a/mv-lm-icp_amd/csrc/corr.hip
+++ b/mv-lm-icp_amd/csrc/corr.hip
@@ -165,6 +165,77 @@
   }
 }
 
+__global__ __launch_bounds__(NT) void compact_fused_kernel(const int* __restrict__ cblock_off, int E, const int* __restrict__ nsrc,
+                                                           const long long* __restrict__ cap_off, long long total_cap, const int* __restrict__ nn_idx,
+                                                           const double* __restrict__ nn_d2, double bound, const int* __restrict__ cblock_cnt,
+                                                           int* __restrict__ first, int* __restrict__ second, double* __restrict__ cd2,
+                                                           int* __restrict__ qpos, const PointRec* const* __restrict__ src_rec,
+                                                           const PointRec* const* __restrict__ dst_rec, const double* const* __restrict__ dst_nor,
+                                                           double* __restrict__ stream, const int* __restrict__ dirty) {
+  __shared__ int wave_tot[NT / 64];
+  __shared__ int s_k[kCompactBlock], s_idx[kCompactBlock];
+  __shared__ double s_d2[kCompactBlock];
+  const int b = blockIdx.x;
+  const int e = find_edge(cblock_off, E, b);
+  if (dirty[e] == 0) return;
+  const int lb = b - cblock_off[e];
+  const int n = nsrc[e];
+  const long long base = cap_off[e];
+  int idx[IPT];
+  double d2[IPT];
+  bool ok[IPT];
+  int cnt = 0;
+#pragma unroll
+  for (int i = 0; i < IPT; ++i) {
+    const int k = lb * kCompactBlock + threadIdx.x * IPT + i;
+    ok[i] = false;
+    if (k < n) {
+      idx[i] = nn_idx[base + k];
+      d2[i] = nn_d2[base + k];
+      ok[i] = idx[i] >= 0 && d2[i] < bound;
+    }
+    cnt += ok[i] ? 1 : 0;
+  }
+  int total;
+  int lpos = block_exclusive_scan(cnt, wave_tot, &total);
+  const int pos0 = cblock_cnt[b];
+#pragma unroll
+  for (int i = 0; i < IPT; ++i) {
+    const int k = lb * kCompactBlock + threadIdx.x * IPT + i;
+    if (k < n) qpos[base + k] = ok[i] ? pos0 + lpos : -1;
+    if (!ok[i]) continue;
+    s_k[lpos] = k; s_idx[lpos] = idx[i]; s_d2[lpos] = d2[i];
+    ++lpos;
+  }
+  __syncthreads();
+  const PointRec* __restrict__ sp = src_rec[e];
+  const PointRec* __restrict__ dp = dst_rec[e];
+  const double* __restrict__ dn = dst_nor[e];
+  for (int j = threadIdx.x; j < total; j += NT) {
+    const int k = s_k[j];
+    const size_t s = (size_t)s_idx[j];
+    const size_t o = (size_t)(base + pos0 + j);
+    first[o] = k; second[o] = (int)s; cd2[o] = s_d2[j];
+    const double2* pa = reinterpret_cast<const double2*>(sp + k);
+    const double2 a0 = pa[0], a1 = pa[1];
+    const double2* pb = reinterpret_cast<const double2*>(dp + s);
+    const double2 b0 = pb[0], b1 = pb[1];
+    __builtin_nontemporal_store(a0.x, &stream[0 * total_cap + o]);
+    __builtin_nontemporal_store(a0.y, &stream[1 * total_cap + o]);
+    __builtin_nontemporal_store(a1.x, &stream[2 * total_cap + o]);
+    __builtin_nontemporal_store(b0.x, &stream[7 * total_cap + o]);
+    __builtin_nontemporal_store(b0.y, &stream[8 * total_cap + o]);
+    __builtin_nontemporal_store(b1.x, &stream[9 * total_cap + o]);
+    if (dn != nullptr) {
+      const double n0 = dn[3 * s], n1 = dn[3 * s + 1], n2 = dn[3 * s + 2];
+      __builtin_nontemporal_store(n0, &stream[3 * total_cap + o]);
+      __builtin_nontemporal_store(n1, &stream[4 * total_cap + o]);
+      __builtin_nontemporal_store(n2, &stream[5 * total_cap + o]);
+      __builtin_nontemporal_store(n0 * b0.x + n1 * b0.y + n2 * b1.x, &stream[6 * total_cap + o]);
+    }
+  }
+}
+
 constexpr int kSelBins = 2048;
 constexpr int kSelShift = 46;
 
@@ -398,16 +469,42 @@
   return MVICP_OK;
 }
 
-int launch_gather_stream(mvicp_ctx* c) {
-  if (c->n_cblocks == 0) return MVICP_OK;
+static int gather_table(mvicp_ctx* c, const void*** d_tab) {
   std::vector<const void*> tab(3 * (size_t)c->E, nullptr);
   for (int e = 0; e < c->E; ++e) {
     tab[e] = c->frames[c->esrc[e]].grid.srec;
     tab[c->E + e] = c->frames[c->edst[e]].grid.srec;
     tab[2 * c->E + e] = c->frames[c->edst[e]].grid.snor;
   }
+  return cached_upload(c, "gather_tab", tab.data(), sizeof(void*) * tab.size(), (void**)d_tab);
+}
+
+int launch_compact_fused(mvicp_ctx* c, double d2_bound) {
+  if (c->n_cblocks == 0) return MVICP_OK;
   const void** d_tab = nullptr;
-  MV_CHECK(cached_upload(c, "gather_tab", tab.data(), sizeof(void*) * tab.size(), (void**)&d_tab));
+  MV_CHECK(gather_table(c, &d_tab));
+  double bytes = 0;
+  for (int e = 0; e < c->E; ++e) if (c->owned[e]) bytes += 2.0 * 12.0 * c->frames[c->esrc[e]].n;
+  {
+    ProfScope ps(c, "compact", bytes);
+    hipLaunchKernelGGL(count_kernel, dim3(c->n_cblocks), dim3(NT), 0, c->stream, c->d_cblock_off, c->E, c->d_nsrc, c->d_cap_off, c->d_nn_idx,
+                       c->d_nn_d2, d2_bound, c->d_cblock_cnt, c->d_dirty);
+    hipLaunchKernelGGL(scan_kernel, dim3(c->E), dim3(NT), 0, c->stream, c->d_cblock_off, c->d_cblock_cnt, c->d_count, c->d_dirty);
+  }
+  {
+    ProfScope ps(c, "gather", 0.0);
+    hipLaunchKernelGGL(compact_fused_kernel, dim3(c->n_cblocks), dim3(NT), 0, c->stream, c->d_cblock_off, c->E, c->d_nsrc, c->d_cap_off, c->total_cap,
+                       c->d_nn_idx, c->d_nn_d2, d2_bound, c->d_cblock_cnt, c->d_first, c->d_second, c->d_cd2, c->d_qpos, (const PointRec* const*)d_tab,
+                       (const PointRec* const*)(d_tab + c->E), (const double* const*)(d_tab + 2 * c->E), c->d_stream, c->d_dirty);
+  }
+  MV_HIP(hipGetLastError());
+  return MVICP_OK;
+}
+
+int launch_gather_stream(mvicp_ctx* c) {
+  if (c->n_cblocks == 0) return MVICP_OK;
+  const void** d_tab = nullptr;
+  MV_CHECK(gather_table(c, &d_tab));
   {
     ProfScope ps(c, "gather", 0.0);
     hipLaunchKernelGGL(gather_kernel, dim3(c->n_cblocks), dim3(NT), 0, c->stream, c->d_cblock_off, c->E, c->d_count, c->d_cap_off, c->total_cap,
diff --git a/mv-lm-icp_amd/csrc/lin_common.h b/mv-lm-icp_amd/csrc/lin_common.h
--- a/mv-lm-icp_amd/csrc/lin_common.h
+++ b/mv-lm-icp_amd/csrc/lin_common.h
@@ -42,6 +42,12 @@
   }
   const int e = blockIdx.x;
   const int tid = threadIdx.x;
+  double a_pre = 0.0, t_pre[3] = {0.0, 0.0, 0.0};
+  if (tid < 9) {
+    const double* Ap = rel + (size_t)e * kEdgeRel;
+    a_pre = Ap[tid / 3 + 3 * (tid % 3)];
+    t_pre[0] = Ap[9]; t_pre[1] = Ap[10]; t_pre[2] = Ap[11];
+  }
   __shared__ double m[8][NACC];
   __shared__ double S[36], X[36], Y[36], R6[36], Lm[36], T1[36], T2[36], T3[36], H[144], v[6];
   const int c0 = chunk_first[e];
@@ -62,13 +68,11 @@
   }
   __syncthreads();
   const double* mm = m[0];
-  const double* A = rel + (size_t)e * kEdgeRel;
-  const double* t = A + 9;
   if (tid < 9) {
     const int i = tid / 3, j = tid % 3;
     double tx[9];
-    cross_mat(t, tx);
-    const double a = A[i + 3 * j];
+    cross_mat(t_pre, tx);
+    const double a = a_pre;
     R6[i * 6 + j] = a;
     R6[(3 + i) * 6 + 3 + j] = a;
     Lm[(3 + i) * 6 + j] = tx[i * 3 + j];
diff --git a/mv-lm-icp_amd/csrc/linearize.hip b/mv-lm-icp_amd/csrc/linearize.hip
--- a/mv-lm-icp_amd/csrc/linearize.hip
+++ b/mv-lm-icp_amd/csrc/linearize.hip
@@ -72,25 +72,11 @@
   const int end = min(cnt, start + chunk);
   __shared__ double srel[NP][kEdgeRel];
   __shared__ double red[NACC / 2][NT + 1];
-  if (threadIdx.x < kEdgeRel) srel[0][threadIdx.x] = rel[(size_t)e * kEdgeRel + threadIdx.x];
-  if constexpr (NP > 1) { if (threadIdx.x >= 32 && threadIdx.x < 32 + kEdgeRel) srel[1][threadIdx.x - 32] = x.rel2[(size_t)e * kEdgeRel + threadIdx.x - 32]; }
-  __syncthreads();
-  double A[NP][9], t[NP][3];
-#pragma unroll
-  for (int k = 0; k < NP; ++k) {
-#pragma unroll
-    for (int i = 0; i < 9; ++i) A[k][i] = srel[k][i];
-#pragma unroll
-    for (int i = 0; i < 3; ++i) t[k][i] = srel[k][9 + i];
-  }
-  double inv_a2 = 1.0;
-  if (ROBUST) { const double a = a_scale[e]; inv_a2 = 1.0 / (a * a); }
-
-  double acc[NP][NACC];
-#pragma unroll
-  for (int k = 0; k < NP; ++k)
-#pragma unroll
-    for (int i = 0; i < NACC; ++i) acc[k][i] = 0.0;
+  double rel_pre = 0.0;
+  if (threadIdx.x < kEdgeRel) rel_pre = rel[(size_t)e * kEdgeRel + threadIdx.x];
+  if constexpr (NP > 1) { if (threadIdx.x >= 32 && threadIdx.x < 32 + kEdgeRel) rel_pre = x.rel2[(size_t)e * kEdgeRel + threadIdx.x - 32]; }
+  double a_pre = 1.0;
+  if (ROBUST) a_pre = a_scale[e];
 
   const size_t base = (size_t)cap_off[e];
   const double* __restrict__ s0 = stream + base;
@@ -122,6 +108,26 @@
     }
   };
   load(cur, pos);
+  if (threadIdx.x < kEdgeRel) srel[0][threadIdx.x] = rel_pre;
+  if constexpr (NP > 1) { if (threadIdx.x >= 32 && threadIdx.x < 32 + kEdgeRel) srel[1][threadIdx.x - 32] = rel_pre; }
+  __syncthreads();
+  double A[NP][9], t[NP][3];
+#pragma unroll
+  for (int k = 0; k < NP; ++k) {
+#pragma unroll
+    for (int i = 0; i < 9; ++i) A[k][i] = srel[k][i];
+#pragma unroll
+    for (int i = 0; i < 3; ++i) t[k][i] = srel[k][9 + i];
+  }
+  double inv_a2 = 1.0;
+  if (ROBUST) { const double a = a_pre; inv_a2 = 1.0 / (a * a); }
+
+  double acc[NP][NACC];
+#pragma unroll
+  for (int k = 0; k < NP; ++k)
+#pragma unroll
+    for (int i = 0; i < NACC; ++i) acc[k][i] = 0.0;
+
   while (pos < end) {
     const int npos = pos + 2 * NT;
     load(nxt, npos);
@@ -185,14 +191,16 @@
 int launch_linearize(mvicp_ctx* c, int plane, int robust) {
   if (c->E == 0) return MVICP_OK;
   const int chunk = c->lin_chunk;
+  const double* rel = c->lin_rel ? c->lin_rel : c->d_rel;
   if (c->n_chunks > 0) {
     const double bytes = stream_pass_bytes(c, plane);
     const double* const* d_src = nullptr;
     MV_CHECK(source_table(c, &d_src));
     ProfScope ps(c, "linearize", bytes);
+    const double* a_scale = c->lin_rel ? c->lin_rel + (size_t)c->E * kEdgeRel : c->d_a;
 #define LAUNCH(P, R)                                                                                                                           \
   hipLaunchKernelGGL((linearize_kernel<P, R, 1>), dim3(c->n_chunks), dim3(NT), 0, c->stream, c->d_chunk_edge, c->d_chunk_start, chunk, c->d_count, \
-                     c->d_cap_off, c->total_cap, c->d_rel, c->d_a, c->d_stream, c->d_partials, d_src, (const int*)c->d_nsrc, (const int*)c->d_chunk_first, PairArgs<1>{})
+                     c->d_cap_off, c->total_cap, rel, a_scale, c->d_stream, c->d_partials, d_src, (const int*)c->d_nsrc, (const int*)c->d_chunk_first, PairArgs<1>{})
     if (plane && robust) LAUNCH(true, true);
     else if (plane) LAUNCH(true, false);
     else if (robust) LAUNCH(false, true);
@@ -202,9 +210,9 @@
   {
     ProfScope ps(c, "reduce", 0.0);
     if (plane)
-      hipLaunchKernelGGL((reduce_expand_kernel<true, 1>), dim3(c->E), dim3(256), 0, c->stream, c->d_chunk_first, chunk, c->d_count, c->d_rel, c->d_partials, c->lin_out ? c->lin_out : c->d_out, PairArgs<1>{});
+      hipLaunchKernelGGL((reduce_expand_kernel<true, 1>), dim3(c->E), dim3(256), 0, c->stream, c->d_chunk_first, chunk, c->d_count, rel, c->d_partials, c->lin_out ? c->lin_out : c->d_out, PairArgs<1>{});
     else
-      hipLaunchKernelGGL((reduce_expand_kernel<false, 1>), dim3(c->E), dim3(256), 0, c->stream, c->d_chunk_first, chunk, c->d_count, c->d_rel, c->d_partials, c->lin_out ? c->lin_out : c->d_out, PairArgs<1>{});
+      hipLaunchKernelGGL((reduce_expand_kernel<false, 1>), dim3(c->E), dim3(256), 0, c->stream, c->d_chunk_first, chunk, c->d_count, rel, c->d_partials, c->lin_out ? c->lin_out : c->d_out, PairArgs<1>{});
   }
   MV_HIP(hipGetLastError());
   return MVICP_OK;
diff --git a/mv-lm-icp_amd/csrc/nn_grid.hip b/mv-lm-icp_amd/csrc/nn_grid.hip
--- a/mv-lm-icp_amd/csrc/nn_grid.hip
+++ b/mv-lm-icp_amd/csrc/nn_grid.hip
@@ -64,14 +64,19 @@
   return (int)(threadIdx.x & 63) == __ffsll((long long)mask) - 1;
 }
 
-__global__ void dirty_reduce_kernel(int E, const int* __restrict__ slot_off, int* __restrict__ slots, int* __restrict__ dirty) {
+__global__ void dirty_reduce_kernel(int E, const int* __restrict__ slot_off, int* __restrict__ slots, int* __restrict__ dirty,
+                                    const int* __restrict__ presume, const int* __restrict__ nsrc, int* __restrict__ count) {
   const int e = blockIdx.x;
   int any = 0;
   for (int k = slot_off[e] + threadIdx.x; k < slot_off[e + 1]; k += blockDim.x) {
     const int v = slots[k];
     if (v) { any = 1; slots[k] = 0; }
   }
-  if (__syncthreads_or(any) && threadIdx.x == 0) dirty[e] = 1;
+  any = __syncthreads_or(any);
+  if (threadIdx.x == 0) {
+    if (any) dirty[e] = 1;
+    else if (presume[e] != 0) count[e] = nsrc[e];
+  }
 }
 
 template <bool TREE_ONLY>
@@ -894,7 +899,8 @@
       hipLaunchKernelGGL(nn_far_kernel, dim3(far_blocks), dim3(NT), 0, c->stream, d_jobs, (const int2*)c->d_far_list, bound, (const unsigned int*)far_cnt, far_next, d_stats, slots,
                          edge_path ? c->d_far_seen : nullptr);
     if (launch_dirty)
-      hipLaunchKernelGGL(dirty_reduce_kernel, dim3(c->E), dim3(256), 0, c->stream, c->E, c->d_dslot_off, c->d_dirty_slots, c->d_dirty);
+      hipLaunchKernelGGL(dirty_reduce_kernel, dim3(c->E), dim3(256), 0, c->stream, c->E, c->d_dslot_off, c->d_dirty_slots, c->d_dirty, (const int*)c->d_presume,
+                     (const int*)c->d_nsrc, c->d_count);
   }
   MV_HIP(hipGetLastError());
   if (d_stats) MV_CHECK(census_collect(c, d_stats, slots, nq, c->nn_tree_only ? 1 : (use_cell ? 3 : 0), "nn_grid"));
@@ -904,7 +910,8 @@
 }
 
 int launch_dirty_reduce(mvicp_ctx* c) {
-  hipLaunchKernelGGL(dirty_reduce_kernel, dim3(c->E), dim3(256), 0, c->stream, c->E, c->d_dslot_off, c->d_dirty_slots, c->d_dirty);
+  hipLaunchKernelGGL(dirty_reduce_kernel, dim3(c->E), dim3(256), 0, c->stream, c->E, c->d_dslot_off, c->d_dirty_slots, c->d_dirty, (const int*)c->d_presume,
+                     (const int*)c->d_nsrc, c->d_count);
   MV_HIP(hipGetLastError());
   return MVICP_OK;
 }
@@ -937,7 +944,8 @@
     j.out_idx = c->d_nn_idx + c->cap_off[e]; j.out_d2 = c->d_nn_d2 + c->cap_off[e];
     j.inv = d.grid.inv; j.out_lb = c->d_nn_lb + c->cap_off[e];
     j.list = ListRef{c->d_qpos + c->cap_off[e], c->d_second + c->cap_off[e], c->d_cd2 + c->cap_off[e], c->d_dirty + e, c->d_dirty_slots + c->dslot_off[e],
-                     c->d_stream + c->cap_off[e], c->total_cap, d.grid.snor, (const PointRec*)d.grid.srec};
+                     c->d_stream + c->cap_off[e], c->total_cap, d.grid.snor, (const PointRec*)d.grid.srec,
+                     c->d_presume + e, c->d_first + c->cap_off[e], (const PointRec*)s.grid.srec};
     j.seed = ((int)c->nn_cache_edge.size() == c->E && c->nn_cache_edge[e]) ? 1 : 0;
     jobs.push_back(j); dsts.push_back(&d);
   }
diff --git a/mv-lm-icp_amd/csrc/nn_list.h b/mv-lm-icp_amd/csrc/nn_list.h
--- a/mv-lm-icp_amd/csrc/nn_list.h
+++ b/mv-lm-icp_amd/csrc/nn_list.h
@@ -4,13 +4,41 @@
 namespace mvicp {
 
 struct ListRef {
-  const int* qpos; int* second; double* cd2; const int* dirty; int* dirty_slots;
+  int* qpos; int* second; double* cd2; const int* dirty; int* dirty_slots;
   double* stream; long long total_cap; const double* dst_nor;
   const PointRec* dst_srec;
+  const int* presume; int* first; const PointRec* src_srec;
 };
 
-__device__ __forceinline__ void update_list_entry(const ListRef& R, int i, int idx_new, double d2_new, double bound, bool same_neighbour) {
+__device__ __forceinline__ void presumed_list_entry(const ListRef& R, int i, int idx_new, double d2_new, double bound, bool fixup) {
+  if (!(idx_new >= 0 && d2_new < bound)) {
+    if (!fixup) { R.qpos[i] = -1; R.dirty_slots[i / 256] = 1; }
+    return;
+  }
+  R.qpos[i] = i; R.first[i] = i; R.second[i] = idx_new; R.cd2[i] = d2_new;
+  const double2* pa = reinterpret_cast<const double2*>(R.src_srec + i);
+  const double2 a0 = pa[0], a1 = pa[1];
+  const double2* pb = reinterpret_cast<const double2*>(R.dst_srec + idx_new);
+  const double2 b0 = pb[0], b1 = pb[1];
+  double* st = R.stream + i;
+  __builtin_nontemporal_store(a0.x, &st[0 * R.total_cap]);
+  __builtin_nontemporal_store(a0.y, &st[1 * R.total_cap]);
+  __builtin_nontemporal_store(a1.x, &st[2 * R.total_cap]);
+  __builtin_nontemporal_store(b0.x, &st[7 * R.total_cap]);
+  __builtin_nontemporal_store(b0.y, &st[8 * R.total_cap]);
+  __builtin_nontemporal_store(b1.x, &st[9 * R.total_cap]);
+  if (R.dst_nor != nullptr) {
+    const double n0 = R.dst_nor[3 * (size_t)idx_new], n1 = R.dst_nor[3 * (size_t)idx_new + 1], n2 = R.dst_nor[3 * (size_t)idx_new + 2];
+    __builtin_nontemporal_store(n0, &st[3 * R.total_cap]);
+    __builtin_nontemporal_store(n1, &st[4 * R.total_cap]);
+    __builtin_nontemporal_store(n2, &st[5 * R.total_cap]);
+    __builtin_nontemporal_store(n0 * b0.x + n1 * b0.y + n2 * b1.x, &st[6 * R.total_cap]);
+  }
+}
+
+__device__ __forceinline__ void update_list_entry(const ListRef& R, int i, int idx_new, double d2_new, double bound, bool same_neighbour, bool fixup = false) {
   if (*R.dirty != 0) return;
+  if (*R.presume != 0) { presumed_list_entry(R, i, idx_new, d2_new, bound, fixup); return; }
   const int pos = R.qpos[i];
   const bool acc = idx_new >= 0 && d2_new < bound;
   bool clean;
diff --git a/mv-lm-icp_amd/csrc/nn_tie.hip b/mv-lm-icp_amd/csrc/nn_tie.hip
--- a/mv-lm-icp_amd/csrc/nn_tie.hip
+++ b/mv-lm-icp_amd/csrc/nn_tie.hip
@@ -49,7 +49,7 @@
     const int pos = J.inv ? J.inv[bi] : bi;
     if (pos != cur) {
       J.out_idx[i] = pos;
-      if (J.list.dirty) update_list_entry(J.list, i, pos, d2, bound, false);
+      if (J.list.dirty) update_list_entry(J.list, i, pos, d2, bound, false, true);
     }
   }
 }
diff --git a/mv-lm-icp_amd/csrc/nn_tile_common.h b/mv-lm-icp_amd/csrc/nn_tile_common.h
--- a/mv-lm-icp_amd/csrc/nn_tile_common.h
+++ b/mv-lm-icp_amd/csrc/nn_tile_common.h
@@ -248,7 +248,8 @@
     if (with_bounds && with_cache) { j.cache = 1; j.miss_max = c->tile_miss; j.reject_cache = c->reject_cache ? 1 : 0; }
     if (with_list) {
       j.list = ListRef{c->d_qpos + c->cap_off[e], c->d_second + c->cap_off[e], c->d_cd2 + c->cap_off[e], c->d_dirty + e, c->d_dirty_slots + c->dslot_off[e],
-                       c->d_stream + c->cap_off[e], c->total_cap, d.grid.snor, (const PointRec*)d.grid.srec};
+                       c->d_stream + c->cap_off[e], c->total_cap, d.grid.snor, (const PointRec*)d.grid.srec,
+                       c->d_presume + e, c->d_first + c->cap_off[e], (const PointRec*)s.grid.srec};
     }
     j.kacc = (float)c->mfma_kacc; j.trig = c->mfma_trig;
     j.tie = tref; j.tie.job = (unsigned int)jobs.size();
```

Result: faster. 1200 iterations/s, median of 6 (+1.9%).
